# eckertzhang/Text2NeRF

Hardware: AMD Instinct MI355X
Metric: ray-samples/s (render) + iters/s (train), 300^3 VM-split, 800x800 (higher is better)
Workload: dtype f32 (basis/MLP products as f16x2-split MFMA, fp32 accumulate); 1 GPU; C2 300^3 800x800 view/GPU, N=518, S1-soft seed 0, white_bg, weights=0, tile marcher; evaluated_samples_per_frame=77423712, appearance_samples_per_frame=4284741, rays_per_gpu=640000, samples_per_ray=518, warmup_frames=233, inregion_timing=none, parallelism=ray-tile x1

## Files before the change

include/t2n.h:

```cpp
#ifndef T2N_H_
#define T2N_H_

#include <stddef.h>
#include <stdint.h>

#ifdef __cplusplus
extern "C" {
#endif

typedef struct t2n_field t2n_field;
typedef void* t2n_stream;

enum {
    T2N_OK = 0,
    T2N_ERR_INVALID = -1,
    T2N_ERR_UNSUPPORTED = -2,
    T2N_ERR_HIP = -3,
    T2N_ERR_WORKSPACE = -4,
    T2N_ERR_STATE = -5
};

enum { T2N_SHADE_MLP_FEA_NOVIEW = 0, T2N_SHADE_SH = 1, T2N_SHADE_RGB = 2,
       T2N_SHADE_MLP_FEA = 3, T2N_SHADE_MLP_PE = 4, T2N_SHADE_MLP = 5 };
enum { T2N_ACT_SOFTPLUS = 0, T2N_ACT_RELU = 1 };

enum {
    T2N_FLAG_TRAIN = 1u,
    T2N_FLAG_ADD_BG = 2u,
    T2N_FLAG_KEEP_CTX = 4u,
    T2N_FLAG_NDC = 16u,
    T2N_FLAG_DEVICE_ROWS = 32u,
    T2N_FLAG_PIPELINE = 64u,
    T2N_FLAG_GATHER_BATCH = 128u,
    T2N_FLAG_REG_L1 = 256u,
    T2N_FLAG_REG_ORTHO = 512u,
    T2N_FLAG_COHERENT = 8u
};

typedef struct t2n_field_desc {
    float aabb_min[3], aabb_max[3];
    float inv_aabb_size[3];
    int32_t grid[3];
    int32_t density_n_comp;
    int32_t app_n_comp;
    int32_t app_dim;
    int32_t shading;
    int32_t fea_pe;
    int32_t feature_c;
    int32_t act;
    float density_shift;
    float distance_scale;
    float weight_thres;
    float step_size;
    float near, far;
    float z_gate;
    int32_t view_pe, pos_pe;
} t2n_field_desc;

typedef struct t2n_field_params {
    const float* density_plane[3];
    const float* density_line[3];
    const float* app_plane[3];
    const float* app_line[3];
    const float* basis_weight;
    const float* mlp_w0; const float* mlp_b0;
    const float* mlp_w1; const float* mlp_b1;
    const float* mlp_w2; const float* mlp_b2;
} t2n_field_params;

typedef struct t2n_field_grads {
    float* density_plane[3];
    float* density_line[3];
    float* app_plane[3];
    float* app_line[3];
    float* basis_weight;
    float* mlp_w0; float* mlp_b0;
    float* mlp_w1; float* mlp_b1;
    float* mlp_w2; float* mlp_b2;
} t2n_field_grads;

enum { T2N_STAT_EVALUATED = 0,
       T2N_STAT_APPEARANCE = 1,
       T2N_STAT_RAYS = 2,
       T2N_STAT_OVERFLOW = 3,
       T2N_STAT_F16_REDO = 4,
       T2N_STAT_LIST_RETRY = 5,
       T2N_STAT_COUNT = 8 };

const char* t2n_last_error(void);
int t2n_version(void);

int t2n_field_create(const t2n_field_desc* desc, t2n_field** out);
int t2n_field_destroy(t2n_field* f);
int t2n_field_upload(t2n_field* f, const t2n_field_params* p, t2n_stream stream);
int t2n_field_set_desc(t2n_field* f, const t2n_field_desc* desc);
int t2n_field_set_factor_storage(t2n_field* f, int bf16);

int t2n_field_set_mlp_precision(t2n_field* f, int exact_fp32);
int t2n_field_set_alpha_mask(t2n_field* f, const float* volume, int D, int H, int W, const float* aabb_min_host,
                             const float* inv_size_host, t2n_stream stream);
int t2n_alpha_at(const t2n_field* f, const float* xyz_world, int64_t n, float* alpha, t2n_stream stream);
int t2n_field_set_early_termination(t2n_field* f, float eps);
int t2n_field_set_feature_staging(t2n_field* f, int on);
int t2n_field_feature_staging_counts(const t2n_field* f, uint64_t out[2]);
int t2n_field_set_density_cache(t2n_field* f, int on);
int t2n_field_set_density_cache_cap(t2n_field* f, uint64_t bytes);
int t2n_field_release_density_cache(t2n_field* f);
int t2n_field_density_cache_counts(const t2n_field* f, uint64_t out[4]);
int t2n_field_density_sum_table(const t2n_field* f, const int* shift, float* out, t2n_stream stream);
#define T2N_APP_VOLUME_MIN_FRAMES 33
int t2n_field_set_appearance_volume(t2n_field* f, int on, int min_frames);
int t2n_field_set_appearance_volume_cap(t2n_field* f, uint64_t bytes);
int t2n_field_release_appearance_volume(t2n_field* f);
int t2n_field_appearance_volume_counts(const t2n_field* f, uint64_t out[4]);
int t2n_field_set_feature_fusion(t2n_field* f, int on);
int t2n_field_feature_fusion_counts(const t2n_field* f, uint64_t out[2]);
int t2n_render_list_shape(int64_t n_rays, int n_samples, int entries_per_ray, uint64_t out[6]);
int t2n_field_feature_rows(t2n_field* f, const float* app_pos, const uint32_t* counters, uint32_t list_cap, int volume, float* feat,
                           uint32_t feat_rows, t2n_stream stream);
int t2n_field_set_feature_stage_shape(t2n_field* f, int workgroups, int defer_cap);
int t2n_field_set_frame_width(t2n_field* f, int width);

int t2n_ray_directions(int H, int W, float fx, float fy, float cx, float cy, int normalize, float* dirs ,
                       t2n_stream stream);
int t2n_get_rays(const float* dirs , int64_t n, const float* c2w_host ,
                 float* rays_o , float* rays_d , float* rays6 ,
                 t2n_stream stream);
int t2n_generate_rays(int H, int W, float fx, float fy, float cx, float cy, const float* c2w_host, float* rays6,
                      t2n_stream stream);

int t2n_sample_ray(const t2n_field* f, const float* rays_o, const float* rays_d, int64_t n, int n_samples, const float* jitter, int ndc,
                   float* pts , float* z_vals , uint8_t* valid , t2n_stream stream);

int t2n_filter_rays_bbox(const t2n_field* f, const float* rays, int64_t n_rays, int ray_stride, uint8_t* mask,
                         t2n_stream stream);

int t2n_density_at(const t2n_field* f, const float* xyz_norm, int64_t n, float* feat, float* sigma, t2n_stream stream);
size_t t2n_shade_workspace_bytes(int64_t n);
int t2n_shade_at(const t2n_field* f, const float* xyz_norm, const float* viewdirs, int64_t n, float* app_feat, float* rgb,
                 void* workspace, size_t workspace_bytes, t2n_stream stream);
int t2n_raw2alpha(const float* sigma, const float* dist, int64_t n_rays, int n_samples, float* alpha, float* weights,
                  float* bg, t2n_stream stream);

size_t t2n_render_workspace_bytes(int64_t rays_per_launch, int n_samples);
size_t t2n_render_head_scratch_bytes(const t2n_field* f, int64_t n_rays);
int t2n_field_set_head_scratch_rows(t2n_field* f, int rows_per_ray);
size_t t2n_render_workspace_bytes_hint(const t2n_field* f, int64_t n_rays, int n_samples);
size_t t2n_render_workspace_bytes_budget(int64_t n_rays, int n_samples, int entries_per_ray);
uint64_t t2n_field_list_retries(const t2n_field* f);
int t2n_render_forward(t2n_field* f, const float* rays, int64_t n_rays, int ray_stride, int n_samples, uint32_t flags,
                       const float* jitter, float* rgb, float* depth, float* weights, float* z_vals, uint64_t* stats,
                       void* workspace, size_t workspace_bytes, t2n_stream stream);

typedef struct t2n_generic_desc {
    float aabb_min[3], aabb_max[3], inv_aabb_size[3];
    int32_t grid[3];
    int32_t density_n_comp[3], app_n_comp[3];
    int32_t app_dim, shading, fea_pe, view_pe, feature_c, act;
    float density_shift, distance_scale, weight_thres, step_size, near, far, z_gate;
    const float* alpha_volume;
    int32_t alpha_dims[3];
    float alpha_aabb_min[3], alpha_aabb_max[3];
} t2n_generic_desc;
size_t t2n_generic_workspace_bytes(int64_t n_rays, int n_samples);
size_t t2n_generic_workspace_bytes_desc(const t2n_generic_desc* desc, int64_t n_rays, int n_samples);
int t2n_generic_forward(const t2n_generic_desc* desc, const t2n_field_params* params, const float* rays, int64_t n_rays, int ray_stride,
                        int n_samples, uint32_t flags, const float* jitter, float* rgb, float* depth, float* weights, float* z_vals,
                        uint64_t* stats, void* workspace, size_t workspace_bytes, t2n_stream stream);
int t2n_generic_backward(const t2n_generic_desc* desc, const t2n_field_params* params, const float* rays, int64_t n_rays, int ray_stride,
                         int n_samples, uint32_t flags, const float* jitter, const float* weights, const float* z_vals,
                         const float* d_rgb, const float* d_depth, const float* d_weights, const t2n_field_grads* grads,
                         void* workspace, size_t workspace_bytes, t2n_stream stream);
typedef struct t2n_generic_bwd_plan {
    int kernel_form;
    uint32_t pass_rows;
    uint32_t max_passes;
    size_t workspace_bytes;
} t2n_generic_bwd_plan;
int t2n_generic_backward_plan(const t2n_generic_desc* desc, int64_t n_rays, int n_samples, uint32_t pass_rows, t2n_generic_bwd_plan* out);
int t2n_generic_backward_staged(const t2n_generic_desc* desc, const t2n_field_params* params, const float* rays, int64_t n_rays,
                                int ray_stride, int n_samples, uint32_t flags, const float* jitter, const float* weights,
                                const float* z_vals, const float* d_rgb, const float* d_depth, const float* d_weights,
                                const t2n_field_grads* grads, void* workspace, size_t workspace_bytes, void* bwd_workspace,
                                size_t bwd_bytes, uint32_t pass_rows, t2n_stream stream);
int t2n_generic_dense_alpha(const t2n_generic_desc* desc, const t2n_field_params* params, const float* lin_x, const float* lin_y,
                            const float* lin_z, int gx, int gy, int gz, float length, float* alpha, t2n_stream stream);
int t2n_generic_filter_rays(const t2n_generic_desc* desc, const float* rays, int64_t n_rays, int ray_stride, int n_samples, int bbox_only,
                            uint8_t* mask, t2n_stream stream);

int t2n_ndc_rays(int H, int W, float focal, float near, int blender, const float* rays_o, const float* rays_d, int64_t n,
                 float* o_out, float* d_out, t2n_stream stream);

int t2n_eval_sh_bases(int deg, const float* dirs, int64_t n, float* out, t2n_stream stream);

int t2n_ray_marcher(const float* rays, int64_t n, int ray_stride, int n_samples, int lindisp, const float* bbox_host,
                    const float* steps, const float* perturb, float* xyz, float* z_vals, float* near_far, t2n_stream stream);

int t2n_frame_postprocess(const float* rgb , const float* depth , int64_t n, float depth_sub, float depth_add,
                          int shift_clamp, float mi, float ma, uint8_t* rgb8, uint8_t* depth8, const float* gt_rgb, double* sq_err_sum,
                          t2n_stream stream);

size_t t2n_ssim_views_workspace_bytes(int V, int H, int W, int filter_size);
int t2n_ssim_views(const void* img0, const void* img1, int dtype , int V, int H, int W,
                   const double* filter_host , int filter_size, double c1, double c2, int clamp01_img0,
                   double* ssim , double* ssim_map , double* sq_err ,
                   void* workspace, size_t workspace_bytes, t2n_stream stream);

size_t t2n_image_filter_workspace_bytes(int H, int W);
int t2n_sparse_bilateral_filtering(const float* depth , const float* image , int H, int W,
                                   const int* filter_sizes_host, int num_iter, float depth_threshold, float* photo_out,
                                   float* depth_out, void* workspace, size_t workspace_bytes, t2n_stream stream);
size_t t2n_warp_workspace_bytes(int H, int W);
int t2n_warp_view(const float* rgb , const float* depth , const uint8_t* mask1 , int H,
                  int W, const double* Ki9_host, const double* T12_host, const double* K9_host, uint8_t* filled, uint8_t* image_u8,
                  double* depth_out, void* workspace, size_t workspace_bytes, t2n_stream stream);
int t2n_warp_finish(const uint8_t* filled, const uint8_t* image_u8, int H, int W, float* image_out ,
                    int64_t* mask_out , t2n_stream stream);

int t2n_dibr_filter_mask2(float* image, int32_t* known, double* depth, int H, int W, float threshold, t2n_stream stream);
int t2n_dibr_filter_mask(float* image, int32_t* known, int H, int W, t2n_stream stream);

size_t t2n_warp_views_workspace_bytes(int H, int W, int V);
int t2n_warp_views(const float* rgb, const float* depth, const uint8_t* mask1, const uint8_t* mask_aux, int H, int W, int V,
                   const double* Ki9_host, const double* T12_host, const double* K9_host, float* image_out, int64_t* mask_out,
                   double* depth_out, float* depth32_out, int64_t* aux_out, void* workspace, size_t workspace_bytes,
                   t2n_stream stream);

enum { T2N_MASK_U8 = 0, T2N_MASK_I32 = 1, T2N_MASK_I64 = 2, T2N_MASK_F32 = 3, T2N_MASK_F64 = 4 };
size_t t2n_format_views_workspace_bytes(int H, int W, int N);
int t2n_format_views(const float* images, const float* depths, const void* masks, int mask_dtype, int N, int H, int W,
                     const float* c2w_host, float fx, float fy, float cx, float cy, float* rays_split, float* all_rays,
                     float* all_rgbs, float* all_depths, int64_t capacity_rows, int64_t* record, void* workspace,
                     size_t workspace_bytes, t2n_stream stream);

size_t t2n_image_filter_views_workspace_bytes(int H, int W, int V);
int t2n_sparse_bilateral_filtering_views(const float* depth, const float* image, int V, int H, int W, const int* filter_sizes_host,
                                         int num_iter, float depth_threshold, float* photo_out, float* depth_out, void* workspace,
                                         size_t workspace_bytes, t2n_stream stream);
size_t t2n_warp_sources_workspace_bytes(int H, int W, int V);
int t2n_warp_sources(const float* rgb, const float* depth, const uint8_t* mask1, int H, int W, int V, const double* Ki9_host,
                     const double* T12_host, const double* K9_host, float* image_out, int64_t* mask_out, double* depth_out,
                     void* workspace, size_t workspace_bytes, t2n_stream stream);
int t2n_inpaint_pack(const float* warp_image, const int32_t* known, const float* rgb_render, const float* depth_render, int H, int W,
                     uint8_t* warp_u8, int64_t* map_filt, uint8_t* mask_image, uint8_t* mask_inv, int64_t* mask_ex, uint8_t* rgb_u8,
                     uint8_t* rgb_masked_u8, double* depth_masked, t2n_stream stream);

size_t t2n_render_workspace_bytes_ctx(int64_t n_rays, int n_samples);
int t2n_render_ctx_rows(const void* fwd_workspace, int64_t n_rays, int n_samples, t2n_stream stream, int64_t* rows);
int t2n_field_device_rows_record(const t2n_field* f, uint32_t out[10]);
size_t t2n_backward_workspace_bytes(const t2n_field* f, int64_t rows, int64_t n_rays, int n_samples);
int t2n_render_backward(t2n_field* f, const float* rays, int64_t n_rays, int ray_stride, int n_samples, uint32_t flags,
                        const float* jitter, const float* d_rgb, const float* d_depth, const float* d_weights,
                        const t2n_field_grads* g, void* fwd_workspace, size_t fwd_workspace_bytes, void* bwd_workspace,
                        size_t bwd_workspace_bytes, t2n_stream stream);

size_t t2n_field_grad_buffer_bytes(const t2n_field* f);
int t2n_field_set_grad_buffer(t2n_field* f, void* buf, size_t bytes);
size_t t2n_field_grad_buffer_density_bytes(const t2n_field* f);
int t2n_field_wait_density_grads(const t2n_field* f, t2n_stream waiter);

size_t t2n_train_loss_workspace_bytes(int64_t n_rays);
int t2n_train_loss(const float* rgb, const float* depth, const float* weights, const float* z_vals, const float* rgb_t,
                   const float* depth_t, int64_t n_rays, int n_samples, float w_depth, float w_trans, float delta, float* d_rgb,
                   float* d_depth, float* d_weights, float* losses, void* workspace, size_t workspace_bytes, t2n_stream stream);

size_t t2n_train_loss_ex_workspace_bytes(int64_t n_rays);
int t2n_train_loss_ex(const float* rgb, const float* depth, const float* weights, const float* z_vals, const float* rgb_t,
                      const float* depth_t, int64_t n_rays, int n_samples, float w_depth, float w_trans, float delta, int depth_kind,
                      float target_std, float* d_rgb, float* d_depth, float* d_weights, float* losses, double* aux, void* workspace,
                      size_t workspace_bytes, t2n_stream stream);
// ... 140 lines not shown
```

text2nerf_amd/_lib.py:

```python
from __future__ import annotations

import ctypes as C
import os
import threading

_HERE = os.path.dirname(os.path.abspath(__file__))
LIB_PATH = os.environ.get("T2N_LIB") or os.path.join(_HERE, "libt2n_hip.so")

T2N_STAT_COUNT = 8
T2N_K_COUNT = 14
KERNEL_NAMES = ("march", "shade", "composite", "upload", "bwd_march", "bwd_mlp", "bwd_scatter", "density", "app_features",
                "bwd_wgrad", "bwd_density", "tv_seed", "adam", "head_step")
STAT_EVALUATED, STAT_APPEARANCE, STAT_RAYS, STAT_OVERFLOW, STAT_F16_REDO, STAT_LIST_RETRY = 0, 1, 2, 3, 4, 5

FLAG_TRAIN, FLAG_ADD_BG, FLAG_KEEP_CTX, FLAG_COHERENT, FLAG_NDC = 1, 2, 4, 8, 16
FLAG_DEVICE_ROWS = 32
FLAG_PIPELINE = 64
FLAG_GATHER_BATCH = 128
FLAG_REG_L1, FLAG_REG_ORTHO = 256, 512
REG_SLOTS = 64
SHADE_IDS = {"MLP_Fea_noview": 0, "SH": 1, "RGB": 2, "MLP_Fea": 3, "MLP_PE": 4, "MLP": 5}
ACT_IDS = {"softplus": 0, "relu": 1}
DEPTH_KINDS = {"mse": 0, "gnll": 1, "si_log": 2, "ssi": 3}
MASK_U8, MASK_I32, MASK_I64, MASK_F32, MASK_F64 = 0, 1, 2, 3, 4


class T2NError(RuntimeError):
    pass


class FieldDesc(C.Structure):
    _fields_ = [("aabb_min", C.c_float * 3), ("aabb_max", C.c_float * 3), ("inv_aabb_size", C.c_float * 3),
                ("grid", C.c_int32 * 3), ("density_n_comp", C.c_int32), ("app_n_comp", C.c_int32),
                ("app_dim", C.c_int32), ("shading", C.c_int32), ("fea_pe", C.c_int32), ("feature_c", C.c_int32),
                ("act", C.c_int32), ("density_shift", C.c_float), ("distance_scale", C.c_float),
                ("weight_thres", C.c_float), ("step_size", C.c_float), ("near", C.c_float), ("far", C.c_float),
                ("z_gate", C.c_float), ("view_pe", C.c_int32), ("pos_pe", C.c_int32)]


class FieldParams(C.Structure):
    _fields_ = [("density_plane", C.c_void_p * 3), ("density_line", C.c_void_p * 3), ("app_plane", C.c_void_p * 3),
                ("app_line", C.c_void_p * 3), ("basis_weight", C.c_void_p),
                ("mlp_w0", C.c_void_p), ("mlp_b0", C.c_void_p), ("mlp_w1", C.c_void_p), ("mlp_b1", C.c_void_p),
                ("mlp_w2", C.c_void_p), ("mlp_b2", C.c_void_p)]


FieldGrads = FieldParams


class GenericDesc(C.Structure):
    _fields_ = [("aabb_min", C.c_float * 3), ("aabb_max", C.c_float * 3), ("inv_aabb_size", C.c_float * 3), ("grid", C.c_int32 * 3),
                ("density_n_comp", C.c_int32 * 3), ("app_n_comp", C.c_int32 * 3), ("app_dim", C.c_int32), ("shading", C.c_int32),
                ("fea_pe", C.c_int32), ("view_pe", C.c_int32), ("feature_c", C.c_int32), ("act", C.c_int32),
                ("density_shift", C.c_float), ("distance_scale", C.c_float), ("weight_thres", C.c_float), ("step_size", C.c_float),
                ("near", C.c_float), ("far", C.c_float), ("z_gate", C.c_float),
                ("alpha_volume", C.c_void_p), ("alpha_dims", C.c_int32 * 3), ("alpha_aabb_min", C.c_float * 3),
                ("alpha_aabb_max", C.c_float * 3)]


class GenericBwdPlan(C.Structure):
    _fields_ = [("kernel_form", C.c_int), ("pass_rows", C.c_uint32), ("max_passes", C.c_uint32), ("workspace_bytes", C.c_size_t)]


TRAIN_HYPER_FLOATS = 32
TRAIN_HEAD_GRAD_FLOATS = 27 * 144 + 128 * 351 + 128 + 128 * 128 + 128 + 3 * 128 + 3 + 1
TRAIN_HEAD_SIZES = (27 * 144, 128 * 351, 128, 128 * 128, 128, 3 * 128, 3)


class TrainStepArgs(C.Structure):
    _fields_ = [("rays", C.c_void_p), ("n_rays", C.c_int64), ("ray_stride", C.c_int32), ("n_samples", C.c_int32),
                ("flags", C.c_uint32), ("phases", C.c_uint32),
                ("jitter", C.c_void_p), ("rgb_target", C.c_void_p), ("depth_target", C.c_void_p),
                ("w_depth", C.c_float), ("w_trans", C.c_float), ("delta", C.c_float),
                ("beta1", C.c_float), ("beta2", C.c_float), ("eps", C.c_float),
                ("hyper", C.c_void_p), ("params", FieldParams),
                ("exp_avg", C.c_void_p * 19), ("exp_avg_sq", C.c_void_p * 19),
                ("head_grads", C.c_void_p), ("rows_capacity", C.c_int64),
                ("workspace", C.c_void_p), ("workspace_bytes", C.c_size_t), ("losses", C.c_void_p), ("host_batch", C.c_void_p), ("host_batch_bytes", C.c_size_t), ("batch_buffer", C.c_void_p),
                ("shard_world", C.c_int32), ("shard_rank", C.c_int32)]


class TrainSource(C.Structure):
    _fields_ = [("rays", C.c_void_p), ("ray_stride", C.c_int32), ("rgb", C.c_void_p), ("depth", C.c_void_p), ("n_rows", C.c_int64),
                ("ids", C.c_void_p)]


_lib = None
_lock = threading.Lock()

SIGNATURES = {
    "t2n_last_error": (C.c_char_p, []),
    "t2n_version": (C.c_int, []),
    "t2n_field_create": (C.c_int, [C.POINTER(FieldDesc), C.POINTER(C.c_void_p)]),
    "t2n_field_destroy": (C.c_int, [C.c_void_p]),
    "t2n_field_upload": (C.c_int, [C.c_void_p, C.POINTER(FieldParams), C.c_void_p]),
    "t2n_field_set_desc": (C.c_int, [C.c_void_p, C.POINTER(FieldDesc)]),
    "t2n_field_set_mlp_precision": (C.c_int, [C.c_void_p, C.c_int]),
    "t2n_field_set_early_termination": (C.c_int, [C.c_void_p, C.c_float]),
    "t2n_field_set_feature_staging": (C.c_int, [C.c_void_p, C.c_int]),
    "t2n_field_feature_staging_counts": (C.c_int, [C.c_void_p, C.POINTER(C.c_uint64)]),
    "t2n_field_set_feature_stage_shape": (C.c_int, [C.c_void_p, C.c_int, C.c_int]),
    "t2n_field_set_density_cache": (C.c_int, [C.c_void_p, C.c_int]),
    "t2n_field_set_density_cache_cap": (C.c_int, [C.c_void_p, C.c_uint64]),
    "t2n_field_release_density_cache": (C.c_int, [C.c_void_p]),
    "t2n_field_density_cache_counts": (C.c_int, [C.c_void_p, C.POINTER(C.c_uint64)]),
    "t2n_field_set_appearance_volume": (C.c_int, [C.c_void_p, C.c_int, C.c_int]),
    "t2n_field_set_appearance_volume_cap": (C.c_int, [C.c_void_p, C.c_uint64]),
    "t2n_field_release_appearance_volume": (C.c_int, [C.c_void_p]),
    "t2n_field_appearance_volume_counts": (C.c_int, [C.c_void_p, C.POINTER(C.c_uint64)]),
    "t2n_field_set_feature_fusion": (C.c_int, [C.c_void_p, C.c_int]),
    "t2n_field_feature_fusion_counts": (C.c_int, [C.c_void_p, C.POINTER(C.c_uint64)]),
    "t2n_render_list_shape": (C.c_int, [C.c_int64, C.c_int, C.c_int, C.POINTER(C.c_uint64)]),
    "t2n_field_feature_rows": (C.c_int, [C.c_void_p, C.c_void_p, C.c_void_p, C.c_uint32, C.c_int, C.c_void_p, C.c_uint32, C.c_void_p]),
    "t2n_field_density_sum_table": (C.c_int, [C.c_void_p, C.POINTER(C.c_int), C.c_void_p, C.c_void_p]),
    "t2n_sample_ray": (C.c_int, [C.c_void_p, C.c_void_p, C.c_void_p, C.c_int64, C.c_int, C.c_void_p, C.c_int, C.c_void_p, C.c_void_p,
                                 C.c_void_p, C.c_void_p]),
    "t2n_field_set_frame_width": (C.c_int, [C.c_void_p, C.c_int]),
    "t2n_field_set_alpha_mask": (C.c_int, [C.c_void_p, C.c_void_p, C.c_int, C.c_int, C.c_int, C.POINTER(C.c_float),
                                           C.POINTER(C.c_float), C.c_void_p]),
    "t2n_alpha_at": (C.c_int, [C.c_void_p, C.c_void_p, C.c_int64, C.c_void_p, C.c_void_p]),
    "t2n_ray_directions": (C.c_int, [C.c_int, C.c_int, C.c_float, C.c_float, C.c_float, C.c_float, C.c_int,
                                     C.c_void_p, C.c_void_p]),
    "t2n_get_rays": (C.c_int, [C.c_void_p, C.c_int64, C.POINTER(C.c_float), C.c_void_p, C.c_void_p, C.c_void_p,
                               C.c_void_p]),
    "t2n_generate_rays": (C.c_int, [C.c_int, C.c_int, C.c_float, C.c_float, C.c_float, C.c_float,
                                    C.POINTER(C.c_float), C.c_void_p, C.c_void_p]),
    "t2n_filter_rays_bbox": (C.c_int, [C.c_void_p, C.c_void_p, C.c_int64, C.c_int, C.c_void_p, C.c_void_p]),
    "t2n_density_at": (C.c_int, [C.c_void_p, C.c_void_p, C.c_int64, C.c_void_p, C.c_void_p, C.c_void_p]),
    "t2n_shade_workspace_bytes": (C.c_size_t, [C.c_int64]),
    "t2n_shade_at": (C.c_int, [C.c_void_p, C.c_void_p, C.c_void_p, C.c_int64, C.c_void_p, C.c_void_p, C.c_void_p,
                               C.c_size_t, C.c_void_p]),
    "t2n_raw2alpha": (C.c_int, [C.c_void_p, C.c_void_p, C.c_int64, C.c_int, C.c_void_p, C.c_void_p, C.c_void_p,
                                C.c_void_p]),
    "t2n_render_workspace_bytes": (C.c_size_t, [C.c_int64, C.c_int]),
    "t2n_render_head_scratch_bytes": (C.c_size_t, [C.c_void_p, C.c_int64]),
    "t2n_field_set_head_scratch_rows": (C.c_int, [C.c_void_p, C.c_int]),
    "t2n_render_workspace_bytes_hint": (C.c_size_t, [C.c_void_p, C.c_int64, C.c_int]),
    "t2n_field_list_retries": (C.c_uint64, [C.c_void_p]),
    "t2n_render_workspace_bytes_budget": (C.c_size_t, [C.c_int64, C.c_int, C.c_int]),
    "t2n_render_forward": (C.c_int, [C.c_void_p, C.c_void_p, C.c_int64, C.c_int, C.c_int, C.c_uint32, C.c_void_p,
                                     C.c_void_p, C.c_void_p, C.c_void_p, C.c_void_p, C.c_void_p, C.c_void_p,
                                     C.c_size_t, C.c_void_p]),
    "t2n_render_workspace_bytes_ctx": (C.c_size_t, [C.c_int64, C.c_int]),
    "t2n_depth_align_global": (C.c_int, [C.c_void_p, C.c_void_p, C.c_int, C.c_int, C.c_void_p, C.c_int, C.c_double, C.c_void_p, C.c_void_p,
                                         C.c_void_p]),
    "t2n_depth_align_fallback": (C.c_int, [C.c_void_p, C.c_void_p, C.c_int, C.c_int, C.c_double, C.c_void_p, C.c_void_p, C.c_void_p]),
    "t2n_filled_pixels_workspace_bytes": (C.c_size_t, [C.c_int, C.c_int]),
    "t2n_filled_pixels_count": (C.c_int, [C.c_void_p, C.c_int, C.c_int, C.c_void_p, C.c_void_p, C.c_void_p]),
    "t2n_filled_pixels_select": (C.c_int, [C.c_void_p, C.c_int, C.c_int, C.c_void_p, C.c_void_p, C.c_int, C.c_void_p, C.c_void_p]),
    "t2n_depth_merge_inputs": (C.c_int, [C.c_void_p, C.c_void_p, C.c_void_p, C.c_int, C.c_int, C.c_double, C.c_void_p, C.c_void_p,
                                         C.c_void_p, C.c_void_p]),
    "t2n_view_finish": (C.c_int, [C.c_void_p, C.c_void_p, C.c_void_p, C.c_int, C.c_int, C.c_double, C.c_void_p, C.c_void_p, C.c_void_p,
                                  C.c_void_p]),
    "t2n_mask_expand": (C.c_int, [C.c_void_p, C.c_int, C.c_int, C.c_void_p, C.c_void_p, C.c_void_p]),
    "t2n_mc_workspace_bytes": (C.c_size_t, [C.c_int, C.c_int, C.c_int]),
    "t2n_mc_count": (C.c_int, [C.c_void_p, C.c_int, C.c_int, C.c_int, C.c_float, C.c_void_p, C.c_void_p, C.c_void_p]),
    "t2n_mc_emit": (C.c_int, [C.c_void_p, C.c_int, C.c_int, C.c_int, C.c_float, C.c_void_p, C.POINTER(C.c_float), C.POINTER(C.c_float),
                              C.c_int, C.c_void_p, C.c_void_p, C.c_void_p, C.c_void_p]),
    "t2n_mesh_components_workspace_bytes": (C.c_size_t, [C.c_int64, C.c_int64]),
    "t2n_mesh_components": (C.c_int, [C.c_void_p, C.c_int64, C.c_int64, C.c_void_p, C.c_void_p, C.c_void_p, C.c_size_t, C.c_void_p]),
    "t2n_mesh_component_sizes": (C.c_int, [C.c_void_p, C.c_int64, C.c_void_p, C.c_int64, C.c_int64, C.c_void_p, C.c_void_p, C.c_void_p]),
    "t2n_mesh_filter_count": (C.c_int, [C.c_void_p, C.c_int64, C.c_void_p, C.c_int64, C.c_void_p, C.c_int64, C.c_void_p, C.c_size_t,
                                        C.c_void_p, C.c_void_p]),
    "t2n_mesh_filter_emit": (C.c_int, [C.c_void_p, C.c_int64, C.c_void_p, C.c_int64, C.c_void_p, C.c_int64, C.c_void_p, C.c_void_p,
                                       C.c_void_p, C.c_void_p, C.c_size_t, C.c_void_p, C.c_void_p, C.c_void_p, C.c_void_p, C.c_void_p]),
    "t2n_field_grad_buffer_bytes": (C.c_size_t, [C.c_void_p]),
    "t2n_field_set_grad_buffer": (C.c_int, [C.c_void_p, C.c_void_p, C.c_size_t]),
    "t2n_field_grad_buffer_density_bytes": (C.c_size_t, [C.c_void_p]),
    "t2n_field_wait_density_grads": (C.c_int, [C.c_void_p, C.c_void_p]),
    "t2n_train_loss_workspace_bytes": (C.c_size_t, [C.c_int64]),
    "t2n_train_loss": (C.c_int, [C.c_void_p, C.c_void_p, C.c_void_p, C.c_void_p, C.c_void_p, C.c_void_p, C.c_int64, C.c_int, C.c_float,
                                 C.c_float, C.c_float, C.c_void_p, C.c_void_p, C.c_void_p, C.c_void_p, C.c_void_p, C.c_size_t, C.c_void_p]),
    "t2n_train_loss_ex_workspace_bytes": (C.c_size_t, [C.c_int64]),
    "t2n_train_loss_ex": (C.c_int, [C.c_void_p, C.c_void_p, C.c_void_p, C.c_void_p, C.c_void_p, C.c_void_p, C.c_int64, C.c_int, C.c_float,
                                    C.c_float, C.c_float, C.c_int, C.c_float, C.c_void_p, C.c_void_p, C.c_void_p, C.c_void_p, C.c_void_p,
                                    C.c_void_p, C.c_size_t, C.c_void_p]),
    "t2n_depth_loss_workspace_bytes": (C.c_size_t, [C.c_int64]),
    "t2n_depth_loss": (C.c_int, [C.c_int, C.c_void_p, C.c_void_p, C.c_void_p, C.c_void_p, C.c_int64, C.c_int, C.c_float, C.c_void_p,
                                 C.c_void_p, C.c_void_p, C.c_void_p, C.c_void_p, C.c_size_t, C.c_void_p]),
    "t2n_distortion_loss_workspace_bytes": (C.c_size_t, [C.c_int64]),
    "t2n_distortion_loss": (C.c_int, [C.c_void_p, C.c_void_p, C.c_int64, C.c_int, C.c_float, C.c_void_p, C.c_void_p, C.c_void_p, C.c_size_t,
                                      C.c_void_p]),
    "t2n_train_loss_dist_workspace_bytes": (C.c_size_t, [C.c_int64]),
    "t2n_train_loss_dist": (C.c_int, [C.c_void_p, C.c_void_p, C.c_void_p, C.c_void_p, C.c_void_p, C.c_void_p, C.c_int64, C.c_int, C.c_float,
                                      C.c_float, C.c_float, C.c_int, C.c_float, C.c_float, C.c_float, C.c_void_p, C.c_void_p, C.c_void_p,
                                      C.c_void_p, C.c_void_p, C.c_void_p, C.c_void_p, C.c_size_t, C.c_void_p]),
    "t2n_field_set_factor_storage": (C.c_int, [C.c_void_p, C.c_int]),
    "t2n_frame_postprocess": (C.c_int, [C.c_void_p, C.c_void_p, C.c_int64, C.c_float, C.c_float, C.c_int, C.c_float, C.c_float,
                              C.c_void_p, C.c_void_p, C.c_void_p, C.c_void_p, C.c_void_p]),
    "t2n_ssim_views_workspace_bytes": (C.c_size_t, [C.c_int, C.c_int, C.c_int, C.c_int]),
    "t2n_ssim_views": (C.c_int, [C.c_void_p, C.c_void_p, C.c_int, C.c_int, C.c_int, C.c_int, C.POINTER(C.c_double), C.c_int, C.c_double,
                                 C.c_double, C.c_int, C.c_void_p, C.c_void_p, C.c_void_p, C.c_void_p, C.c_size_t, C.c_void_p]),
    "t2n_image_filter_workspace_bytes": (C.c_size_t, [C.c_int, C.c_int]),
    "t2n_sparse_bilateral_filtering": (C.c_int, [C.c_void_p, C.c_void_p, C.c_int, C.c_int, C.POINTER(C.c_int), C.c_int, C.c_float,
                                                 C.c_void_p, C.c_void_p, C.c_void_p, C.c_size_t, C.c_void_p]),
    "t2n_warp_workspace_bytes": (C.c_size_t, [C.c_int, C.c_int]),
    "t2n_warp_view": (C.c_int, [C.c_void_p, C.c_void_p, C.c_void_p, C.c_int, C.c_int, C.POINTER(C.c_double), C.POINTER(C.c_double),
                                C.POINTER(C.c_double), C.c_void_p, C.c_void_p, C.c_void_p, C.c_void_p, C.c_size_t, C.c_void_p]),
    "t2n_warp_finish": (C.c_int, [C.c_void_p, C.c_void_p, C.c_int, C.c_int, C.c_void_p, C.c_void_p, C.c_void_p]),
    "t2n_warp_views_workspace_bytes": (C.c_size_t, [C.c_int, C.c_int, C.c_int]),
    "t2n_warp_views": (C.c_int, [C.c_void_p, C.c_void_p, C.c_void_p, C.c_void_p, C.c_int, C.c_int, C.c_int, C.POINTER(C.c_double),
                                 C.POINTER(C.c_double), C.POINTER(C.c_double), C.c_void_p, C.c_void_p, C.c_void_p, C.c_void_p,
                                 C.c_void_p, C.c_void_p, C.c_size_t, C.c_void_p]),
    "t2n_format_views_workspace_bytes": (C.c_size_t, [C.c_int, C.c_int, C.c_int]),
    "t2n_format_views": (C.c_int, [C.c_void_p, C.c_void_p, C.c_void_p, C.c_int, C.c_int, C.c_int, C.c_int, C.POINTER(C.c_float),
                                   C.c_float, C.c_float, C.c_float, C.c_float, C.c_void_p, C.c_void_p, C.c_void_p, C.c_void_p,
                                   C.c_int64, C.c_void_p, C.c_void_p, C.c_size_t, C.c_void_p]),
    "t2n_image_filter_views_workspace_bytes": (C.c_size_t, [C.c_int, C.c_int, C.c_int]),
    "t2n_sparse_bilateral_filtering_views": (C.c_int, [C.c_void_p, C.c_void_p, C.c_int, C.c_int, C.c_int, C.POINTER(C.c_int), C.c_int,
                                                       C.c_float, C.c_void_p, C.c_void_p, C.c_void_p, C.c_size_t, C.c_void_p]),
    "t2n_warp_sources_workspace_bytes": (C.c_size_t, [C.c_int, C.c_int, C.c_int]),
    "t2n_warp_sources": (C.c_int, [C.c_void_p, C.c_void_p, C.c_void_p, C.c_int, C.c_int, C.c_int, C.POINTER(C.c_double),
                                   C.POINTER(C.c_double), C.POINTER(C.c_double), C.c_void_p, C.c_void_p, C.c_void_p, C.c_void_p,
                                   C.c_size_t, C.c_void_p]),
    "t2n_inpaint_pack": (C.c_int, [C.c_void_p, C.c_void_p, C.c_void_p, C.c_void_p, C.c_int, C.c_int, C.c_void_p, C.c_void_p, C.c_void_p,
                                   C.c_void_p, C.c_void_p, C.c_void_p, C.c_void_p, C.c_void_p, C.c_void_p]),
    "t2n_adam_step_multi": (C.c_int, [C.c_int, C.c_void_p, C.c_void_p, C.c_void_p, C.c_void_p, C.c_void_p, C.c_void_p, C.c_float,
                            C.c_float, C.c_float, C.c_void_p, C.c_void_p]),
    "t2n_ray_marcher": (C.c_int, [C.c_void_p, C.c_int64, C.c_int, C.c_int, C.c_int, C.POINTER(C.c_float), C.c_void_p, C.c_void_p,
                        C.c_void_p, C.c_void_p, C.c_void_p, C.c_void_p]),
    "t2n_dibr_filter_mask2": (C.c_int, [C.c_void_p, C.c_void_p, C.c_void_p, C.c_int, C.c_int, C.c_float, C.c_void_p]),
    "t2n_dibr_filter_mask": (C.c_int, [C.c_void_p, C.c_void_p, C.c_int, C.c_int, C.c_void_p]),
    "t2n_eval_sh_bases": (C.c_int, [C.c_int, C.c_void_p, C.c_int64, C.c_void_p, C.c_void_p]),
    "t2n_ndc_rays": (C.c_int, [C.c_int, C.c_int, C.c_float, C.c_float, C.c_int, C.c_void_p, C.c_void_p, C.c_int64, C.c_void_p,
                     C.c_void_p, C.c_void_p]),
    "t2n_render_ctx_rows": (C.c_int, [C.c_void_p, C.c_int64, C.c_int, C.c_void_p, C.POINTER(C.c_int64)]),
    "t2n_field_device_rows_record": (C.c_int, [C.c_void_p, C.POINTER(C.c_uint32)]),
    "t2n_backward_workspace_bytes": (C.c_size_t, [C.c_void_p, C.c_int64, C.c_int64, C.c_int]),
    "t2n_render_backward": (C.c_int, [C.c_void_p, C.c_void_p, C.c_int64, C.c_int, C.c_int, C.c_uint32, C.c_void_p,
                                      C.c_void_p, C.c_void_p, C.c_void_p, C.POINTER(FieldGrads), C.c_void_p, C.c_size_t,
                                      C.c_void_p, C.c_size_t, C.c_void_p]),
    "t2n_tv_grad_add": (C.c_int, [C.c_void_p, C.c_void_p, C.c_int, C.c_int, C.c_int, C.c_float, C.c_void_p]),
    "t2n_tv_value": (C.c_int, [C.c_void_p, C.c_int, C.c_int, C.c_int, C.c_void_p, C.c_void_p]),
    "t2n_tv_grad_set": (C.c_int, [C.c_void_p, C.c_void_p, C.c_int, C.c_int, C.c_int, C.c_float, C.c_void_p, C.c_void_p]),
    "t2n_field_tv_adam_step": (C.c_int, [C.c_void_p, C.c_void_p, C.c_void_p, C.c_void_p, C.c_void_p, C.c_void_p, C.c_float, C.c_float,
                                         C.c_float, C.c_float, C.c_float, C.c_void_p]),
    "t2n_field_tv_seed": (C.c_int, [C.c_void_p, C.c_float, C.c_float, C.c_void_p]),
    "t2n_l1_value": (C.c_int, [C.c_void_p, C.c_int64, C.c_void_p, C.c_void_p]),
    "t2n_l1_grad_add": (C.c_int, [C.c_void_p, C.c_void_p, C.c_int64, C.c_float, C.c_void_p]),
    "t2n_l1_grad_set": (C.c_int, [C.c_void_p, C.c_void_p, C.c_int64, C.c_float, C.c_void_p, C.c_void_p]),
    "t2n_ortho_workspace_bytes": (C.c_size_t, [C.c_int]),
    "t2n_ortho_value": (C.c_int, [C.c_void_p, C.c_int, C.c_int64, C.c_void_p, C.c_void_p, C.c_size_t, C.c_void_p]),
    "t2n_ortho_grad_add": (C.c_int, [C.c_void_p, C.c_void_p, C.c_int, C.c_int64, C.c_float, C.c_void_p, C.c_size_t, C.c_void_p]),
    "t2n_ortho_grad_set": (C.c_int, [C.c_void_p, C.c_void_p, C.c_int, C.c_int64, C.c_float, C.c_void_p, C.c_void_p, C.c_size_t,
                                     C.c_void_p]),
    "t2n_field_reg_seed": (C.c_int, [C.c_void_p, C.c_float, C.c_float, C.c_float, C.c_float, C.c_float, C.c_float, C.c_void_p]),
    "t2n_field_reg_adam_step": (C.c_int, [C.c_void_p, C.c_void_p, C.c_void_p, C.c_void_p, C.c_void_p, C.c_void_p, C.c_float, C.c_float,
                                          C.c_float, C.c_float, C.c_float, C.c_float, C.c_float, C.c_float, C.c_float, C.c_void_p]),
    "t2n_field_upload_head": (C.c_int, [C.c_void_p, C.c_void_p, C.c_void_p]),
    "t2n_adam_step": (C.c_int, [C.c_void_p, C.c_void_p, C.c_void_p, C.c_void_p, C.c_int64, C.c_float, C.c_float, C.c_float,
                                C.c_float, C.c_int64, C.c_void_p]),
    "t2n_compute_alpha": (C.c_int, [C.c_void_p, C.c_void_p, C.c_int64, C.c_float, C.c_void_p, C.c_void_p]),
    "t2n_dense_alpha": (C.c_int, [C.c_void_p, C.c_void_p, C.c_void_p, C.c_void_p, C.c_int, C.c_int, C.c_int, C.c_float,
                                  C.c_void_p, C.c_void_p]),
    "t2n_alpha_volume": (C.c_int, [C.c_void_p, C.c_int, C.c_int, C.c_int, C.c_float, C.c_void_p, C.c_void_p, C.c_void_p]),
    "t2n_upsample_bilinear": (C.c_int, [C.c_void_p, C.c_int, C.c_int, C.c_int, C.c_void_p, C.c_int, C.c_int, C.c_void_p]),
    "t2n_filter_rays_alpha": (C.c_int, [C.c_void_p, C.c_void_p, C.c_int64, C.c_int, C.c_int, C.c_void_p, C.c_void_p]),
    "t2n_generic_workspace_bytes": (C.c_size_t, [C.c_int64, C.c_int]),
    "t2n_generic_workspace_bytes_desc": (C.c_size_t, [C.POINTER(GenericDesc), C.c_int64, C.c_int]),
    "t2n_generic_forward": (C.c_int, [C.POINTER(GenericDesc), C.POINTER(FieldParams), C.c_void_p, C.c_int64, C.c_int, C.c_int, C.c_uint32,
                                      C.c_void_p, C.c_void_p, C.c_void_p, C.c_void_p, C.c_void_p, C.c_void_p, C.c_void_p, C.c_size_t,
                                      C.c_void_p]),
    "t2n_generic_backward": (C.c_int, [C.POINTER(GenericDesc), C.POINTER(FieldParams), C.c_void_p, C.c_int64, C.c_int, C.c_int, C.c_uint32,
                                       C.c_void_p, C.c_void_p, C.c_void_p, C.c_void_p, C.c_void_p, C.c_void_p, C.POINTER(FieldGrads),
# ... 60 lines not shown
```

text2nerf_amd/csrc/t2n_api.hip:

```cpp
#include <stdarg.h>

#include "t2n_device.h"

namespace t2n {

static thread_local char g_err[512] = "";

void set_error(const char* fmt, ...) {
    va_list ap;
    va_start(ap, fmt);
    vsnprintf(g_err, sizeof(g_err), fmt, ap);
    va_end(ap);
}

int hip_fail(hipError_t e, const char* what) {
    set_error("HIP error %d (%s) in %s", (int)e, hipGetErrorString(e), what);
    return T2N_ERR_HIP;
}

void timing_begin(t2n_field* f, int k, hipStream_t s) {
    if (!((f->timing >> k) & 1)) return;
    TimingSlot& t = f->slots[k];
    if (t.used >= kTimingEvents) return;
    if (!t.start[t.used]) {
// ... 751 lines not shown
                    ShadeCtx ctx{nullptr, feat32 - row0 * 32, nullptr, nullptr};
                    if ((rc = launch_shade_list(f, L.app_pos, L.app_ray, L.rays, ray_stride, L.counters, L.list_cap, L.app_rgb, &ctx, s, true,
                                                (unsigned)(row0 + cap), nullptr, 0, nullptr, (unsigned)(row0 / 32), (unsigned)((row0 + cap) / 32)))) return rc;
                    if ((rc = launch_head_forward(f, nullptr, cap, feat32, L.app_pos, L.app_ray, L.rays, ray_stride, L.counters, L.list_cap, x0, h0,
                                                  h1, L.app_rgb, s, plan, row0))) return rc;
                }
            }
        } else {
            if (kr.rows >= 32) {
                ShadeCtx ctx{(float*)(ws + kr.x144), (float*)(ws + kr.feat32), (float*)(ws + kr.h0), (float*)(ws + kr.h1)};
                if ((rc = launch_shade_list(f, L.app_pos, L.app_ray, L.rays, ray_stride, L.counters, L.list_cap, L.app_rgb, &ctx, s, false, kr.rows))) return rc;
            } else if ((rc = launch_shade_list(f, L.app_pos, L.app_ray, L.rays, ray_stride, L.counters, L.list_cap, L.app_rgb, nullptr, s, false,
                                               0xffffffffu, keep ? nullptr : L.feat, L.feat_rows, stats, 0, 0xffffffffu, L.slot_rows))) return rc;
        }
        if ((rc = tiles ? launch_composite(f, L, s, f->frame_w, (int)(cnt / f->frame_w)) : launch_composite(f, L, s))) return rc;
        if (tiles && finish_supported(f) && (rc = launch_finish_rays(f, L, (const float*)(ws + c.sigma), (const float4*)(ws + c.scratch), s))) return rc;
    }
    return T2N_OK;
}

extern "C" size_t t2n_render_workspace_bytes_hint(const t2n_field* f, int64_t n_rays, int n_samples) {
    if (!f || n_rays <= 0 || n_samples <= 0) return 0;
    counts_poll(const_cast<t2n_field*>(f), false);
    const size_t worst = carve(n_rays, n_samples).total;
    if (n_rays < kBudgetMinRays) return worst;
    unsigned b = f->list_hint ? f->list_hint + f->list_hint / 2u + 12u : 32u;
    if (b < kBudgetMin) b = kBudgetMin;
    if (b >= (unsigned)n_samples) return worst;
    const size_t want = carve_workspace(n_rays, n_samples, true, true, b).total;
    return want < worst ? want : worst;
}
extern "C" uint64_t t2n_field_list_retries(const t2n_field* f) {
    if (!f) return 0;
    counts_poll(const_cast<t2n_field*>(f), true);
    return f->list_retries;
}
extern "C" size_t t2n_render_workspace_bytes_budget(int64_t n_rays, int n_samples, int entries_per_ray) {
    if (n_rays <= 0 || n_samples <= 0 || entries_per_ray < 0) return 0;
    return carve_workspace(n_rays, n_samples, true, true, (unsigned)entries_per_ray).total;
}

extern "C" int t2n_field_set_alpha_mask(t2n_field* f, const float* volume, int D, int H, int W, const float* aabb_min_host,
                                        const float* inv_size_host, t2n_stream stream) {
    if (!f) { set_error("t2n_field_set_alpha_mask: NULL field"); return T2N_ERR_INVALID; }
    if (f->buf_alpha) { T2N_HIP(hipStreamSynchronize((hipStream_t)stream)); (void)hipFree(f->buf_alpha); f->buf_alpha = nullptr; }
    f->dev.alpha = nullptr;
    if (!volume) return T2N_OK;
    if (D < 1 || H < 1 || W < 1 || !aabb_min_host || !inv_size_host) { set_error("t2n_field_set_alpha_mask: bad argument"); return T2N_ERR_INVALID; }
    const size_t bytes = (size_t)D * H * W * sizeof(float);
    T2N_HIP(hipMalloc((void**)&f->buf_alpha, bytes));
    T2N_HIP(hipMemcpyAsync(f->buf_alpha, volume, bytes, hipMemcpyDeviceToDevice, (hipStream_t)stream));
    f->dev.alpha = f->buf_alpha; f->dev.aD = D; f->dev.aH = H; f->dev.aW = W;
    for (int k = 0; k < 3; ++k) { f->dev.a_min[k] = aabb_min_host[k]; f->dev.a_inv[k] = inv_size_host[k]; }
    return T2N_OK;
}

extern "C" int t2n_field_set_head_scratch_rows(t2n_field* f, int rows_per_ray) {
    if (!f || rows_per_ray < 1 || rows_per_ray > 4096) { set_error("t2n_field_set_head_scratch_rows: rows_per_ray must lie in [1, 4096]"); return T2N_ERR_INVALID; }
    f->head_rows_per_ray = rows_per_ray;
    return T2N_OK;
}

extern "C" int t2n_field_set_frame_width(t2n_field* f, int width) {
    if (!f || width < 0) { set_error("t2n_field_set_frame_width: bad argument"); return T2N_ERR_INVALID; }
    f->frame_w = width;
    return T2N_OK;
}

extern "C" int t2n_field_set_factor_storage(t2n_field* f, int bf16) {
    if (!f) { set_error("t2n_field_set_factor_storage: NULL field"); return T2N_ERR_INVALID; }
    if ((bf16 != 0) != (f->factor_bf16 != 0)) f->uploaded = false;
    f->factor_bf16 = bf16 ? 1 : 0;
    if (!f->factor_bf16)
        for (int k = 0; k < 3; ++k) {
            f->dev.den.plane_h[k] = f->dev.den.line_h[k] = f->dev.app.plane_h[k] = f->dev.app.line_h[k] = nullptr;
        }
    return T2N_OK;
}

extern "C" int t2n_field_set_early_termination(t2n_field* f, float eps) {
    if (!f || !(eps >= 0.f) || eps > f->desc.weight_thres) {
        set_error("t2n_field_set_early_termination: eps must lie in [0, weight_thres]");
        return T2N_ERR_INVALID;
    }
    f->term_eps = eps;
    return T2N_OK;
}

extern "C" int t2n_field_set_mlp_precision(t2n_field* f, int exact_fp32) {
    if (!f) { set_error("t2n_field_set_mlp_precision: NULL field"); return T2N_ERR_INVALID; }
    f->mlp_split = exact_fp32 ? 0 : 1;
    return T2N_OK;
}

extern "C" int t2n_field_set_feature_staging(t2n_field* f, int on) {
    if (!f) { set_error("t2n_field_set_feature_staging: NULL field"); return T2N_ERR_INVALID; }
    f->feature_staging = on ? 1 : 0;
    return T2N_OK;
}

extern "C" int t2n_field_set_density_cache(t2n_field* f, int on) {
    if (!f) { set_error("t2n_field_set_density_cache: NULL field"); return T2N_ERR_INVALID; }
    f->dcache_on = on ? 1 : 0;
    return T2N_OK;
}
extern "C" int t2n_field_set_density_cache_cap(t2n_field* f, uint64_t bytes) {
    if (!f) { set_error("t2n_field_set_density_cache_cap: NULL field"); return T2N_ERR_INVALID; }
    f->dcache_cap = (size_t)bytes;
    f->dcache_alloc_failed = false;
    return T2N_OK;
}
extern "C" int t2n_field_release_density_cache(t2n_field* f) {
    if (!f) { set_error("t2n_field_release_density_cache: NULL field"); return T2N_ERR_INVALID; }
    density_cache_release(f);
    return T2N_OK;
}
extern "C" int t2n_field_density_cache_counts(const t2n_field* f, uint64_t out[4]) {
    if (!f || !out) { set_error("t2n_field_density_cache_counts: NULL argument"); return T2N_ERR_INVALID; }
    out[0] = f->dcache_counts[0]; out[1] = f->dcache_counts[1]; out[2] = f->dcache_counts[2]; out[3] = (uint64_t)f->dcache_bytes;
    return T2N_OK;
}
extern "C" int t2n_field_set_appearance_volume(t2n_field* f, int on, int min_frames) {
    if (!f || min_frames < 0) { set_error("t2n_field_set_appearance_volume: NULL field or min_frames < 0"); return T2N_ERR_INVALID; }
    f->avol_on = on ? 1 : 0;
    f->avol_min_frames = min_frames ? min_frames : T2N_APP_VOLUME_MIN_FRAMES;
    return T2N_OK;
}
extern "C" int t2n_field_set_appearance_volume_cap(t2n_field* f, uint64_t bytes) {
    if (!f) { set_error("t2n_field_set_appearance_volume_cap: NULL field"); return T2N_ERR_INVALID; }
    f->avol_cap = (size_t)bytes;
    f->avol_alloc_failed = false;
    return T2N_OK;
}
extern "C" int t2n_field_release_appearance_volume(t2n_field* f) {
    if (!f) { set_error("t2n_field_release_appearance_volume: NULL field"); return T2N_ERR_INVALID; }
    appearance_volume_release(f);
    return T2N_OK;
}
extern "C" int t2n_field_appearance_volume_counts(const t2n_field* f, uint64_t out[4]) {
    if (!f || !out) { set_error("t2n_field_appearance_volume_counts: NULL argument"); return T2N_ERR_INVALID; }
    out[0] = (uint64_t)f->avol_bytes; out[1] = f->avol_counts[2]; out[2] = f->avol_counts[0]; out[3] = f->avol_counts[1];
    return T2N_OK;
}
extern "C" int t2n_field_set_feature_fusion(t2n_field* f, int on) {
    if (!f) { set_error("t2n_field_set_feature_fusion: NULL field"); return T2N_ERR_INVALID; }
    f->fusion_on = on ? 1 : 0;
    return T2N_OK;
}
extern "C" int t2n_field_feature_fusion_counts(const t2n_field* f, uint64_t out[2]) {
    if (!f || !out) { set_error("t2n_field_feature_fusion_counts: NULL argument"); return T2N_ERR_INVALID; }
    out[0] = f->fusion_counts[0]; out[1] = f->fusion_counts[1];
    return T2N_OK;
}
extern "C" int t2n_render_list_shape(int64_t n_rays, int n_samples, int entries_per_ray, uint64_t out[6]) {
    if (n_rays <= 0 || n_samples <= 0 || entries_per_ray < 0 || !out) { set_error("t2n_render_list_shape: bad argument"); return T2N_ERR_INVALID; }
    const Carve c = carve_workspace(n_rays, n_samples, true, true, (unsigned)entries_per_ray);
    out[0] = c.list_cap; out[1] = c.feat_rows; out[2] = fuse_rows(c.list_cap, c.feat_rows) ? 1 : 0;
    out[3] = c.app_pos; out[4] = c.feat; out[5] = c.counters;
    return T2N_OK;
}
extern "C" int t2n_field_feature_rows(t2n_field* f, const float* app_pos, const uint32_t* counters, uint32_t list_cap, int volume, float* feat,
                                      uint32_t feat_rows, t2n_stream stream) {
    if (!f || !app_pos || !counters || !feat || feat_rows % 32u) { set_error("t2n_field_feature_rows: bad argument"); return T2N_ERR_INVALID; }
    if (!f->uploaded) { set_error("t2n_field_feature_rows: the field has no uploaded parameters"); return T2N_ERR_STATE; }
    if (f->desc.shading != T2N_SHADE_MLP_FEA_NOVIEW || !f->mlp_split) { set_error("t2n_field_feature_rows: needs the fused MLP_Fea_noview head on split products"); return T2N_ERR_UNSUPPORTED; }
    hipStream_t s = (hipStream_t)stream;
    AvolScope avol_scope{f};
    f->dev.avol = nullptr;
    if (volume) {
        const int on = f->avol_on, mf = f->avol_min_frames;
        f->avol_on = 1; f->avol_min_frames = 1;
        const int rc = appearance_volume_prepare(f, s);
        f->avol_on = on; f->avol_min_frames = mf;
        if (rc) return rc;
        if (!f->dev.avol) { set_error("t2n_field_feature_rows: this field gets no feature volume (cap, addressing, allocation)"); return T2N_ERR_UNSUPPORTED; }
    }
    return launch_feature_rows(f, (const float4*)app_pos, counters, list_cap, feat, feat_rows, s);
}
extern "C" int t2n_field_density_sum_table(const t2n_field* f, const int* shift, float* out, t2n_stream stream) {
    if (!f || !shift || !out) { set_error("t2n_field_density_sum_table: NULL argument"); return T2N_ERR_INVALID; }
    if (!f->uploaded) { set_error("t2n_field_density_sum_table: the field has no uploaded factors"); return T2N_ERR_STATE; }
    return launch_density_sum_table(f, out, shift, (hipStream_t)stream);
}

extern "C" int t2n_field_set_feature_stage_shape(t2n_field* f, int workgroups, int defer_cap) {
    if (!f) { set_error("t2n_field_set_feature_stage_shape: NULL field"); return T2N_ERR_INVALID; }
    if (workgroups < 0 || defer_cap < 0 || defer_cap > 64) { set_error("t2n_field_set_feature_stage_shape: workgroups >= 0, defer_cap in [0, 64]"); return T2N_ERR_INVALID; }
    f->feature_workgroups = workgroups;
    f->feature_defer_cap = defer_cap ? defer_cap : 16;
    return T2N_OK;
}

extern "C" int t2n_field_feature_staging_counts(const t2n_field* f, uint64_t out[2]) {
    if (!f || !out) { set_error("t2n_field_feature_staging_counts: NULL argument"); return T2N_ERR_INVALID; }
    out[0] = out[1] = 0;
    if (!f->staging_counts) return T2N_OK;
    T2N_HIP(hipDeviceSynchronize());
    unsigned long long h[2];
    T2N_HIP(hipMemcpy(h, f->staging_counts, sizeof(h), hipMemcpyDeviceToHost));
    out[0] = h[0]; out[1] = h[1];
    return T2N_OK;
}

extern "C" int t2n_timing_enable(t2n_field* f, int on) {
    if (!f) return T2N_ERR_INVALID;
    f->timing = on == 0 ? 0 : (on == 1 ? (1 << T2N_K_COUNT) - 1 : (on >> 1) & ((1 << T2N_K_COUNT) - 1));
    return T2N_OK;
}

extern "C" int t2n_timing_read(t2n_field* f, double* ms, int64_t* launches, int reset) {
    if (!f || !ms || !launches) { set_error("t2n_timing_read: NULL argument"); return T2N_ERR_INVALID; }
    timing_flush(f);
    for (int k = 0; k < T2N_K_COUNT; ++k) {
        ms[k] = f->slots[k].ms; launches[k] = f->slots[k].launches;
        if (reset) { f->slots[k].ms = 0.0; f->slots[k].launches = 0; }
    }
    return T2N_OK;
}
```

text2nerf_amd/csrc/t2n_app_rows.h:

```cpp
#pragma once
#include "t2n_internal.h"
#include "t2n_device.h"

namespace t2n {

struct AvVolume { const float* avol; unsigned row, slice, ny1; };

template <int LPE>
__device__ __forceinline__ void av_feature_row(const FactorSet& app, const AvVolume& v, const float4 mine, const bool live, const int q,
                                               float* __restrict__ row, const bool store) {
    constexpr int NQ = 8 / LPE;
    const char* __restrict__ V = reinterpret_cast<const char*>(v.avol);
    const Axes3 A = sample_axes_inbox(app, mine.x, mine.y, mine.z);
    const unsigned ix = (unsigned)min(max(A.a[0].i0, 0), app.W[0] - 1), iy = (unsigned)min(max(A.a[1].i0, 0), app.H[0] - 1);
    const unsigned iz = (unsigned)min(max(A.a[2].i0, 0), app.H[1] - 1);
    const unsigned cell = umad24(umad24(iz, v.ny1, iy), v.row, ix * kAvCornerBytes);
    const unsigned o00 = (live ? cell : 0u) + (unsigned)q * 16u;
    const unsigned o01 = o00 + v.row, o10 = o00 + v.slice, o11 = o10 + v.row;
    const unsigned off[4] = {o00, o01, o10, o11};
    float4 c[4][2][NQ];
#pragma unroll
    for (int zy = 0; zy < 4; ++zy)
#pragma unroll
        for (int x = 0; x < 2; ++x)
#pragma unroll
            for (int i = 0; i < NQ; ++i)
                c[zy][x][i] = *reinterpret_cast<const float4*>(V + (size_t)off[zy] + ((int)kAvCornerBytes * x + 16 * LPE * i));
    __builtin_amdgcn_sched_barrier(0);
    const float wx0 = live ? A.a[0].w0 : 0.f, wx1 = live ? A.a[0].w1 : 0.f;
    const float wyx[2][2] = {{A.a[1].w0 * wx0, A.a[1].w0 * wx1}, {A.a[1].w1 * wx0, A.a[1].w1 * wx1}};
    const float wz[2] = {A.a[2].w0, A.a[2].w1};
    float4 r[NQ];
#pragma unroll
    for (int zy = 0; zy < 4; ++zy)
#pragma unroll
        for (int x = 0; x < 2; ++x) {
            const float w = wyx[zy & 1][x] * wz[zy >> 1];
#pragma unroll
            for (int i = 0; i < NQ; ++i) r[i] = (zy == 0 && x == 0) ? f4_mul(c[0][0][i], w) : f4_fma(c[zy][x][i], w, r[i]);
        }
    if (q == 6 % LPE) r[6 / LPE].w = live ? mine.w : 0.f;
    if (q == 7 % LPE) r[7 / LPE] = make_float4(0.f, 0.f, 0.f, 0.f);
    if (store) {
#pragma unroll
        for (int i = 0; i < NQ; ++i) *reinterpret_cast<float4*>(row + 4 * LPE * i) = r[i];
    }
}

__device__ __forceinline__ void av_slot_rows(const FactorSet& app, const AvVolume& v, const float4* pos, float* feat, unsigned count, int lane) {
    typedef unsigned u32x4_t __attribute__((ext_vector_type(4)));
    const int e = lane >> 3, q = lane & 7;
    const auto rsrc = __builtin_amdgcn_make_buffer_rsrc(const_cast<float4*>(pos), 0, (int)(count * 16u), 0x00020000);
#pragma unroll 1
    for (unsigned c0 = 0; c0 < count; c0 += 64u) {
        const unsigned left = count - c0;
        const unsigned mine_i = (unsigned)lane < left ? c0 + (unsigned)lane : count - 1u;
        const u32x4_t p = __builtin_amdgcn_raw_buffer_load_b128(rsrc, (int)(mine_i * 16u), 0, 16);
        const unsigned npass = left < 64u ? (left + 7u) >> 3 : 8u;
#pragma unroll 1
        for (unsigned s = 0; s < npass; ++s) {
            const int src = (int)(8u * s) + e;
            const float4 mine = make_float4(__uint_as_float(__shfl(p.x, src)), __uint_as_float(__shfl(p.y, src)),
                                            __uint_as_float(__shfl(p.z, src)), __uint_as_float(__shfl(p.w, src)));
            const bool live = (unsigned)src < left;
            av_feature_row<8>(app, v, mine, live, q, feat + (size_t)(c0 + (unsigned)src) * 32u + 4u * (unsigned)q, live);
        }
    }
}

}
```

text2nerf_amd/csrc/t2n_internal.h:

```cpp
#pragma once
#include <hip/hip_runtime.h>
#include <stdint.h>
#include <stdio.h>
#include <string.h>

#include "../../include/t2n.h"

namespace t2n {

constexpr int kWave = 64;
constexpr int kMaxSamples = 8192;
constexpr int kAppDimMax = 32;

__host__ __device__ constexpr int mat0(int k) { return k == 2 ? 1 : 0; }
__host__ __device__ constexpr int mat1(int k) { return k == 0 ? 1 : 2; }
__host__ __device__ constexpr int vecm(int k) { return 2 - k; }

struct FactorSet {
    const float* plane[3];
    const float* line[3];
    int W[3], H[3], L[3];
    int C;
    const void* plane_h[3];
    const void* line_h[3];
};

struct FieldDev {
    FactorSet den, app;
    float aabb0[3], aabb1[3], inv[3];
    float shift, dscale, thres, step, near, far, zgate;
    int act, shading, app_dim;
    const float* basisA;
    const float* w0A;
    const float* w1A;
    const float* w2A;
    const float* alpha; int aW, aH, aD; float a_min[3], a_inv[3];
    const uint4* basisH; const uint4* w0H; const uint4* w1H; const uint4* w2H; const float* biasH;
    const float* ztab;
    float term_eps;
    const float* dsum; unsigned ds_row, ds_slice;
    const float* avol; unsigned av_row, av_slice;
};

struct TrainScalars {
    float lr_over_bc1[19];
    float inv_bc2_sqrt;
    unsigned skip;
    unsigned pad[3];
};
struct TrainState {
    unsigned step;
    unsigned seq;
    unsigned skipped;
    unsigned pad[5];
    TrainScalars sc[2];
};

constexpr int kTimingEvents = 1024;
struct TimingSlot {
    hipEvent_t start[kTimingEvents], stop[kTimingEvents];
    int used = 0;
    int64_t untimed = 0;
    double ms = 0.0;
    int64_t launches = 0;
};

}

struct t2n_field {
    t2n_field_desc desc;
    t2n::FieldDev dev;
    float* buf_den_plane[3] = {nullptr, nullptr, nullptr};
    float* buf_den_line[3] = {nullptr, nullptr, nullptr};
    float* buf_app_plane[3] = {nullptr, nullptr, nullptr};
    float* buf_app_line[3] = {nullptr, nullptr, nullptr};
    void* hbuf_den_plane[3] = {nullptr, nullptr, nullptr};
    void* hbuf_den_line[3] = {nullptr, nullptr, nullptr};
    void* hbuf_app_plane[3] = {nullptr, nullptr, nullptr};
    void* hbuf_app_line[3] = {nullptr, nullptr, nullptr};
    int factor_bf16 = 0;
    float* buf_mlp = nullptr;
    void* buf_mlp_h = nullptr;
    const unsigned* split_unsafe = nullptr;
    void* buf_ss = nullptr;
    bool ss_dirty = true;
    void* ss_event = nullptr; void* ss_stream = nullptr;
    unsigned* ss_ok_host = nullptr; void* ss_ok_event = nullptr; int ss_variant = -2;
    float* buf_alpha = nullptr;
    int mlp_split = 1;
    int feature_staging = 1;
    unsigned long long* staging_counts = nullptr;
    int feature_defer_cap = 16;
    int feature_workgroups = 0;
    float* gbuf_den_plane[3] = {nullptr, nullptr, nullptr};
    float* gbuf_den_line[3] = {nullptr, nullptr, nullptr};
    float* gbuf_app_plane[3] = {nullptr, nullptr, nullptr};
    float* gbuf_app_line[3] = {nullptr, nullptr, nullptr};
    bool gbuf_external = false;
    float* gbuf_all = nullptr; size_t gbuf_bytes = 0;
    t2n_field_params params_ref;
    bool uploaded = false;
    int timing = 0;
    int frame_w = 0;
    int head_rows_per_ray = 32;
    float term_eps = 0.f;
    t2n::TimingSlot slots[T2N_K_COUNT];
    static constexpr int kCountSlots = 4;
    struct CountSlot { unsigned* host = nullptr; void* ev = nullptr; bool pending = false; int64_t n_rays = 0; int n_samples = 0; unsigned budget = 0; };
    CountSlot count_slots[kCountSlots]; int count_next = 0;
    void* side_stream = nullptr; void* ev_fork = nullptr; void* ev_join = nullptr;
    void* ev_den = nullptr;
    unsigned* plan_host = nullptr; unsigned plan_seq = 0;
    void* ev_pack = nullptr;
    void* gemm_stream = nullptr; void* ev_fork2 = nullptr; void* ev_join2 = nullptr;
    void* train_dev = nullptr; unsigned* train_host = nullptr; void* train_ev[12] = {};
    unsigned train_calls = 0; bool train_chain = false;
    bool train_packed = false;
    t2n_train_source train_src = {}; bool train_src_set = false;
    bool train_src_fresh = false;
    unsigned list_hint = 0;
    void* reg_ws = nullptr; size_t reg_ws_bytes = 0;
    unsigned long long list_retries = 0;
    float* dcache = nullptr; size_t dcache_bytes = 0;
    unsigned long long den_version = 1, dcache_version = 0, dcache_seen = 0;
    int dcache_on = 1; size_t dcache_cap = 0;
    bool dcache_alloc_failed = false;
    void* dcache_ev = nullptr; void* dcache_stream = nullptr;
    unsigned long long dcache_counts[3] = {0, 0, 0};
    float* avol = nullptr; size_t avol_bytes = 0;
    unsigned long long app_version = 1, avol_version = 0, avol_seen = 0, avol_run = 0;
    int avol_on = 1, avol_min_frames = T2N_APP_VOLUME_MIN_FRAMES; size_t avol_cap = 0;
    bool avol_alloc_failed = false;
    void* avol_ev = nullptr; void* avol_stream = nullptr;
    unsigned long long avol_counts[3] = {0, 0, 0};
    int fusion_on = 1;
    unsigned long long fusion_counts[2] = {0, 0};
};

namespace t2n {

void set_error(const char* fmt, ...);
int hip_fail(hipError_t e, const char* what);

#define T2N_HIP(call)                                        \
    do {                                                     \
        hipError_t e__ = (call);                             \
        if (e__ != hipSuccess) return t2n::hip_fail(e__, #call); \
    } while (0)

void counts_poll(t2n_field* f, bool wait);
void timing_begin(t2n_field* f, int k, hipStream_t s);
void timing_end(t2n_field* f, int k, hipStream_t s);

int launch_relayout(t2n_field* f, const t2n_field_params* p, hipStream_t s);
int launch_pack_mlp(t2n_field* f, const t2n_field_params* p, hipStream_t s, unsigned* absmax_out = nullptr);

struct RenderLaunch {
    const float* rays; int64_t n_rays; int ray_stride; int n_samples; uint32_t flags;
    const float* jitter; float* rgb; float* depth; float* weights; float* z_vals; uint64_t* stats;
    float* acc; int4* ray_app; unsigned* counters; float4* app_pos; int* app_ray; float4* app_rgb; unsigned list_cap;
    float* feat = nullptr; unsigned feat_rows = 0;
    bool slot_rows = false;
    float* sigma_ctx; float4* rgb_raw;
};
int launch_march(t2n_field* f, const RenderLaunch& L, hipStream_t s);
int launch_ray_stats(const RenderLaunch& L, hipStream_t s);
int launch_filter_bbox(const FieldDev& F, const float* rays, long long n_rays, int ray_stride, uint8_t* mask, hipStream_t s);
int launch_filter_alpha(const FieldDev& F, const float* rays, long long n_rays, int ray_stride, int n_samples, uint8_t* mask, hipStream_t s);
size_t density_cache_bytes(const t2n_field* f);
int density_cache_prepare(t2n_field* f, hipStream_t s);
void density_cache_release(t2n_field* f);
int launch_density_sum_table(const t2n_field* f, float* out, const int shift[3], hipStream_t s);
#ifndef T2N_AVOL_STRIDE
#define T2N_AVOL_STRIDE 32
#endif
constexpr int kAvStride = T2N_AVOL_STRIDE;
constexpr int kAvFeatures = 27;
constexpr unsigned kAvCornerBytes = kAvStride * sizeof(float);
static_assert(kAvStride % 4 == 0 && kAvStride >= 28 && kAvStride <= 32, "corner stride: whole quads that hold the 27 features");
struct AvolScope { t2n_field* f; ~AvolScope() { f->dev.avol = nullptr; } };
size_t appearance_volume_bytes(const t2n_field* f);
int appearance_volume_prepare(t2n_field* f, hipStream_t s);
void appearance_volume_release(t2n_field* f);
int launch_app_volume_build(const t2n_field* f, float* out, hipStream_t s);
int launch_app_features_vol(t2n_field* f, const float4* app_pos, const unsigned* counters_dev, unsigned list_cap, unsigned tile_hi, float* feat,
                            hipStream_t s);
int launch_feature_rows(t2n_field* f, const float4* app_pos, const unsigned* counters_dev, unsigned list_cap, float* feat, unsigned feat_rows,
                        hipStream_t s);
int launch_march_tiles(t2n_field* f, const RenderLaunch& L, int img_w, int img_h, float* spill, float4* scratch, hipStream_t s);
constexpr int kLists = 8;
inline bool fuse_rows(unsigned list_cap, unsigned feat_rows) { return feat_rows && (unsigned long long)list_cap * kLists <= feat_rows; }
constexpr int kCounterStride = 64;
inline unsigned list_capacity(long long n_rays, int n_samples) {
    const unsigned nblocks = (unsigned)((n_rays + 3) / 4);
    return ((nblocks >> 3) + ((nblocks & 7u) ? 1u : 0u)) * 4u * (unsigned)n_samples + (unsigned)n_samples;
}
inline unsigned list_capacity_budget(long long n_rays, int n_samples, unsigned budget) {
    const unsigned worst = list_capacity(n_rays, n_samples);
    if (budget == 0 || budget >= (unsigned)n_samples) return worst;
    const unsigned long long per = ((unsigned long long)n_rays * budget + kLists - 1) / kLists + (unsigned)n_samples;
    return per < worst ? (unsigned)per : worst;
}
struct ShadeCtx { float* x144; float* feat32; float* h0; float* h1; };
int launch_shade_list(t2n_field* f, const float4* app_pos, const int* app_ray, const float* rays, int ray_stride,
                      const unsigned* counters_dev, unsigned list_cap, float4* app_rgb, const ShadeCtx* ctx, hipStream_t s,
                      bool features_only = false, unsigned ctx_rows = 0xffffffffu, float* feat = nullptr, unsigned feat_rows = 0,
                      uint64_t* stats = nullptr, unsigned tile_lo = 0, unsigned tile_hi = 0xffffffffu, bool slot_rows = false);
constexpr int kRangeFlagWord = 32;
constexpr int kKeptMagicWord = 33, kKeptRowsWord = 34;
constexpr int kOverflowWord = 35;
constexpr int kHeadPlanWord = 40;
constexpr int kFailEntriesWord = 36;
constexpr unsigned kKeptMagic = 0x4b455054u;
int launch_mlp_ss(t2n_field* f, const float* feat, const unsigned* counters_dev, unsigned list_cap, unsigned tile_hi, float4* app_rgb,
                  unsigned* range_flag, hipStream_t s, bool slot_rows = false);

struct HeadDims { int shading, C, fea_pe, view_pe, pos_pe, o_feat, o_view, o_pe_a, n_pe_a, o_pe_v, n_pe_v, K0, K0pad; };
HeadDims head_dims(const t2n_field_desc& d);
inline bool head_is_generic(int shading) { return shading == T2N_SHADE_MLP_FEA || shading == T2N_SHADE_MLP_PE || shading == T2N_SHADE_MLP; }
struct HeadPlanDev { unsigned t[kLists + 1]; unsigned rows; };
int launch_head_plan(const unsigned* counters, unsigned list_cap, HeadPlanDev* plan, hipStream_t s);
int launch_dense_rows(const float* IN, int ldin, const float* Wt, int K, int N, const float* bias, int relu, long long rows, float* OUT, int ldo,
                      hipStream_t s, const HeadPlanDev* plan, long long row0);
int launch_head_forward(t2n_field* f, const unsigned tiles_before[kLists + 1], long long rows, const float* feat32, const float4* app_pos,
                        const int* app_ray, const float* rays, int ray_stride, const unsigned* counters, unsigned list_cap, float* x0,
                        float* h0, float* h1, float4* app_rgb, hipStream_t s, const HeadPlanDev* plan = nullptr, long long row0 = 0);
int launch_head_in_bwd(t2n_field* f, const float* gx, const float* feat32, long long rows, float* gf, hipStream_t s);
struct SetupOps {
    unsigned* zero_ptr[6]; unsigned long long zero_words[6]; int nz = 0;
    unsigned* set_ptr[4]; unsigned set_val[4]; int ns = 0;
    bool overflow = false;
    void zero(void* p, size_t bytes) {
        if (!p || !bytes) return;
        if (nz >= 6) { overflow = true; return; }
        zero_ptr[nz] = (unsigned*)p; zero_words[nz] = (bytes + 3) / 4; ++nz;
    }
    void set(void* p, unsigned v) {
        if (ns >= 4) { overflow = true; return; }
        set_ptr[ns] = (unsigned*)p; set_val[ns] = v; ++ns;
    }
};
int launch_setup(const SetupOps& o, hipStream_t s);
int launch_simple_head_bwd(t2n_field* f, const unsigned tiles_before[kLists + 1], long long rows, const float4* go, const float4* app_rgb,
                           const int* app_ray, const float* rays, int ray_stride, const unsigned* counters, unsigned list_cap, float* gf,
                           hipStream_t s);

size_t gemm_h_pack_bytes(int K0);
int gemm_h_pack(t2n_field* f, void* buf, int K0, hipStream_t s);
int launch_gemm_nn_h(void* packbuf, int which, int K0, const float* IN, int ldin, long long rows, const float* ACT, int ldact, float* OUT,
                     int ldo, hipStream_t s);
int launch_gemm_tn_b(const float* A, int lda, const float* B, int ldb, long long rows, int N, float* part, int ldp, int chunk_rows,
                     int ng, int chunks, bool pe, float* db, hipStream_t s, const unsigned* rows_dev = nullptr);
struct TnPlan { int chunk_rows, chunks, ng, ldp; };
TnPlan tn_plan(int64_t rows, int N);
size_t tn_part_bytes(int64_t rows, int k0);
bool gemm_fp32_mode(const t2n_field* f);
void launch_bwd_l2(const float4* go, const float* h1, long long rows, const float* w2, float* g1, float* dw2, float* db2, float* scratch,
                   hipStream_t s, const unsigned* rows_dev = nullptr);
void launch_gemm_tn(int MB, bool fp32, const float* A, int lda, const float* B, int ldb, long long rows, int M, int N, float* C, int ldc,
                    float* part, hipStream_t s, const float* pe_feat = nullptr, float* db = nullptr, const unsigned* rows_dev = nullptr,
                    bool reduce = true);
struct WgradRegions { size_t l2, tn[3], total; };
WgradRegions wgrad_regions(int64_t rows, int k0);
void launch_wgrad_reduce(const char* base, long long rows, float* dw2, float* db2, float* dw1, float* dw0, float* dwb, hipStream_t s,
                         const float* loss_part = nullptr, long long n_rays = 0, float w_depth = 0.f, float w_trans = 0.f, float* losses = nullptr);
void launch_gemm_nn(const float* IN, int ldin, const float* W, int ldw, long long rows, int K, int N, const float* ACT, int ldact, float* OUT,
                    int ldo, hipStream_t s);
void launch_colsum(const float* G, int ld, long long rows, int N, float* db, hipStream_t s);
void launch_pe_fwd(const float* feat, long long rows, float* x, hipStream_t s);
void launch_pe_bwd(const float* gx, const float* feat, long long rows, float* gf, hipStream_t s);
size_t mlp_bwd_ss_pack_bytes();
int launch_mlp_bwd_ss(t2n_field* f, void* packbuf, const float4* go, float* h1, const float* h0, const float* feat, float* g0, float* gf,
                      float* gx, long long rows, hipStream_t s, bool packed = false, const unsigned* rows_dev = nullptr,
                      float* g1_out = nullptr);
int mlp_bwd_ss_pack(t2n_field* f, void* packbuf, hipStream_t s, bool zeroed, bool one_launch = false, bool absmax_done = false);
void* mlp_bwd_ss_absmax_words(void* packbuf);
int launch_tv_seed_dev(t2n_field* f, const float* tvw_dev, hipStream_t s, int world = 1, int rank = 0, bool l1_dev = false);
int launch_ortho_lines(t2n_field* f, float w_den, float w_app, const float* w_dev, hipStream_t s);
size_t reg_ws_bytes(const t2n_field* f);
int launch_factor_adam_dev(t2n_field* f, const t2n_field_params* params, float* const* m, float* const* v, float beta1, float beta2, float eps,
                           const TrainScalars* st, int first, int count, hipStream_t s, int world = 1, int rank = 0, bool relayout_only = false);
void shard_partition(const t2n_field* f, int world, int rank, unsigned lo[12], unsigned hi[12], unsigned body[12]);
int launch_head_adam_dev(const t2n_field_params* params, const float* grads_flat, float* const* m, float* const* v, float beta1, float beta2,
                         float eps, const TrainScalars* st, hipStream_t s, bool zero_grads = false, unsigned* zero_words4 = nullptr);
int launch_train_loss(const float* rgb, const float* depth, const float* weights, const float* z_vals, const float* rgb_t, const float* depth_t,
                      int64_t n_rays, int n_samples, float w_depth, float w_trans, float delta, float* d_rgb, float* d_depth, float* d_weights,
                      float* losses, float* part, bool reduce, hipStream_t s);
struct Carve { size_t acc, ray_app, counters, app_pos, app_ray, app_rgb, sigma, rgb_raw, scratch, feat, total; unsigned list_cap, feat_rows; };
Carve carve_workspace(int64_t rays, int n_samples, bool ctx, bool feat = true, unsigned budget = 0);
int launch_composite(t2n_field* f, const RenderLaunch& L, hipStream_t s, int img_w = 0, int img_h = 0);
inline bool finish_supported(const t2n_field* f) { return !head_is_generic(f->desc.shading); }
int launch_finish_rays(t2n_field* f, const RenderLaunch& L, const float* spill, const float4* scratch, hipStream_t s);
int post_counts(const unsigned* counters_dev, unsigned* host_dst, hipStream_t s);
int ctx_counts_post(const void* ws, const unsigned* counters_dev, hipStream_t s);
struct KeptRows { size_t x144, feat32, h0, h1; unsigned rows; };
inline KeptRows kept_rows(size_t ctx_total, size_t workspace_bytes) {
    KeptRows k{0, 0, 0, 0, 0};
    const size_t base = (ctx_total + 255) / 256 * 256;
    if (workspace_bytes <= base) return k;
    size_t rows = (workspace_bytes - base) / ((144 + 32 + 128 + 128) * 4);
    rows = rows / 32 * 32;
    if (rows > 0x7fffffe0u) rows = 0x7fffffe0u;
    k.rows = (unsigned)rows;
    k.x144 = base; k.feat32 = k.x144 + rows * 144 * 4; k.h0 = k.feat32 + rows * 32 * 4; k.h1 = k.h0 + rows * 128 * 4;
    return k;
}

}
```

text2nerf_amd/csrc/t2n_march_tiles.hip:

```cpp
#include "t2n_device.h"
#include "t2n_app_rows.h"

namespace t2n {

constexpr int kMaxLog2W = 2;
constexpr int kDStrideMax = (1 << (2 * kMaxLog2W)) + 4;
constexpr int kPairFloats = 3 * 16 * kDStrideMax;
constexpr int kSumFloats = 96;
constexpr int kStageFloats = kPairFloats + kSumFloats;
static_assert(63 + 21 < kSumFloats && kStageFloats % 4 == 0, "summed table: the farthest read stays in the wave's region; 16-B aligned regions");
typedef float f32x4_t __attribute__((ext_vector_type(4)));

struct TileArgs {
    FieldDev F;
    const float* rays; long long n_rays; int ray_stride; int n_samples; int img_w, img_h;
    float* acc; float* depth; int4* ray_app;
    float* wbuf;
    float4* scratch; int cap; unsigned* ovf_count; int* ovf_list;
    float4* app_pos; int* app_ray; unsigned* counters; unsigned list_cap; unsigned long long* stats;
    float* dense_w;
    float* feat;
#ifdef MT_PROF
    unsigned long long* prof;
#endif
};

__device__ __forceinline__ void lds_fence_w() {
    __builtin_amdgcn_fence(__ATOMIC_RELEASE, "wavefront");
    __builtin_amdgcn_wave_barrier();
    __builtin_amdgcn_fence(__ATOMIC_ACQUIRE, "wavefront");
}

template <int CTRL>
__device__ __forceinline__ int dpp_shr(int v, int identity) {
    return __builtin_amdgcn_update_dpp(identity, v, CTRL, 0xf, 0xf, false);
}
__device__ __forceinline__ int wave_min_i(int v) {
    const int big = 0x7fffffff;
    v = min(v, dpp_shr<0x111>(v, big));
    v = min(v, dpp_shr<0x112>(v, big));
    v = min(v, dpp_shr<0x114>(v, big));
    v = min(v, dpp_shr<0x118>(v, big));
    const int a = __builtin_amdgcn_readlane(v, 15), b = __builtin_amdgcn_readlane(v, 31);
    const int c = __builtin_amdgcn_readlane(v, 47), d = __builtin_amdgcn_readlane(v, 63);
    return min(min(a, b), min(c, d));
}
__device__ __forceinline__ int wave_max_i(int v) {
    const int small = -0x7fffffff;
    v = max(v, dpp_shr<0x111>(v, small));
    v = max(v, dpp_shr<0x112>(v, small));
    v = max(v, dpp_shr<0x114>(v, small));
    v = max(v, dpp_shr<0x118>(v, small));
    const int a = __builtin_amdgcn_readlane(v, 15), b = __builtin_amdgcn_readlane(v, 31);
    const int c = __builtin_amdgcn_readlane(v, 47), d = __builtin_amdgcn_readlane(v, 63);
    return max(max(a, b), max(c, d));
}

__device__ __forceinline__ unsigned wave_or_u(unsigned v) {
    v |= (unsigned)dpp_shr<0x111>((int)v, 0);
    v |= (unsigned)dpp_shr<0x112>((int)v, 0);
    v |= (unsigned)dpp_shr<0x114>((int)v, 0);
    v |= (unsigned)dpp_shr<0x118>((int)v, 0);
    const unsigned a = (unsigned)__builtin_amdgcn_readlane((int)v, 15), b = (unsigned)__builtin_amdgcn_readlane((int)v, 31);
    const unsigned c = (unsigned)__builtin_amdgcn_readlane((int)v, 47), d = (unsigned)__builtin_amdgcn_readlane((int)v, 63);
    return (a | b) | (c | d);
}

template <int LOG2W>
__device__ __forceinline__ void table_build(const FactorSet& S, const int (&amn)[3], float* __restrict__ stD, int l15, int lq) {
    constexpr int WS = 1 << LOG2W, SL = WS * WS, NB = SL / 16, ST = SL + 4;
    const int gs[3] = {S.W[0], S.H[0], S.H[1]};
    float4 av[3][NB], bv[3];
#pragma unroll
    for (int k = 0; k < 3; ++k) {
        const int m0 = mat0(k), m1 = mat1(k), vv = vecm(k);
        const float4* __restrict__ P = reinterpret_cast<const float4*>(S.plane[k]);
        const float4* __restrict__ Ln = reinterpret_cast<const float4*>(S.line[k]);
        const unsigned jr = (unsigned)min(amn[vv] + (l15 & (WS - 1)), gs[vv] - 1);
        bv[k] = Ln[jr * 4u + (unsigned)lq];
#pragma unroll
        for (int mb = 0; mb < NB; ++mb) {
            const int t = mb * 16 + l15;
            const unsigned yy = (unsigned)min(amn[m1] + (t >> LOG2W), gs[m1] - 1), xx = (unsigned)min(amn[m0] + (t & (WS - 1)), gs[m0] - 1);
            av[k][mb] = P[(__umul24(yy, (unsigned)gs[m0]) + xx) * 4u + (unsigned)lq];
        }
    }
#pragma unroll
    for (int k = 0; k < 3; ++k) {
        float* __restrict__ Dk = stD + kSumFloats + k * 16 * ST + l15 * ST + lq * 4;
#pragma unroll
        for (int mb = 0; mb < NB; ++mb) {
            f32x4_t d = {0.f, 0.f, 0.f, 0.f};
            d = __builtin_amdgcn_mfma_f32_16x16x4f32(av[k][mb].x, bv[k].x, d, 0, 0, 0);
            d = __builtin_amdgcn_mfma_f32_16x16x4f32(av[k][mb].y, bv[k].y, d, 0, 0, 0);
            d = __builtin_amdgcn_mfma_f32_16x16x4f32(av[k][mb].z, bv[k].z, d, 0, 0, 0);
            d = __builtin_amdgcn_mfma_f32_16x16x4f32(av[k][mb].w, bv[k].w, d, 0, 0, 0);
            *reinterpret_cast<float4*>(Dk + mb * 16) = make_float4(d[0], d[1], d[2], d[3]);
        }
    }
}
template <int LOG2W>
__device__ __forceinline__ void table_sum(float* __restrict__ stD, int lane) {
    static_assert(LOG2W == 2, "the summed table is one entry per lane: 4 taps per axis");
    constexpr int ST = (1 << (2 * LOG2W)) + 4;
    const unsigned x = (unsigned)lane & 3u, y = ((unsigned)lane >> 2) & 3u, z = (unsigned)lane >> 4;
    const float* __restrict__ D = stD + kSumFloats;
    const float d0 = D[__umul24(z, (unsigned)ST) + ((unsigned)lane & 15u)];
    const float d1 = D[16 * ST + __umul24(y, (unsigned)ST) + (z << 2 | x)];
    const float d2 = D[32 * ST + __umul24(x, (unsigned)ST) + (z << 2 | y)];
    stD[lane] = (d0 + d1) + d2;
}
__device__ __forceinline__ float table_read3(const Axes3& A, int org, const float* __restrict__ stS) {
    const Axis& ax = A.a[0];
    const Axis& ay = A.a[1];
    const Axis& az = A.a[2];
    const float* __restrict__ D = stS + (((az.i0 << 4) + ((ay.i0 << 2) + ax.i0)) - org);
    const float wnw = ay.w0 * ax.w0, wne = ay.w0 * ax.w1, wsw = ay.w1 * ax.w0, wse = ay.w1 * ax.w1;
    float v0 = D[0] * wnw, v1 = D[16] * wnw;
    v0 = fmaf(D[1], wne, v0); v1 = fmaf(D[17], wne, v1);
    v0 = fmaf(D[4], wsw, v0); v1 = fmaf(D[20], wsw, v1);
    v0 = fmaf(D[5], wse, v0); v1 = fmaf(D[21], wse, v1);
    return fmaf(v1, az.w1, v0 * az.w0);
}

struct __attribute__((aligned(4))) F2U { float a, b; };
struct CellTaps { F2U d00, d01, d10, d11; };
__device__ __forceinline__ unsigned cached_offset(const FieldDev& F, const Axes3& A) {
    return umad24(umad24((unsigned)A.a[2].i0, (unsigned)F.den.H[0] + 1u, (unsigned)A.a[1].i0), F.ds_row, (unsigned)A.a[0].i0 << 2);
}
__device__ __forceinline__ CellTaps cached_load(const FieldDev& F, unsigned off) {
    const char* __restrict__ B = reinterpret_cast<const char*>(F.dsum);
    CellTaps t;
    t.d00 = *reinterpret_cast<const F2U*>(B + off);
    t.d01 = *reinterpret_cast<const F2U*>(B + (off + F.ds_row));
    t.d10 = *reinterpret_cast<const F2U*>(B + (off + F.ds_slice));
    t.d11 = *reinterpret_cast<const F2U*>(B + (off + F.ds_slice + F.ds_row));
    return t;
}
__device__ __forceinline__ float cached_read3(const Axes3& A, const CellTaps& t) {
    const Axis& ax = A.a[0];
    const Axis& ay = A.a[1];
    const Axis& az = A.a[2];
    const float wnw = ay.w0 * ax.w0, wne = ay.w0 * ax.w1, wsw = ay.w1 * ax.w0, wse = ay.w1 * ax.w1;
    float v0 = t.d00.a * wnw, v1 = t.d10.a * wnw;
    v0 = fmaf(t.d00.b, wne, v0); v1 = fmaf(t.d10.b, wne, v1);
    v0 = fmaf(t.d01.a, wsw, v0); v1 = fmaf(t.d11.a, wsw, v1);
    v0 = fmaf(t.d01.b, wse, v0); v1 = fmaf(t.d11.b, wse, v1);
    return fmaf(v1, az.w1, v0 * az.w0);
}

template <int K>
__device__ __forceinline__ float pair_dot_global(const FactorSet& S, const Axes3& A, float part) {
    const Axis& ax = A.a[mat0(K)];
    const Axis& ay = A.a[mat1(K)];
    const Axis& al = A.a[vecm(K)];
    const float4* __restrict__ P = reinterpret_cast<const float4*>(S.plane[K]);
    const float4* __restrict__ L = reinterpret_cast<const float4*>(S.line[K]);
    const unsigned W = (unsigned)S.W[K];
    const unsigned nw = ((unsigned)ay.i0 * W + ax.i0) * 4, ne = ((unsigned)ay.i0 * W + ax.i1) * 4;
    const unsigned sw = ((unsigned)ay.i1 * W + ax.i0) * 4, se = ((unsigned)ay.i1 * W + ax.i1) * 4;
#pragma unroll 1
    for (int q = 0; q < 4; ++q) {
        float4 v = f4_mul(P[nw + q], ay.w0 * ax.w0);
        v = f4_fma(P[ne + q], ay.w0 * ax.w1, v);
        v = f4_fma(P[sw + q], ay.w1 * ax.w0, v);
        v = f4_fma(P[se + q], ay.w1 * ax.w1, v);
        float4 l = f4_mul(L[al.i0 * 4 + q], al.w0);
        l = f4_fma(L[al.i1 * 4 + q], al.w1, l);
        part = fmaf(v.x, l.x, part); part = fmaf(v.y, l.y, part); part = fmaf(v.z, l.z, part); part = fmaf(v.w, l.w, part);
    }
    return part;
}

__device__ __forceinline__ void void_entries(float4* __restrict__ app_pos, int* __restrict__ app_ray, unsigned list, unsigned list_cap,
                                             unsigned lo, unsigned hi, int lane) {
    if (hi > list_cap) hi = list_cap;
    for (unsigned e = lo + (unsigned)lane; e < hi; e += 64u) {
        app_pos[(size_t)list * list_cap + e] = make_float4(0.f, 0.f, 0.f, 0.f);
        app_ray[(size_t)list * list_cap + e] = 0;
    }
}

__device__ __forceinline__ void slot_rows(const FieldDev& F, const float4* __restrict__ app_pos, float* __restrict__ feat, size_t slot,
                                          unsigned count, int lane) {
    if (!count) return;
    asm volatile("s_waitcnt vmcnt(0)" ::: "memory");
    const AvVolume vol{F.avol, F.av_row, F.av_slice, (unsigned)F.app.H[0] + 1u};
    av_slot_rows(F.app, vol, app_pos + slot, feat + slot * 32u, count, lane);
}

constexpr int kDenseLd = 20;
constexpr int kDenseFloats = 64 * kDenseLd;
struct __attribute__((aligned(4))) F4U { float x, y, z, w; };

#ifndef T2N_MT_WAVES
#define T2N_MT_WAVES 5
#endif
#ifndef T2N_MTD_WAVES
#define T2N_MTD_WAVES 4
#endif
#ifndef T2N_MTC_WAVES
#define T2N_MTC_WAVES 5
#endif
#ifndef T2N_MTCD_WAVES
#define T2N_MTCD_WAVES 4
#endif
#ifdef MT_PROF
#define MT_T(var) do { const unsigned long long tn = __builtin_readcyclecounter(); var += tn - p_t; p_t = tn; } while (0)
#else
#define MT_T(var) do {} while (0)
#endif
constexpr int mt_waves(bool dense, bool cached) { return cached ? (dense ? T2N_MTCD_WAVES : T2N_MTC_WAVES) : (dense ? T2N_MTD_WAVES : T2N_MT_WAVES); }
template <bool DENSE, bool ALPHA = false, bool RELU = false, bool CACHED = false, bool ROWS = false>
__global__ __launch_bounds__(256) __attribute__((amdgpu_waves_per_eu(mt_waves(DENSE, CACHED), mt_waves(DENSE, CACHED)))) void k_march_tiles(const TileArgs a) {
    extern __shared__ __attribute__((aligned(16))) float smem[];
    const int lane = threadIdx.x & 63, wid = threadIdx.x >> 6;
    const int l15 = lane & 15, lq = lane >> 4;
    float* __restrict__ stD = smem + (size_t)wid * kStageFloats;
    if constexpr (!CACHED) {
        for (int i = lane; i < kStageFloats; i += 64) stD[i] = 0.f;
        lds_fence_w();
    }
    float* __restrict__ wt = smem + (CACHED ? 0 : 4 * kStageFloats) + (size_t)wid * kDenseFloats;
    const FieldDev& F = a.F;
    const int tiles_x = (a.img_w + 7) >> 3;
    const long long tile = (long long)blockIdx.x * 4 + wid;
    const int ty = (int)(tile / tiles_x), tx = (int)(tile - (long long)ty * tiles_x);
    const int px = tx * 8 + (lane & 7), py = ty * 8 + (lane >> 3);
    if (ty * 8 >= a.img_h) return;
    const bool have = px < a.img_w && py < a.img_h;
    const long long r = have ? (long long)py * a.img_w + px : 0;
    const int N = a.n_samples;
    Ray ray;
    if (have) ray = load_ray(F, a.rays + r * a.ray_stride, a.ray_stride);
    else { ray.ox = ray.oy = ray.oz = 1e30f; ray.dx = ray.dy = ray.dz = 0.f; ray.tmin = 0.f; ray.last = 0.f; }
    int lo = N, hi = -1;
    if (have) ray_interval<false>(F, ray, N, lo, hi);
    const int wlo = wave_min_i(lo), whi = wave_max_i(hi);

    float T = 1.f, acc = 0.f, dep = 0.f;
    int first = -1, last = -1;
    unsigned napp = 0;
    int nev = 0;
    int ovf_from = 0;

    long long frow[4];
    if constexpr (DENSE) {
#pragma unroll
        for (int j = 0; j < 4; ++j) {
            const int rho = (lane >> 2) + 16 * j;
            const int fx = tx * 8 + (rho & 7), fy = ty * 8 + (rho >> 3);
            frow[j] = (fx < a.img_w && fy < a.img_h) ? ((long long)fy * a.img_w + fx) * N : -1;
        }
    }
    constexpr int kSteps = 2;
    const int i_begin = DENSE ? (wlo & ~15) : wlo, i_end = DENSE ? min(N - 1, whi | 15) : whi;
    const float eps = DENSE ? 0.f : F.term_eps;
    bool dead = false;
#ifdef MT_PROF
    unsigned long long p_coord = 0, p_axes = 0, p_build = 0, p_read = 0, p_act = 0, p_pairs = 0;
    const unsigned long long p_start = __builtin_readcyclecounter();
    unsigned long long p_t = p_start;
#endif
    for (int i = i_begin; i <= i_end; i += kSteps) {
        if (eps > 0.f && (((i - i_begin) & 15) == 0)) {
            dead = T < eps;
            if (!__any(have && i <= hi && !dead)) break;
        }
        float xn[kSteps], yn[kSteps], zn[kSteps], z[kSteps], w_out[kSteps];
        bool ok[kSteps];
        Axes3 A[kSteps];
        bool any_ok = false;
#pragma unroll
        for (int q = 0; q < kSteps; ++q) {
            const int idx = i + q;
            xn[q] = yn[q] = zn[q] = z[q] = w_out[q] = 0.f;
            ok[q] = false;
            if (have && idx >= lo && idx <= hi && idx <= i_end && !dead) {
                z[q] = sample_z<false, true>(F, ray, idx, 0.f);
                ok[q] = sample_point<false>(F, ray, z[q], xn[q], yn[q], zn[q]);
                if constexpr (ALPHA) { if (ok[q]) ok[q] = alpha_pass(F, ray, z[q]); }
            }
            any_ok |= ok[q];
        }
        const unsigned long long okm = __ballot(any_ok);
        MT_T(p_coord);
        if (!DENSE && !okm && !__any(have && napp >= (unsigned)a.cap)) continue;
        float part[kSteps];
#pragma unroll
        for (int q = 0; q < kSteps; ++q) part[q] = 0.f;
        if (okm) {
#pragma unroll
            for (int q = 0; q < kSteps; ++q) A[q] = sample_axes_inbox(F.den, xn[q], yn[q], zn[q]);
            int sel0 = 0, sel1 = 0, sel2 = 0;
#pragma unroll
            for (int q = kSteps - 1; q >= 0; --q)
                if (ok[q]) { sel0 = A[q].a[0].i0; sel1 = A[q].a[1].i0; sel2 = A[q].a[2].i0; }
            const int lead = (int)__builtin_ctzll(okm);
            const int ref0 = __builtin_amdgcn_readlane(sel0, lead), ref1 = __builtin_amdgcn_readlane(sel1, lead),
                      ref2 = __builtin_amdgcn_readlane(sel2, lead);
            unsigned bits = 0u;
#pragma unroll
            for (int q = 0; q < kSteps; ++q)
                if (ok[q]) {
                    const unsigned d0 = (unsigned)(A[q].a[0].i0 - ref0 + 5), d1 = (unsigned)(A[q].a[1].i0 - ref1 + 5),
                                   d2 = (unsigned)(A[q].a[2].i0 - ref2 + 5);
                    bits |= (d0 < 10u ? 1u << d0 : 0x40000000u) | (d1 < 10u ? 1u << (10u + d1) : 0x40000000u) |
                            (d2 < 10u ? 1u << (20u + d2) : 0x40000000u);
                }
            bits = wave_or_u(bits);
            const unsigned f0 = bits & 1023u, f1 = (bits >> 10) & 1023u, f2 = (bits >> 20) & 1023u;
            const int amn[3] = {ref0 - 5 + __builtin_ctz(f0), ref1 - 5 + __builtin_ctz(f1), ref2 - 5 + __builtin_ctz(f2)};
            const int span = max(max(32 - __builtin_clz(f0) - __builtin_ctz(f0), 32 - __builtin_clz(f1) - __builtin_ctz(f1)),
                                 32 - __builtin_clz(f2) - __builtin_ctz(f2)) + 1;
            const bool ranged = !(bits & 0x40000000u);
            MT_T(p_axes);
            if (CACHED && ranged && span <= 4) {
                unsigned off[kSteps];
                CellTaps ct[kSteps];
#pragma unroll
                for (int q = 0; q < kSteps; ++q) off[q] = ok[q] ? cached_offset(F, A[q]) : 0u;
#pragma unroll
                for (int q = 0; q < kSteps; ++q) ct[q] = cached_load(F, off[q]);
                MT_T(p_build);
#pragma unroll
                for (int q = 0; q < kSteps; ++q)
                    if (ok[q]) part[q] = cached_read3(A[q], ct[q]);
                MT_T(p_read);
            } else if (ranged && span <= 4) {
                table_build<2>(F.den, amn, stD, l15, lq);
                lds_fence_w();
                {
                    int ln = lane;
                    asm volatile("" : "+v"(ln));
                    table_sum<2>(stD, ln);
                }
                lds_fence_w();
                MT_T(p_build);
                int org = (amn[2] << 4) + (amn[1] << 2) + amn[0];
                asm volatile("" : "+s"(org));
#pragma unroll
                for (int q = 0; q < kSteps; ++q)
                    if (ok[q]) part[q] = table_read3(A[q], org, stD);
                lds_fence_w();
                MT_T(p_read);
            } else {
#pragma unroll
                for (int q = 0; q < kSteps; ++q)
                    if (ok[q]) {
                        float pq = pair_dot_global<0>(F.den, A[q], 0.f);
                        pq = pair_dot_global<1>(F.den, A[q], pq);
                        part[q] = pair_dot_global<2>(F.den, A[q], pq);
                    }
            }
        }
#pragma unroll
        for (int q = 0; q < kSteps; ++q) {
            const int idx = i + q;
            const bool spill = have && idx <= i_end && napp >= (unsigned)a.cap && !DENSE;
            if (ok[q]) {
                const float sg = feature2density<RELU ? T2N_ACT_RELU : T2N_ACT_SOFTPLUS>(F, part[q]);
                const float dist = idx < N - 1 ? sample_z<false, true>(F, ray, idx + 1, 0.f) - z[q] : 0.f;
                const float alpha = 1.f - exp_finite((-sg) * (dist * F.dscale));
                const float w = alpha * T;
                T = T * ((1.f - alpha) + 1e-10f);
                acc += w;
                dep = fmaf(w, z[q], dep);
                if (w > F.thres) {
                    if (napp < (unsigned)a.cap) a.scratch[(size_t)r * a.cap + napp] = make_float4(xn[q], yn[q], zn[q], w);
                    ++napp;
                    if (napp == (unsigned)a.cap) ovf_from = idx + 1;
                }
                if (first < 0) first = idx;
                last = idx;
                ++nev;
                w_out[q] = w;
            }
            if (spill) a.wbuf[r * N + idx] = w_out[q];
            if constexpr (DENSE) {
                if (idx < N) {
                    const int c16 = idx & 15;
                    wt[lane * kDenseLd + c16] = w_out[q];
                }
                if ((idx < N && (idx & 15) == 15) || idx == N - 1) {
                    lds_fence_w();
                    const int col = (idx & ~15) + 4 * (lane & 3);
#pragma unroll
                    for (int j = 0; j < 4; ++j) {
                        if (frow[j] < 0 || col >= N) continue;
                        const int rho = (lane >> 2) + 16 * j;
                        const float4 vw = *reinterpret_cast<const float4*>(wt + rho * kDenseLd + 4 * (lane & 3));
                        if (col + 3 < N) {
                            *reinterpret_cast<F4U*>(a.dense_w + frow[j] + col) = F4U{vw.x, vw.y, vw.z, vw.w};
                        } else {
                            const float ew[4] = {vw.x, vw.y, vw.z, vw.w};
#pragma unroll
                            for (int e = 0; e < 4; ++e)
                                if (col + e < N) a.dense_w[frow[j] + col + e] = ew[e];
                        }
                    }
                    lds_fence_w();
                }
            }
        }
#ifdef MT_PROF
        MT_T(p_act); ++p_pairs;
#endif
    }
#ifdef MT_PROF
    if (lane == 0 && a.prof) {
        unsigned long long* o = a.prof + (size_t)(blockIdx.x * 4 + wid) * 8;
        o[0] = p_coord; o[1] = p_axes; o[2] = p_build; o[3] = p_read; o[4] = p_act; o[5] = p_pairs; o[6] = __builtin_readcyclecounter() - p_start;
    }
#endif
    const int Lw = last >= first && first >= 0 ? last - first + 1 : 0;
    if (have) {
        a.acc[r] = acc;
        a.depth[r] = dep + (1.f - acc) * ray.last;
    }
    const bool over = have && napp > (unsigned)a.cap;
    const unsigned n = (have && !over) ? napp : 0u;
    unsigned incl = n;
#pragma unroll
    for (int o = 1; o < 64; o <<= 1) {
        const unsigned t = __shfl_up(incl, o);
        if (lane >= o) incl += t;
    }
    const unsigned total = __shfl(incl, 63);
    const unsigned list = blockIdx.x & 7u;
    unsigned base = 0;
    if (lane == 0 && total) base = atomicAdd(&a.counters[list * kCounterStride], total);
    base = __shfl(base, 0);
    const bool fits = base + total <= a.list_cap;
    if (!fits && total) void_entries(a.app_pos, a.app_ray, list, a.list_cap, base, base + total, lane);
    const unsigned slot0 = list * a.list_cap + base + (incl - n);
    if (have) {
        if (over || !fits) {
            const unsigned k = atomicAdd(a.ovf_count, 1u);
            a.ovf_list[k] = (int)r;
            a.ray_app[r] = make_int4(ovf_from, (int)napp, nev, Lw > 0 ? (first | (Lw << 11)) : 0);
        } else {
            a.ray_app[r] = make_int4((int)slot0, fits ? (int)n : 0, nev, Lw > 0 ? (first | (Lw << 11)) : 0);
            if (fits) {
                const float4* __restrict__ src = a.scratch + (size_t)r * a.cap;
                for (unsigned k = 0; k < n; k += 4) {
                    const float4 e0 = src[k], e1 = src[k + 1 < n ? k + 1 : n - 1], e2 = src[k + 2 < n ? k + 2 : n - 1],
                                 e3 = src[k + 3 < n ? k + 3 : n - 1];
                    a.app_pos[slot0 + k] = e0; a.app_ray[slot0 + k] = (int)r;
                    if (k + 1 < n) { a.app_pos[slot0 + k + 1] = e1; a.app_ray[slot0 + k + 1] = (int)r; }
                    if (k + 2 < n) { a.app_pos[slot0 + k + 2] = e2; a.app_ray[slot0 + k + 2] = (int)r; }
                    if (k + 3 < n) { a.app_pos[slot0 + k + 3] = e3; a.app_ray[slot0 + k + 3] = (int)r; }
                }
            }
        }
    }
    if constexpr (ROWS) {
        static_assert(CACHED && !DENSE, "rows in the tail: cached, weight-free frames only");
#ifndef T2N_MT_NO_TAIL_ROWS
        const unsigned ubase = (unsigned)__builtin_amdgcn_readfirstlane((int)base), utotal = (unsigned)__builtin_amdgcn_readfirstlane((int)total);
        unsigned cnt = utotal;
        if (ubase + utotal > a.list_cap) cnt = ubase < a.list_cap ? a.list_cap - ubase : 0u;
        slot_rows(F, a.app_pos, a.feat, (size_t)list * a.list_cap + ubase, cnt, lane);
#endif
    }
}

struct CompactArgs {
    FieldDev F;
    const float* rays; long long n_rays; int ray_stride; int n_samples;
    const float* wbuf;
    int4* ray_app; float4* app_pos; int* app_ray; unsigned* counters; unsigned list_cap;
    unsigned long long* stats;
    const float4* scratch; int cap;
    int finisher;
    float* feat;
};
__device__ __forceinline__ void reserve_slots(const CompactArgs& a, long long r, unsigned list, int lane, const int4 ra, unsigned& slot0,
                                              unsigned& napp, int* ovf_slot) {
    slot0 = 0;
    napp = (unsigned)__builtin_amdgcn_readfirstlane((int)napp);
    bool fits = napp == 0;
    for (unsigned att = 0; att < (unsigned)kLists && !fits; ++att) {
        const unsigned l = (list + att) & (unsigned)(kLists - 1);
        unsigned s0 = 0xffffffffu;
        if (lane == 0 && a.counters[l * kCounterStride] + napp <= a.list_cap) s0 = atomicAdd(&a.counters[l * kCounterStride], napp);
        s0 = (unsigned)__builtin_amdgcn_readfirstlane((int)s0);
        if (s0 == 0xffffffffu) continue;
        if (s0 + napp <= a.list_cap) { slot0 = l * a.list_cap + s0; fits = true; }
        else if (s0 < a.list_cap) {
            void_entries(a.app_pos, a.app_ray, l, a.list_cap, s0, a.list_cap, lane);
            if (a.feat) slot_rows(a.F, a.app_pos, a.feat, (size_t)l * a.list_cap + s0, a.list_cap - s0, lane);
        }
    }
    if (lane == 0) {
        if (fits || !a.finisher) a.ray_app[r] = make_int4((int)slot0, fits ? (int)napp : 0, ra.z, ra.w);
        else {
            a.ray_app[r] = make_int4(-ra.x - 1, (int)napp, ra.z, ra.w);
            *ovf_slot = (int)((unsigned)r | 0x80000000u);
            atomicAdd(&a.counters[kFailEntriesWord], napp);
        }
        if (!fits && !a.finisher && a.stats) a.stats[T2N_STAT_OVERFLOW] = 1ull;
        if (!fits) a.counters[kOverflowWord] = 1u;
    }
    if (!fits) napp = 0;
}
__device__ __forceinline__ void compact_span(const CompactArgs& a, long long r, const Ray& ray, int from, int end, unsigned slot0, unsigned run,
                                             int lane) {
    const FieldDev& F = a.F;
    const int N = a.n_samples;
    for (int base = from; base < end; base += 64) {
        const int i = base + lane;
        const float w = i < end ? a.wbuf[r * N + i] : 0.f;
        const bool m = (i < end) & (w > F.thres);
        const unsigned long long bal = __ballot(m);
        if (m) {
            const unsigned pre = (unsigned)__popcll(bal & ((1ull << lane) - 1ull));
            const float z = sample_z<false>(F, ray, i, 0.f);
            float xn, yn, zn;
            sample_point<false>(F, ray, z, xn, yn, zn);
            const unsigned s = slot0 + run + pre;
            a.app_pos[s] = make_float4(xn, yn, zn, w);
            a.app_ray[s] = (int)r;
        }
        run += (unsigned)__popcll(bal);
    }
}
__device__ __forceinline__ void compact_ray_staged(const CompactArgs& a, long long r, unsigned list, int lane, int* ovf_slot) {
    const int4 ra = a.ray_app[r];
    const int first = ra.w & 2047, Lw = ra.w >> 11, from = ra.x;
    unsigned napp = (unsigned)ra.y, slot0;
    reserve_slots(a, r, list, lane, ra, slot0, napp, ovf_slot);
    const unsigned staged = napp < (unsigned)a.cap ? napp : (unsigned)a.cap;
    for (unsigned k = (unsigned)lane; k < staged; k += 64u) {
        a.app_pos[slot0 + k] = a.scratch[(size_t)r * a.cap + k];
        a.app_ray[slot0 + k] = (int)r;
    }
    if (napp > staged) {
        const Ray ray = load_ray(a.F, a.rays + r * a.ray_stride, a.ray_stride);
        compact_span(a, r, ray, from, first + Lw, slot0, staged, lane);
    }
    if (a.feat) slot_rows(a.F, a.app_pos, a.feat, (size_t)slot0, napp, lane);
}
__global__ __launch_bounds__(256) void k_compact_list(const CompactArgs a, const unsigned* ovf_count, int* ovf_list) {
    const int lane = threadIdx.x & 63;
    const unsigned n = *ovf_count;
    for (unsigned k = blockIdx.x * 4u + (threadIdx.x >> 6); k < n; k += gridDim.x * 4u)
        compact_ray_staged(a, ovf_list[k], blockIdx.x & 7u, lane, ovf_list + k);
}

__global__ __launch_bounds__(256) void k_dense_fill(const FieldDev F, const float* __restrict__ rays, long long n_rays, int ray_stride, int N,
                                                    float* __restrict__ w, float* __restrict__ z) {
    const int lane = threadIdx.x & 63;
    const long long r = (long long)blockIdx.x * 4 + (threadIdx.x >> 6);
    if (r >= n_rays) return;
    Ray ray;
    if (z) ray = load_ray(F, rays + r * ray_stride, ray_stride);
    for (int i = lane; i < N; i += 64) {
        if (z) z[r * N + i] = sample_z<false>(F, ray, i, 0.f);
        if (w) w[r * N + i] = 0.f;
    }
}

struct SumTableArgs { FactorSet den; float* out; int n[3]; int nb[3]; int shift[3]; long long boxes; };
__global__ __launch_bounds__(256) void k_density_sum_table(const SumTableArgs a) {
    __shared__ __attribute__((aligned(16))) float smem[4 * kStageFloats];
    const int lane = threadIdx.x & 63, wid = threadIdx.x >> 6;
    const long long box = (long long)blockIdx.x * 4 + wid;
    if (box >= a.boxes) return;
    float* __restrict__ stD = smem + (size_t)wid * kStageFloats;
    const int bx = (int)(box % a.nb[0]), by = (int)((box / a.nb[0]) % a.nb[1]), bz = (int)(box / ((long long)a.nb[0] * a.nb[1]));
    const int o[3] = {4 * bx - a.shift[0], 4 * by - a.shift[1], 4 * bz - a.shift[2]};
    const int amn[3] = {max(o[0], 0), max(o[1], 0), max(o[2], 0)};
    table_build<2>(a.den, amn, stD, lane & 15, lane >> 4);
    lds_fence_w();
    table_sum<2>(stD, lane);
    lds_fence_w();
    const int x = amn[0] + (lane & 3), y = amn[1] + ((lane >> 2) & 3), z = amn[2] + (lane >> 4);
    if (x < o[0] + 4 && y < o[1] + 4 && z < o[2] + 4 && x <= a.n[0] && y <= a.n[1] && z <= a.n[2])
        a.out[((size_t)z * (a.n[1] + 1) + y) * (a.n[0] + 1) + x] = stD[lane];
}

size_t density_cache_bytes(const t2n_field* f) {
    const int* g = f->desc.grid;
    return (size_t)(g[0] + 1) * (g[1] + 1) * (g[2] + 1) * sizeof(float);
}

int launch_density_sum_table(const t2n_field* f, float* out, const int shift[3], hipStream_t s) {
    SumTableArgs a;
    a.den = f->dev.den; a.out = out;
    a.boxes = 1;
    for (int k = 0; k < 3; ++k) {
        if (shift[k] < 0 || shift[k] > 3) { set_error("density sum table: shift[%d]=%d outside [0, 3]", k, shift[k]); return T2N_ERR_INVALID; }
        a.n[k] = f->desc.grid[k]; a.shift[k] = shift[k];
        a.nb[k] = (a.n[k] + shift[k]) / 4 + 1;
        a.boxes *= a.nb[k];
    }
    hipLaunchKernelGGL(k_density_sum_table, dim3((unsigned)((a.boxes + 3) / 4)), dim3(256), 0, s, a);
    T2N_HIP(hipGetLastError());
    return T2N_OK;
}

void density_cache_release(t2n_field* f) {
    if (f->dcache) { (void)hipDeviceSynchronize(); (void)hipFree(f->dcache); }
    f->dcache = nullptr; f->dcache_bytes = 0; f->dcache_version = 0; f->dcache_seen = 0; f->dcache_alloc_failed = false;
    f->dev.dsum = nullptr;
}

int density_cache_prepare(t2n_field* f, hipStream_t s) {
    f->dev.dsum = nullptr;
    const bool second = f->dcache_seen == f->den_version;
    f->dcache_seen = f->den_version;
    if (!f->dcache_on) return T2N_OK;
    const int* g = f->desc.grid;
    const size_t bytes = density_cache_bytes(f);
    size_t cap = f->dcache_cap;
    if (!cap) {
        static size_t dev_total = 0;
        if (!dev_total) { size_t fr = 0, tot = 0; if (hipMemGetInfo(&fr, &tot) == hipSuccess) dev_total = tot; else (void)hipGetLastError(); }
        cap = dev_total / 64;
    }
    const bool addressable = (size_t)(g[1] + 1) * (g[2] + 1) < (1u << 24) && bytes < (1ull << 32);
    if ((size_t)g[0] * g[1] * g[2] * sizeof(float) > cap || !addressable) return T2N_OK;
    if (f->dcache && f->dcache_version == f->den_version) {
        if (f->dcache_stream != (void*)s) T2N_HIP(hipStreamWaitEvent(s, (hipEvent_t)f->dcache_ev, 0));
    } else {
        if (!second) return T2N_OK;
        if (!f->dcache) {
            if (f->dcache_alloc_failed) return T2N_OK;
            if (hipMalloc((void**)&f->dcache, bytes + 16) != hipSuccess) {
                (void)hipGetLastError();
                f->dcache = nullptr; f->dcache_alloc_failed = true;
                return T2N_OK;
            }
            f->dcache_bytes = bytes + 16;
        }
        if (!f->dcache_ev) T2N_HIP(hipEventCreateWithFlags((hipEvent_t*)&f->dcache_ev, hipEventDisableTiming));
        const int shift[3] = {0, 0, 0};
        const int rc = launch_density_sum_table(f, f->dcache, shift, s);
        if (rc) return rc;
        T2N_HIP(hipEventRecord((hipEvent_t)f->dcache_ev, s));
        f->dcache_stream = (void*)s;
        f->dcache_version = f->den_version;
        ++f->dcache_counts[2];
    }
    f->dev.dsum = f->dcache;
    f->dev.ds_row = (unsigned)(g[0] + 1) * 4u;
    f->dev.ds_slice = f->dev.ds_row * (unsigned)(g[1] + 1);
    return T2N_OK;
}

int launch_march_tiles(t2n_field* f, const RenderLaunch& L, int img_w, int img_h, float* spill, float4* scratch, hipStream_t s) {
    const int cap = L.n_samples / 4 > 0 ? L.n_samples / 4 : 1;
    unsigned* ovf_count = (unsigned*)((char*)scratch + (size_t)L.n_rays * cap * 16);
    int* ovf_list = (int*)((char*)ovf_count + 256);
    const bool dense = L.weights != nullptr;
    TileArgs a;
    a.F = f->dev;
    a.rays = L.rays; a.n_rays = L.n_rays; a.ray_stride = L.ray_stride; a.n_samples = L.n_samples; a.img_w = img_w; a.img_h = img_h;
    a.acc = L.acc; a.depth = L.depth; a.ray_app = L.ray_app;
    a.wbuf = L.weights ? L.weights : spill;
    a.scratch = scratch; a.cap = cap; a.ovf_count = ovf_count; a.ovf_list = ovf_list;
    a.app_pos = L.app_pos; a.app_ray = L.app_ray; a.counters = L.counters; a.list_cap = L.list_cap; a.stats = (unsigned long long*)L.stats;
    a.dense_w = L.weights;
    const bool rows = L.slot_rows && f->dev.dsum != nullptr && f->dev.avol != nullptr && !dense && !f->dev.alpha;
    if (L.slot_rows && !rows) { set_error("launch_march_tiles: a fused frame needs the cached table, the feature volume, no mask and no weights rows"); return T2N_ERR_STATE; }
    a.feat = rows ? L.feat : nullptr;
    ++f->fusion_counts[rows ? 0 : 1];
    a.F.term_eps = (!L.weights && !L.z_vals && !L.sigma_ctx) ? f->term_eps : 0.f;
#ifdef MT_PROF
    static unsigned long long* prof = nullptr;
    static int prof_calls = 0;
    const long long prof_waves = ((long long)((img_w + 7) / 8) * ((img_h + 7) / 8) + 3) / 4 * 4;
    if (!prof) T2N_HIP(hipMalloc((void**)&prof, (size_t)65536 * 8 * 8));
    T2N_HIP(hipMemsetAsync(prof, 0, (size_t)65536 * 8 * 8, s));
    a.prof = prof_waves <= 65536 ? prof : nullptr;
#endif
    const long long tiles = (long long)((img_w + 7) / 8) * ((img_h + 7) / 8);
    const dim3 grid((unsigned)((tiles + 3) / 4));
    timing_begin(f, T2N_K_MARCH, s);
    if (L.weights || L.z_vals)
        hipLaunchKernelGGL(k_dense_fill, dim3((unsigned)((L.n_rays + 3) / 4)), dim3(256), 0, s, f->dev, L.rays, (long long)L.n_rays, L.ray_stride,
                           L.n_samples, L.weights, L.z_vals);
    const bool cached = f->dev.dsum != nullptr;
    const size_t lds = (size_t)4 * ((cached ? 0 : kStageFloats) + (dense ? kDenseFloats : 0)) * sizeof(float);
    const bool mask = f->dev.alpha != nullptr, relu = f->dev.act == T2N_ACT_RELU;
    ++f->dcache_counts[cached ? 0 : 1];
#define T2N_MT_LAUNCH(D, A, R) do { if (rows) hipLaunchKernelGGL((k_march_tiles<D, A, R, true, !D && !A>), grid, dim3(256), lds, s, a); \
                                    else if (cached) hipLaunchKernelGGL((k_march_tiles<D, A, R, true>), grid, dim3(256), lds, s, a); \
                                    else hipLaunchKernelGGL((k_march_tiles<D, A, R, false>), grid, dim3(256), lds, s, a); } while (0)
    if (dense) { if (mask) { if (relu) T2N_MT_LAUNCH(true, true, true); else T2N_MT_LAUNCH(true, true, false); }
                 else { if (relu) T2N_MT_LAUNCH(true, false, true); else T2N_MT_LAUNCH(true, false, false); } }
    else { if (mask) { if (relu) T2N_MT_LAUNCH(false, true, true); else T2N_MT_LAUNCH(false, true, false); }
           else { if (relu) T2N_MT_LAUNCH(false, false, true); else T2N_MT_LAUNCH(false, false, false); } }
#undef T2N_MT_LAUNCH
    T2N_HIP(hipGetLastError());
#ifdef MT_PROF
    if (a.prof && ++prof_calls == 20) {
        static unsigned long long h[65536 * 8];
        T2N_HIP(hipStreamSynchronize(s));
        T2N_HIP(hipMemcpy(h, prof, sizeof(h), hipMemcpyDeviceToHost));
        double sum[8] = {0, 0, 0, 0, 0, 0, 0, 0};
        long long n = 0;
        for (long long i = 0; i < prof_waves; ++i) if (h[i * 8 + 5]) { ++n; for (int k = 0; k < 8; ++k) sum[k] += (double)h[i * 8 + k]; }
        if (n) fprintf(stderr, "[mt prof] %lld waves, per wave: step pairs %.1f, cycles in the step loop %.0f = coordinates + validity %.0f, axis taps + union bit set %.0f, "
                               "table build (loads -> MFMA -> LDS) %.0f, table reads %.0f, activation + compositing + staging %.0f; per step pair %.0f\n",
                       n, sum[5] / n, (sum[0] + sum[1] + sum[2] + sum[3] + sum[4]) / n, sum[0] / n, sum[1] / n, sum[2] / n, sum[3] / n, sum[4] / n,
                       (sum[0] + sum[1] + sum[2] + sum[3] + sum[4]) / (sum[5] > 0 ? sum[5] : 1));
    }
#endif
    CompactArgs c;
    c.F = f->dev;
    c.rays = L.rays; c.n_rays = L.n_rays; c.ray_stride = L.ray_stride; c.n_samples = L.n_samples;
    c.wbuf = a.wbuf;
    c.ray_app = L.ray_app; c.app_pos = L.app_pos; c.app_ray = L.app_ray; c.counters = L.counters; c.list_cap = L.list_cap;
    c.stats = (unsigned long long*)L.stats;
    c.scratch = scratch; c.cap = cap;
    c.finisher = finish_supported(f) ? 1 : 0;
    c.feat = a.feat;
    hipLaunchKernelGGL(k_compact_list, dim3(64), dim3(256), 0, s, c, (const unsigned*)ovf_count, ovf_list);
    timing_end(f, T2N_K_MARCH, s);
    T2N_HIP(hipGetLastError());
    return launch_ray_stats(L, s);
}

}
```

text2nerf_amd/tensorf.py:

```python
from __future__ import annotations

import ctypes as C
import math
import os
import weakref
import time
from typing import Optional

import numpy as np
import torch
import torch.nn as nn

from . import _lib
from ._lib import FLAG_ADD_BG, FLAG_COHERENT, FLAG_DEVICE_ROWS, FLAG_KEEP_CTX, FLAG_NDC, FLAG_TRAIN, T2NError

MAT_MODE = [[0, 1], [0, 2], [1, 2]]
VEC_MODE = [2, 1, 0]

_SEED_MIN_RAYS = 8192
_WORKSPACE = {}


def _distortion_weight(w) -> float:
    w = float(w)
# ... 184 lines not shown
def workspace_budget(device=None) -> int:
    env = os.environ.get("T2N_WORKSPACE_GIB")
    if env is not None:
        return int(float(env) * (1 << 30))
    total = torch.cuda.get_device_properties(device).total_memory if device is not None and torch.cuda.is_available() else 64 << 30
    return int(min(32 << 30, total // 8))


def raw2alpha(sigma: torch.Tensor, dist: torch.Tensor):
    lib = _lib.load()
    sigma = sigma.contiguous().float()
    dist = dist.contiguous().float()
    R, N = sigma.shape
    alpha = torch.empty_like(sigma)
    w = torch.empty_like(sigma)
    bg = torch.empty(R, 1, device=sigma.device, dtype=torch.float32)
    _lib.check(lib.t2n_raw2alpha(_lib.ptr(sigma), _lib.ptr(dist), R, N, _lib.ptr(alpha), _lib.ptr(w), _lib.ptr(bg),
                                 _lib.current_stream_ptr(sigma.device)), "t2n_raw2alpha")
    return alpha, w, bg


def positional_encoding(positions, freqs):
    if positions.device.type != "cuda":
        raise T2NError("positional_encoding: the mirror computes on the MI355X only")
    octaves = torch.pow(2.0, torch.arange(freqs, device=positions.device, dtype=torch.float32))
    arg = (positions.unsqueeze(-1) * octaves).flatten(-2)
    return torch.cat([arg.sin(), arg.cos()], dim=-1)


def SHRender(xyz_sampled, viewdirs, features):
    from .sh import eval_sh_bases
    basis = eval_sh_bases(2, viewdirs)
    coeff = features.reshape(-1, 3, basis.shape[-1])
    return torch.relu((coeff * basis[:, None]).sum(-1) + 0.5)


def RGBRender(xyz_sampled, viewdirs, features):
    return features


class AlphaGridMask(nn.Module):

    def __init__(self, device, aabb, alpha_volume):
        super().__init__()
        self.device = device
        self.aabb = torch.as_tensor(aabb, dtype=torch.float32).to(device)
        self.aabbSize = self.aabb[1] - self.aabb[0]
        self.invgridSize = 1.0 / self.aabbSize * 2
        self.alpha_volume = alpha_volume.view(1, 1, *alpha_volume.shape[-3:]).float().to(device)
        self.gridSize = torch.LongTensor([alpha_volume.shape[-1], alpha_volume.shape[-2], alpha_volume.shape[-3]]).to(device)
        object.__setattr__(self, "_field", None)

    def normalize_coord(self, xyz_sampled):
        return (xyz_sampled - self.aabb[0]) * self.invgridSize - 1

    def sample_alpha(self, xyz_sampled):
        if self._field is None:
            raise T2NError("AlphaGridMask.sample_alpha needs the mask to be attached to a TensorVMSplit (tensorf.alphaMask = mask)")
        return self._field._alpha_at(xyz_sampled)


class MLPRender_Fea_noview(nn.Module):

    def __init__(self, inChanel, feape=6, featureC=128):
        super().__init__()
        self.in_mlpC = 2 * feape * inChanel + inChanel
        self.feape = feape
        l0, l1, l2 = nn.Linear(self.in_mlpC, featureC), nn.Linear(featureC, featureC), nn.Linear(featureC, 3)
        self.mlp = nn.Sequential(l0, nn.ReLU(inplace=True), l1, nn.ReLU(inplace=True), l2)
        nn.init.constant_(self.mlp[-1].bias, 0)

    def forward(self, pts, viewdirs, features):
        raise T2NError("MLPRender_Fea_noview runs fused inside TensorVMSplit's HIP shade kernel; call "
                       "TensorVMSplit.shade(xyz_norm) / forward(rays) instead")


class _ViewHead(nn.Module):

    def _build(self, in_mlpC, featureC):
        self.in_mlpC = in_mlpC
        l0, l1, l2 = nn.Linear(in_mlpC, featureC), nn.Linear(featureC, featureC), nn.Linear(featureC, 3)
        self.mlp = nn.Sequential(l0, nn.ReLU(inplace=True), l1, nn.ReLU(inplace=True), l2)
        nn.init.constant_(self.mlp[-1].bias, 0)

    def forward(self, pts, viewdirs, features):
        raise T2NError(f"{type(self).__name__} runs inside TensorVMSplit's HIP render call; use TensorVMSplit.forward(rays)")


class MLPRender_Fea(_ViewHead):

    def __init__(self, inChanel, viewpe=6, feape=6, featureC=128):
        super().__init__()
        self.viewpe, self.feape = viewpe, feape
        self._build(2 * viewpe * 3 + 2 * feape * inChanel + 3 + inChanel, featureC)


class MLPRender_PE(_ViewHead):

    def __init__(self, inChanel, viewpe=6, pospe=6, featureC=128):
        super().__init__()
        self.viewpe, self.pospe = viewpe, pospe
        self._build((3 + 2 * viewpe * 3) + (3 + 2 * pospe * 3) + inChanel, featureC)


class MLPRender(_ViewHead):

    def __init__(self, inChanel, viewpe=6, featureC=128):
        super().__init__()
        self.viewpe = viewpe
        self._build((3 + 2 * viewpe * 3) + inChanel, featureC)


class TensorBase(nn.Module):

    def __init__(self, aabb, gridSize, device, density_n_comp=8, appearance_n_comp=24, app_dim=27,
                 shadingMode="MLP_PE", alphaMask=None, near_far=[2.0, 6.0], density_shift=-10, alphaMask_thres=0.001,
                 distance_scale=25, rayMarch_weight_thres=0.0001, pos_pe=6, view_pe=6, fea_pe=6, featureC=128,
                 step_ratio=2.0, fea2denseAct="softplus"):
        super().__init__()
        if isinstance(density_n_comp, int):
            density_n_comp = [density_n_comp] * 3
        if isinstance(appearance_n_comp, int):
            appearance_n_comp = [appearance_n_comp] * 3
        self.density_n_comp = list(density_n_comp)
        self.app_n_comp = list(appearance_n_comp)
        self.app_dim = app_dim
        self.aabb = torch.as_tensor(aabb, dtype=torch.float32).to(device)
        self.alphaMask = alphaMask
        self.device = device
        self.density_shift = density_shift
        self.alphaMask_thres = alphaMask_thres
        self.distance_scale = distance_scale
        self.rayMarch_weight_thres = rayMarch_weight_thres
        self.fea2denseAct = fea2denseAct
        self.near_far = near_far
        self.step_ratio = step_ratio
        self.matMode, self.vecMode, self.comp_w = MAT_MODE, VEC_MODE, [1, 1, 1]
        self.shadingMode, self.pos_pe, self.view_pe, self.fea_pe, self.featureC = shadingMode, pos_pe, view_pe, fea_pe, featureC
        self.keep_activation_rows = True
        self.defer_factor_grads = False
        self.materialize_weights = True
        self.z_gate = 2.0
        self.frame_width = 0
        self.mlp_exact_fp32 = False
        self.feature_stage_shape = (0, 0)
        self.feature_staging = True
        self.factor_storage = "fp32"
        self.density_cache = True
        self.density_cache_cap_bytes = 0
        self.appearance_volume = True
        self.appearance_volume_min_frames = 0
        self.appearance_volume_cap_bytes = 0
        self.feature_fusion = True
        self.early_termination = 0.0
        self._handle = None
        self._uploaded_key = None
        self._gbuf = None
        self._gbuf_dirty = False
        self._gbuf_stale = False
        self.last_stats = None
        self._dcache_base = [0, 0, 0]
        _FIELDS.add(self)

        if shadingMode not in _lib.SHADE_IDS:
            raise T2NError(f"shadingMode {shadingMode!r} is not implemented by the HIP renderer "
                           f"(supported: {sorted(_lib.SHADE_IDS)})")
        self.update_stepSize(gridSize)
        self.init_svd_volume(gridSize[0], device)
        self.init_render_func(shadingMode, pos_pe, view_pe, fea_pe, featureC, device)
        self._is_general()

    def init_render_func(self, shadingMode, pos_pe, view_pe, fea_pe, featureC, device):
        if shadingMode == "MLP_Fea_noview":
            self.renderModule = MLPRender_Fea_noview(self.app_dim, fea_pe, featureC).to(device)
        elif shadingMode == "MLP_PE":
            raise T2NError("shadingMode 'MLP_PE': the reference's MLPRender_PE sizes its first layer for 3 inputs it never "
                           "concatenates (models/tensorBase.py:115 vs :126-131) and fails with a shape error for every "
                           "pos_pe / view_pe; there is no behaviour to reproduce")
        elif shadingMode == "MLP_Fea":
            self.renderModule = MLPRender_Fea(self.app_dim, view_pe, fea_pe, featureC).to(device)
        elif shadingMode == "MLP":
            self.renderModule = MLPRender(self.app_dim, view_pe, featureC).to(device)
        elif shadingMode == "SH":
            self.renderModule = SHRender
        elif shadingMode == "RGB":
            assert self.app_dim == 3
            self.renderModule = RGBRender
        else:
            raise T2NError(f"Unrecognized shading module {shadingMode!r}")

    def _sample(self, rays_o, rays_d, N, jitter, ndc):
        lib = _lib.load()
        h = self.sync_params()
        dev = self.basis_mat.weight.device if hasattr(self, "basis_mat") else self._all_params()[0].device
        o = rays_o.detach().reshape(-1, 3).contiguous().float().to(dev)
        d = rays_d.detach().reshape(-1, 3).contiguous().float().to(dev)
        n = o.shape[0]
        pts = torch.empty(n, N, 3, device=dev, dtype=torch.float32)
        z = None if ndc else torch.empty(n, N, device=dev, dtype=torch.float32)
        valid = torch.empty(n, N, device=dev, dtype=torch.uint8)
        with torch.cuda.device(dev):
            _lib.check(lib.t2n_sample_ray(h, _lib.ptr(o), _lib.ptr(d), n, int(N), _lib.ptr(jitter), 1 if ndc else 0, _lib.ptr(pts),
                                          _lib.ptr(z), _lib.ptr(valid), _lib.current_stream_ptr(dev)), "t2n_sample_ray")
        return pts, z, valid.bool()

    def sample_ray(self, rays_o, rays_d, is_train=True, N_samples=-1):
        N = int(N_samples) if N_samples > 0 else self.nSamples
        jitter = None
        if is_train:
            jitter = to_device_async(torch.rand(rays_d.reshape(-1, 3).shape[0], 1), self._all_params()[0].device).reshape(-1).contiguous()
        pts, z, valid = self._sample(rays_o, rays_d, N, jitter, False)
        lead = tuple(rays_o.shape[:-1])
        return pts.reshape(lead + (N, 3)), z.reshape(lead + (N,)), valid.reshape(lead + (N,))

    def sample_ray_ndc(self, rays_o, rays_d, is_train=True, N_samples=-1):
        N = int(N_samples) if N_samples > 0 else self.nSamples
        near, far = self.near_far
        dev = self._all_params()[0].device
        interpx = torch.linspace(near, far, N).unsqueeze(0).to(rays_o)
        if is_train:
            interpx += torch.rand_like(interpx).to(rays_o) * ((far - near) / N)
        table = interpx.to(dev).reshape(-1).contiguous().float()
        pts, _, valid = self._sample(rays_o, rays_d, N, table, True)
        lead = tuple(rays_o.shape[:-1])
        return pts.reshape(lead + (N, 3)), interpx, valid.reshape(lead + (N,))

    def update_stepSize(self, gridSize):
        aabb = self.aabb.detach().float().cpu()
        size = aabb[1] - aabb[0]
        grid = torch.LongTensor([int(x) for x in gridSize])
        units = size / (grid - 1)
        step = torch.mean(units) * self.step_ratio
        diag = torch.sqrt(torch.sum(torch.square(size)))
        self.aabbSize = size.to(self.device)
        self.invaabbSize = (2.0 / size).to(self.device)
        self.gridSize = grid.to(self.device)
        self.units = units.to(self.device)
        self.stepSize = step.to(self.device)
        self.aabbDiag = diag.to(self.device)
        self.nSamples = int((diag / step).item()) + 1
        if self._handle is not None:
            lib = _lib.load()
            d = self._desc()
            _lib.check(lib.t2n_field_set_desc(self._handle, C.byref(d)), "t2n_field_set_desc")

    def get_kwargs(self):
        return {"aabb": self.aabb, "gridSize": self.gridSize.tolist(), "density_n_comp": self.density_n_comp,
                "appearance_n_comp": self.app_n_comp, "app_dim": self.app_dim, "density_shift": self.density_shift,
                "alphaMask_thres": self.alphaMask_thres, "distance_scale": self.distance_scale,
                "rayMarch_weight_thres": self.rayMarch_weight_thres, "fea2denseAct": self.fea2denseAct,
                "near_far": self.near_far, "step_ratio": self.step_ratio, "shadingMode": self.shadingMode,
                "pos_pe": self.pos_pe, "view_pe": self.view_pe, "fea_pe": self.fea_pe, "featureC": self.featureC}

    def state_dict(self, *a, **k):
        sd = super().state_dict(*a, **k)
        return type(sd)((key, v) for key, v in sd.items() if not key.startswith("alphaMask."))

    def save(self, path):
        ckpt = {"kwargs": self.get_kwargs(), "state_dict": self.state_dict()}
        if self.alphaMask is not None:
            vol = self.alphaMask.alpha_volume.bool().cpu().numpy()
            ckpt.update({"alphaMask.shape": vol.shape})
            ckpt.update({"alphaMask.mask": np.packbits(vol.reshape(-1))})
            ckpt.update({"alphaMask.aabb": self.alphaMask.aabb.cpu()})
        torch.save(ckpt, path)

    def load(self, ckpt):
        if "alphaMask.aabb" in ckpt.keys():
            length = int(np.prod(ckpt["alphaMask.shape"]))
            vol = torch.from_numpy(np.unpackbits(ckpt["alphaMask.mask"])[:length].reshape(ckpt["alphaMask.shape"]))
            self.alphaMask = AlphaGridMask(self.device, ckpt["alphaMask.aabb"].to(self.device), vol.float().to(self.device))
        self.load_state_dict(ckpt["state_dict"], strict=False)

    def _desc(self) -> _lib.FieldDesc:
        d = _lib.FieldDesc()
        a = self.aabb.detach().float().cpu()
        inv = self.invaabbSize.detach().float().cpu()
        for k in range(3):
            d.aabb_min[k], d.aabb_max[k], d.inv_aabb_size[k] = float(a[0, k]), float(a[1, k]), float(inv[k])
            d.grid[k] = int(self.gridSize[k])
        kd, ka, kdim, kpe, kfc = self._kernel_shape()
        d.density_n_comp, d.app_n_comp, d.app_dim = kd, ka, kdim
        d.shading = _lib.SHADE_IDS[self.shadingMode]
        d.fea_pe, d.feature_c = kpe, kfc
        d.act = _lib.ACT_IDS[self.fea2denseAct]
        d.density_shift, d.distance_scale = float(self.density_shift), float(self.distance_scale)
        d.weight_thres = float(self.rayMarch_weight_thres)
        d.step_size = float(self.stepSize)
        d.near, d.far = float(self.near_far[0]), float(self.near_far[1])
        d.z_gate = float(self.z_gate)
        d.view_pe, d.pos_pe = int(self.view_pe), int(self.pos_pe)
        return d

    KERNEL_DEN, KERNEL_APP, KERNEL_DIM, KERNEL_PE, KERNEL_FC = 16, 48, 27, 6, 128

    GENERAL_DIM, GENERAL_FC, GENERAL_PE = 64, 256, 16

    def _is_general(self):
        flag = self.__dict__.get("_general_flag")
        if flag is None:
            wide_head = False
            if isinstance(self.renderModule, nn.Module):
                wide_head = self.featureC > self.KERNEL_FC
                if self.shadingMode == "MLP_Fea_noview":
                    wide_head = wide_head or self.app_dim > self.KERNEL_DIM or self.fea_pe > self.KERNEL_PE
                else:
# ... 97 lines not shown
        return self._embedded_params() if self._needs_embed() else self._real_params()

    def _autograd_params(self):
        return self._all_params()

    def _kernel_views(self, tensors):
        return list(tensors)

    def _param_struct(self, tensors, cls=_lib.FieldParams):
        s = cls()
        t = [None if x is None else x.data_ptr() for x in tensors]
        for k in range(3):
            s.density_plane[k] = t[k]
            s.density_line[k] = t[3 + k]
            s.app_plane[k] = t[6 + k]
            s.app_line[k] = t[9 + k]
        s.basis_weight = t[12]
        if len(t) > 13:
            s.mlp_w0, s.mlp_b0, s.mlp_w1, s.mlp_b1, s.mlp_w2, s.mlp_b2 = t[13:19]
        return s

    def supports_deferred_factor_grads(self):
        return type(self)._kernel_views is TensorVMSplit._kernel_views and type(self)._autograd_params is TensorVMSplit._autograd_params \
            and self.factor_storage == "fp32" and not self._needs_embed() and not self._is_general()

    def factor_grad_buffer(self, _raw=False):
        if getattr(self, "_gbuf", None) is not None:
            if getattr(self, "_gbuf_stale", False) and not _raw:
                self._drop_preseed()
                self._gbuf.zero_()
                self._gbuf_stale = False
                self._gbuf_dirty = False
            return self._gbuf
        h = self.sync_params()
        if getattr(self, "_gbuf", None) is None:
            lib = _lib.load()
            dev = self.basis_mat.weight.device
            n = int(lib.t2n_field_grad_buffer_bytes(h))
            self._gbuf = torch.zeros(n // 4, device=dev, dtype=torch.float32)
            _lib.check(lib.t2n_field_set_grad_buffer(h, _lib.ptr(self._gbuf), n), "t2n_field_set_grad_buffer")
            self._gbuf_dirty = False
            self._gbuf_stale = False
        return self._gbuf

    def zero_factor_grads(self, lazy=False):
        have = getattr(self, "_gbuf", None) is not None
        if lazy and have and self._gbuf_dirty:
            self._gbuf_stale = True
        else:
            self._drop_preseed()
            if have and self._gbuf_dirty:
                self._gbuf.zero_()
            self._gbuf_stale = False
            self._gbuf_dirty = False
        self._gbuf_reduced = False
        self._deferred_grad_key = None

    def _drop_preseed(self):
        pre = self.__dict__.get("_gbuf_preseed")
        if pre is not None:
            torch.cuda.current_stream(self.basis_mat.weight.device).wait_event(pre[3])
            self.__dict__["_gbuf_preseed"] = None

    def _tv_weights(self, tv):
        tv_d = tv_a = 0.0
        for planes, weight in tv:
            if planes is self.density_plane:
                tv_d = float(weight) * 1e-2
            elif planes is self.app_plane:
                tv_a = float(weight) * 1e-2
            else:
                raise T2NError("train_step: tv entries must be tensorf.density_plane / tensorf.app_plane")
        return tv_d, tv_a

    def _reg_weights(self, l1, ortho):
        l1_p = l1_l = o_d = o_a = 0.0
        for group, weight in l1:
            if group is self.density_plane:
                l1_p = float(weight)
            elif group is self.density_line:
                l1_l = float(weight)
            else:
                raise T2NError("l1 entries must be tensorf.density_plane / tensorf.density_line")
        for group, weight in ortho:
            if group is self.density_line:
                o_d = float(weight)
            elif group is self.app_line:
                o_a = float(weight)
            else:
                raise T2NError("ortho entries must be tensorf.density_line / tensorf.app_line")
        return l1_p, l1_l, o_d, o_a

    def _factor_key(self):
        return tuple((p.data_ptr(), p._version) for p in self._all_params()[:12])

    def seed_factor_grads_with_tv(self, tv, ahead=False, l1=(), ortho=()):
        lib = _lib.load()
        tv_d, tv_a = self._tv_weights(tv)
        reg = self._reg_weights(l1, ortho)
        dev = self.basis_mat.weight.device
        pre = self.__dict__.get("_gbuf_preseed")
        if not ahead and pre is not None and getattr(self, "_gbuf_stale", False) and pre[:2] == (tv_d, tv_a) and pre[2] == self._factor_key() \
                and pre[4] == reg:
            self.__dict__["_gbuf_preseed"] = None
            self._gbuf_stale = False
            self._gbuf_dirty = True
            self._gbuf_reduced = False
            return pre[3]
        h = self.sync_params()
        self.factor_grad_buffer(_raw=True)
        cur = torch.cuda.current_stream(dev)
        side = self.__dict__.get("_seed_stream")
        if side is None:
            side = self.__dict__["_seed_stream"] = torch.cuda.Stream(device=dev)
        side.wait_stream(cur)
        with torch.cuda.device(dev):
            if any(reg):
                _lib.check(lib.t2n_field_reg_seed(h, tv_d, tv_a, *reg, side.cuda_stream), "t2n_field_reg_seed")
            else:
                _lib.check(lib.t2n_field_tv_seed(h, tv_d, tv_a, side.cuda_stream), "t2n_field_tv_seed")
        ev = side.record_event()
        self._gbuf_dirty = True
        self._gbuf_reduced = False
        if ahead:
            self._gbuf_stale = True
            self.__dict__["_gbuf_preseed"] = (tv_d, tv_a, self._factor_key(), ev, reg)
        else:
            self._gbuf_stale = False
            self.__dict__["_gbuf_preseed"] = None
        return ev

    def sync_params(self, force=False, frame_width=None):
        lib = _lib.load()
        ps = self._all_params()
        dev = ps[0].device
        if dev.type != "cuda":
            raise T2NError(f"TensorVMSplit parameters live on {dev}; the renderer runs on an MI355X (cuda/HIP) only")
        for p in ps:
            if p.dtype != torch.float32 or not p.is_contiguous():
                raise T2NError("parameters must be contiguous float32")
        if self._handle is None:
            h = C.c_void_p()
            d = self._desc()
            _lib.check(lib.t2n_field_create(C.byref(d), C.byref(h)), "t2n_field_create")
            self._handle = h
            self._precision_set = None
            self._term_set = None
            self._storage_set = None
            self._frame_w_set = None
            self._staging_set = None
            self._dcache_set = (True, 0)
            self._avol_set = (True, 0, 0)
            self._fusion_set = True
            self._stage_shape_set = (0, 0)
            self._head_rows_set = 32
            self._alpha_key = "unset"
        queued = False
        mask = self.alphaMask
        mkey = None if mask is None else (mask.alpha_volume.data_ptr(), mask.alpha_volume._version, tuple(mask.alpha_volume.shape))
        if getattr(self, "_alpha_key", "unset") != mkey:
            queued = True
            self._wait_readers(dev)
            with torch.cuda.device(dev):
                if mask is None:
                    _lib.check(lib.t2n_field_set_alpha_mask(self._handle, None, 0, 0, 0, None, None, _lib.current_stream_ptr(dev)),
                               "t2n_field_set_alpha_mask")
                else:
                    vol = mask.alpha_volume.reshape(mask.alpha_volume.shape[-3:]).contiguous().float().to(dev)
                    amin = (C.c_float * 3)(*mask.aabb[0].float().cpu().tolist())
                    ainv = (C.c_float * 3)(*mask.invgridSize.float().cpu().tolist())
                    D, H, W = vol.shape
                    _lib.check(lib.t2n_field_set_alpha_mask(self._handle, _lib.ptr(vol), D, H, W, amin, ainv,
                                                            _lib.current_stream_ptr(dev)), "t2n_field_set_alpha_mask")
                    object.__setattr__(mask, "_field", self)
            self._alpha_key = mkey
        hr = int(getattr(self, "head_scratch_rows_per_ray", 32))
        if getattr(self, "_head_rows_set", 32) != hr:
            _lib.check(lib.t2n_field_set_head_scratch_rows(self._handle, hr), "t2n_field_set_head_scratch_rows")
            self._head_rows_set = hr
        fw = int(self.frame_width if frame_width is None else frame_width)
        if getattr(self, "_frame_w_set", None) != fw:
            _lib.check(lib.t2n_field_set_frame_width(self._handle, fw), "t2n_field_set_frame_width")
            self._frame_w_set = fw
        if self._precision_set != bool(self.mlp_exact_fp32):
            _lib.check(lib.t2n_field_set_mlp_precision(self._handle, 1 if self.mlp_exact_fp32 else 0),
                       "t2n_field_set_mlp_precision")
            self._precision_set = bool(self.mlp_exact_fp32)
        if getattr(self, "_staging_set", None) != bool(self.feature_staging):
            _lib.check(lib.t2n_field_set_feature_staging(self._handle, 1 if self.feature_staging else 0),
                       "t2n_field_set_feature_staging")
            self._staging_set = bool(self.feature_staging)
        dc = (bool(getattr(self, "density_cache", True)), int(getattr(self, "density_cache_cap_bytes", 0)))
        if getattr(self, "_dcache_set", (True, 0)) != dc:
            _lib.check(lib.t2n_field_set_density_cache(self._handle, 1 if dc[0] else 0), "t2n_field_set_density_cache")
            _lib.check(lib.t2n_field_set_density_cache_cap(self._handle, dc[1]), "t2n_field_set_density_cache_cap")
            self._dcache_set = dc
        av = (bool(getattr(self, "appearance_volume", True)), int(getattr(self, "appearance_volume_min_frames", 0)),
              int(getattr(self, "appearance_volume_cap_bytes", 0)))
        if getattr(self, "_avol_set", (True, 0, 0)) != av:
            _lib.check(lib.t2n_field_set_appearance_volume(self._handle, 1 if av[0] else 0, av[1]), "t2n_field_set_appearance_volume")
            _lib.check(lib.t2n_field_set_appearance_volume_cap(self._handle, av[2]), "t2n_field_set_appearance_volume_cap")
            self._avol_set = av
        fu = bool(getattr(self, "feature_fusion", True))
        if getattr(self, "_fusion_set", True) != fu:
            _lib.check(lib.t2n_field_set_feature_fusion(self._handle, 1 if fu else 0), "t2n_field_set_feature_fusion")
            self._fusion_set = fu
        shape = tuple(int(v) for v in self.feature_stage_shape)
        if getattr(self, "_stage_shape_set", (0, 0)) != shape:
            _lib.check(lib.t2n_field_set_feature_stage_shape(self._handle, shape[0], shape[1]), "t2n_field_set_feature_stage_shape")
            self._stage_shape_set = shape
        et = max(0.0, min(float(self.early_termination or 0.0), float(self.rayMarch_weight_thres)))
        if getattr(self, "_term_set", None) != et:
            _lib.check(lib.t2n_field_set_early_termination(self._handle, et), "t2n_field_set_early_termination")
            self._term_set = et
        if self.factor_storage not in ("fp32", "bf16"):
            raise T2NError(f"factor_storage {self.factor_storage!r}: expected 'fp32' or 'bf16'")
        if getattr(self, "_storage_set", None) != self.factor_storage:
            _lib.check(lib.t2n_field_set_factor_storage(self._handle, 1 if self.factor_storage == "bf16" else 0),
                       "t2n_field_set_factor_storage")
            self._storage_set = self.factor_storage
            force = True
        key = tuple((p.data_ptr(), p._version) for p in ps)
        if force or key != self._uploaded_key:
            self._wait_readers(dev)
            with torch.cuda.device(dev):
                st = self._param_struct([p.detach() for p in ps])
                if not force and self._uploaded_key is not None and key[:12] == getattr(self, "_device_factor_key", None):
                    _lib.check(lib.t2n_field_upload_head(self._handle, C.byref(st), _lib.current_stream_ptr(dev)),
                               "t2n_field_upload_head")
                else:
                    _lib.check(lib.t2n_field_upload(self._handle, C.byref(st), _lib.current_stream_ptr(dev)),
                               "t2n_field_upload")
            self._uploaded_key = key
            self._device_factor_key = key[:12]
            queued = True
        cur = torch.cuda.current_stream(dev)
        if queued:
            ev = torch.cuda.Event()
            ev.record(cur)
            self._upload_event, self._upload_seen, self._upload_stream = ev, {int(cur.cuda_stream)}, int(cur.cuda_stream)
        elif getattr(self, "_upload_event", None) is not None and int(cur.cuda_stream) not in self._upload_seen:
            cur.wait_event(self._upload_event)
            self._upload_seen.add(int(cur.cuda_stream))
        return self._handle

    def _wait_readers(self, dev):
        readers = self.__dict__.get("_reader_events")
        if readers:
            cur = torch.cuda.current_stream(dev)
            for sid, ev in readers.items():
                if sid != int(cur.cuda_stream):
                    cur.wait_event(ev)
            readers.clear()

    def _note_reader(self, dev):
        seen = getattr(self, "_upload_seen", None)
        cur = torch.cuda.current_stream(dev)
        sid = int(cur.cuda_stream)
        if seen is None or sid == getattr(self, "_upload_stream", sid):
            return
        ev = torch.cuda.Event()
        ev.record(cur)
        self.__dict__.setdefault("_reader_events", {})[sid] = ev

    def __del__(self):
        try:
            if getattr(self, "_handle", None) is not None:
                _lib.load().t2n_field_destroy(self._handle)
                self._handle = None
                self._device_rows_ovf_seen = self._device_rows_issued = 0
        except Exception:
            pass

    def timing(self, on=True, kernels=None):
        mode = 1 if on else 0
        if on and kernels is not None:
            mode = sum(1 << (_lib.KERNEL_NAMES.index(k) + 1) for k in kernels)
        _lib.check(_lib.load().t2n_timing_enable(self.sync_params(), mode), "t2n_timing_enable")

    def read_timing(self, reset=True):
        ms = (C.c_double * _lib.T2N_K_COUNT)()
        n = (C.c_int64 * _lib.T2N_K_COUNT)()
        _lib.check(_lib.load().t2n_timing_read(self.sync_params(), ms, n, 1 if reset else 0), "t2n_timing_read")
        return {_lib.KERNEL_NAMES[k]: (ms[k], n[k]) for k in range(_lib.T2N_K_COUNT) if n[k]}

    def normalize_coord(self, xyz_sampled):
        return (xyz_sampled - self.aabb[0]) * self.invaabbSize - 1

    def feature2density(self, density_features):
        if self.fea2denseAct == "softplus":
            return torch.nn.functional.softplus(density_features + self.density_shift)
        return torch.relu(density_features)

    def _density_at(self, xyz, want_sigma):
        lib = _lib.load()
        h = self.sync_params()
        xyz = xyz.detach().reshape(-1, 3).contiguous().float().to(self.basis_mat.weight.device)
        n = xyz.shape[0]
        out = torch.empty(n, device=xyz.device, dtype=torch.float32)
        with torch.cuda.device(xyz.device):
            _lib.check(lib.t2n_density_at(h, _lib.ptr(xyz), n, None if want_sigma else _lib.ptr(out),
                                          _lib.ptr(out) if want_sigma else None, _lib.current_stream_ptr(xyz.device)),
                       "t2n_density_at")
        return out

    def _alpha_at(self, xyz_world):
        lib = _lib.load()
        h = self.sync_params()
        dev = self.basis_mat.weight.device
        xyz = xyz_world.detach().reshape(-1, 3).contiguous().float().to(dev)
        out = torch.empty(xyz.shape[0], device=dev, dtype=torch.float32)
        with torch.cuda.device(dev):
            _lib.check(lib.t2n_alpha_at(h, _lib.ptr(xyz), xyz.shape[0], _lib.ptr(out), _lib.current_stream_ptr(dev)), "t2n_alpha_at")
        return out

    def compute_sigma(self, xyz_norm):
        return self._density_at(xyz_norm, want_sigma=True)

    def shade(self, xyz_norm, viewdirs=None, want_features=True, want_rgb=True):
        lib = _lib.load()
        h = self.sync_params()
        dev = self.basis_mat.weight.device
        xyz = xyz_norm.detach().reshape(-1, 3).contiguous().float().to(dev)
        n = xyz.shape[0]
        vd = None if viewdirs is None else viewdirs.detach().reshape(-1, 3).contiguous().float().to(dev)
        feat = torch.empty(n, self.app_dim, device=dev, dtype=torch.float32) if want_features else None
        rgb = torch.empty(n, 3, device=dev, dtype=torch.float32) if want_rgb else None
        ws = workspace(dev, 256)
        with torch.cuda.device(dev):
            _lib.check(lib.t2n_shade_at(h, _lib.ptr(xyz), _lib.ptr(vd), n, _lib.ptr(feat), _lib.ptr(rgb), _lib.ptr(ws),
                                        ws.numel(), _lib.current_stream_ptr(dev)), "t2n_shade_at")
        return feat, rgb

    @torch.no_grad()
    def filtering_rays(self, all_rays, all_rgbs, all_depth=None, N_samples=256, chunk=10240 * 5, bbox_only=False):
        if not bbox_only and self.alphaMask is None:
            raise T2NError("filtering_rays(bbox_only=False) needs an alphaMask (updateAlphaMask() or a checkpoint's)")
        lib = _lib.load()
        general = self._is_general()
        h = None if general else self.sync_params()
        d = self._general_desc() if general else None
        dev = self.basis_mat.weight.device
        tt = time.time()
        flat = all_rays.reshape(-1, all_rays.shape[-1])
        masks = []
        for idx in torch.split(torch.arange(flat.shape[0]), chunk):
            r = flat[idx].to(dev).contiguous().float()
            m = torch.empty(r.shape[0], dtype=torch.uint8, device=dev)
            with torch.cuda.device(dev):
                if general:
                    _lib.check(lib.t2n_generic_filter_rays(C.byref(d), _lib.ptr(r), r.shape[0], r.shape[1], int(N_samples),
                                                           1 if bbox_only else 0, _lib.ptr(m), _lib.current_stream_ptr(dev)),
                               "t2n_generic_filter_rays")
                elif bbox_only:
                    _lib.check(lib.t2n_filter_rays_bbox(h, _lib.ptr(r), r.shape[0], r.shape[1], _lib.ptr(m),
                                                        _lib.current_stream_ptr(dev)), "t2n_filter_rays_bbox")
                else:
                    _lib.check(lib.t2n_filter_rays_alpha(h, _lib.ptr(r), r.shape[0], r.shape[1], int(N_samples), _lib.ptr(m),
                                                         _lib.current_stream_ptr(dev)), "t2n_filter_rays_alpha")
# ... 475 lines not shown
                    _lib.check(lib.t2n_train_loss_ex(_lib.ptr(rgb), _lib.ptr(depth), _lib.ptr(w), _lib.ptr(z), _lib.ptr(rgb_t), _lib.ptr(dep_t), R, N,
                                                     float(w_depth), float(w_trans), float(delta), kind, float(depth_std), _lib.ptr(d_rgb),
                                                     _lib.ptr(d_depth), _lib.ptr(d_w), _lib.ptr(losses), _lib.ptr(aux), _lib.ptr(lws), lws.numel(),
                                                     _lib.current_stream_ptr(dev)), "t2n_train_loss_ex")
                self.__dict__["last_depth_aux"] = aux
            self._head_flat.zero_()
            views, off = [], 0
            for p in head:
                views.append(self._head_flat[off:off + p.numel()].view_as(p))
                off += p.numel()
            if seed_ev is not None:
                torch.cuda.current_stream(dev).wait_event(seed_ev)
            try:
                grads = self._backward_raw(rays, jitter, N, flags, ws, d_rgb, d_depth, d_w, head_grads=views, device_rows=device_rows)
            except T2NError as e:
                if not device_rows or "DEVICE_ROWS" not in str(e):
                    raise
                device_rows = False
                grads = self._backward_raw(rays, jitter, N, flags, ws, d_rgb, d_depth, d_w, head_grads=views, device_rows=False)
            if device_rows:
                self.device_rows_steps = getattr(self, "device_rows_steps", 0) + 1
                self._device_rows_issued = getattr(self, "_device_rows_issued", 0) + 1
            for p, g in zip(params, grads):
                p.grad = g
            if all_reduce is not None:
                all_reduce()
            _step_with_terms(optimizer, tv, l1, ortho)
            if seed_terms is not None:
                self.seed_factor_grads_with_tv(seed_terms[0], ahead=True, l1=seed_terms[1], ortho=seed_terms[2])
            if speculative:
                evs = self.__dict__.setdefault("_spec_events", [])
                ev = torch.cuda.Event()
                ev.record(torch.cuda.current_stream(dev))
                evs.append(ev)
                if len(evs) > 2:
                    evs.pop(0).synchronize()
        return losses

    def train_step_indexed(self, source, ids, optimizer, N_samples=-1, white_bg=True, w_depth=0.005, w_trans=1e3, delta=0.1,
                           tv=(), all_reduce=None, all_reduce_averages=True, speculative=False, fused=None, graph=None, depth_loss="mse",
                           depth_std=0.1, l1=(), ortho=(), distortion=0.0):
        from .dataset import check_ids
        ids = check_ids(ids, len(source))
        distortion = _distortion_weight(distortion)
        self.__dict__["last_depth_aux"] = None
        self.__dict__["last_distortion"] = None
        l1, ortho = _live_terms(l1), _live_terms(ortho)
        if l1 or ortho:
            _check_reg_route(optimizer, graph, all_reduce)
            if getattr(optimizer, "field", None) is self:
                self._reg_weights(l1, ortho)
        fuse = self._fused_step_for(optimizer, N_samples, white_bg, all_reduce, all_reduce_averages, speculative, fused, graph,
                                    _depth_kind(depth_loss), distortion)
        if fuse is not None:
            fs, N, flags, use_graph = fuse
            return fs.step_indexed(source, ids, N, flags, w_depth, w_trans, delta, tv, use_graph, all_reduce, l1=l1, ortho=ortho)
        rays, rgb_t, dep_t = source.rows(ids)
        return self.train_step(rays, rgb_t, dep_t, optimizer, N_samples=N_samples, white_bg=white_bg, w_depth=w_depth, w_trans=w_trans,
                               delta=delta, tv=tv, all_reduce=all_reduce, all_reduce_averages=all_reduce_averages, speculative=speculative,
                               fused=False if fused is None else fused, graph=graph, depth_loss=depth_loss, depth_std=depth_std, l1=l1, ortho=ortho,
                               distortion=distortion)

    def _fused_step_for(self, optimizer, N_samples, white_bg, all_reduce, all_reduce_averages, speculative, fused, graph, depth_kind=0,
                        distortion=0.0):
        if depth_kind != 0:
            if fused:
                raise T2NError("train_step(fused=True): the one-call step computes the \"mse\" depth term only; depth_loss=gnll / si_log / ssi "
                               "runs on the composed route (fused=None or False)")
            return None
        if distortion > 0:
            if fused or graph:
                raise T2NError(f"train_step({'fused' if fused else 'graph'}=True): the one-call step and its graph form have their loss folded "
                               "into the backward and carry no distortion term; distortion > 0 runs on the composed route (fused=None or "
                               "False, graph=None or False)")
            return None
        can_fuse = self._can_fuse_train_step(optimizer) and (all_reduce is None or all_reduce_averages) and not speculative
        if fused and not can_fuse:
            raise T2NError("train_step(fused=True): needs the tuned field shape with the MLP_Fea_noview head (split-f16 arithmetic), fp32 factor "
                           "storage, no alpha mask, optim.TVAdam(field=tensorf) and an averaging all_reduce")
        if not can_fuse or fused is False:
            return None
        from .trainer import FusedStep
        fs = self.__dict__.get("_fused_step")
        if fs is None or fs.opt is not optimizer:
            fs = self.__dict__["_fused_step"] = FusedStep(self, optimizer)
        N = int(N_samples) if N_samples > 0 else self.nSamples
        flags = FLAG_ADD_BG if (white_bg or bool(torch.rand((1,)) < 0.5)) else 0
        return fs, N, flags, bool(graph) and all_reduce is None

    def _can_fuse_train_step(self, optimizer):
        return (getattr(optimizer, "field", None) is self and self.supports_deferred_factor_grads() and self.shadingMode == "MLP_Fea_noview"
                and not self.mlp_exact_fp32 and self.alphaMask is None and int(self.app_dim) == 27 and int(self.fea_pe) == 6
                and int(self.featureC) == 128 and list(self.density_n_comp) == [16] * 3 and list(self.app_n_comp) == [48] * 3
                and (int(self.nSamples) <= 1024))

    def _poll_device_rows(self):
        if not getattr(self, "device_rows_steps", 0) or self._handle is None:
            return True
        rec = (C.c_uint32 * 10)()
        _lib.check(_lib.load().t2n_field_device_rows_record(self._handle, rec), "t2n_field_device_rows_record")
        if rec[9] < getattr(self, "_device_rows_issued", 0):
            self.device_rows_unanswered = getattr(self, "device_rows_unanswered", 0) + 1
        margin = getattr(self, "_device_rows_margin", 1.25)
        seen = getattr(self, "_device_rows_ovf_seen", 0)
        overflowed = rec[8] > seen
        if overflowed:
            self.device_rows_overflows = getattr(self, "device_rows_overflows", 0) + int(rec[8] - seen)
            self._device_rows_ovf_seen = int(rec[8])
            margin = min(2.0, margin * 1.25)
            self._device_rows_clean = 0
        else:
            self._device_rows_clean = getattr(self, "_device_rows_clean", 0) + 1
            if self._device_rows_clean >= 64:
                margin, self._device_rows_clean = max(1.25, margin / 1.1), 0
        self._device_rows_margin = margin
        need = max(rec[0:8])
        if need:
            self._ctx_rows_hint = (int(need * margin) + 95) // 32 * 32
        return not overflowed

    def stats(self):
        s = self.last_stats.cpu().tolist()
        if s[_lib.STAT_OVERFLOW]:
            raise T2NError("appearance list overflow — workspace sizing bug")
        return {"evaluated": s[_lib.STAT_EVALUATED], "appearance": s[_lib.STAT_APPEARANCE], "f16_redo": s[_lib.STAT_F16_REDO],
                "list_retry": s[_lib.STAT_LIST_RETRY]}

    def feature_staging_counts(self):
        if self._handle is None:
            return (0, 0)
        out = (C.c_uint64 * 2)()
        _lib.check(_lib.load().t2n_field_feature_staging_counts(self._handle, out), "t2n_field_feature_staging_counts")
        return (int(out[0]), int(out[1]))

    def density_cache_counts(self):
        base = self.__dict__.get("_dcache_base", [0, 0, 0])
        out = (C.c_uint64 * 4)()
        if self._handle is not None:
            _lib.check(_lib.load().t2n_field_density_cache_counts(self._handle, out), "t2n_field_density_cache_counts")
        return {"cached": base[0] + int(out[0]), "uncached": base[1] + int(out[1]), "builds": base[2] + int(out[2]), "bytes": int(out[3])}

    def appearance_volume_counts(self):
        out = (C.c_uint64 * 4)()
        if self._handle is not None:
            _lib.check(_lib.load().t2n_field_appearance_volume_counts(self._handle, out), "t2n_field_appearance_volume_counts")
        return {"bytes": int(out[0]), "builds": int(out[1]), "volume": int(out[2]), "direct": int(out[3])}

    def feature_fusion_counts(self):
        out = (C.c_uint64 * 2)()
        if self._handle is not None:
            _lib.check(_lib.load().t2n_field_feature_fusion_counts(self._handle, out), "t2n_field_feature_fusion_counts")
        return {"fused": int(out[0]), "unfused": int(out[1])}

    def density_sum_table(self, shift=(0, 0, 0)):
        h = self.sync_params()
        g = [int(v) for v in self.gridSize]
        dev = self._all_params()[0].device
        out = torch.empty((g[2] + 1, g[1] + 1, g[0] + 1), dtype=torch.float32, device=dev)
        sh = (C.c_int * 3)(*[int(v) for v in shift])
        with torch.cuda.device(dev):
            _lib.check(_lib.load().t2n_field_density_sum_table(h, sh, _lib.ptr(out), _lib.current_stream_ptr(dev)), "t2n_field_density_sum_table")
        return out


class TensorVMSplit(TensorBase):

    def __init__(self, aabb, gridSize, device, **kargs):
        super().__init__(aabb, gridSize, device, **kargs)

    def init_svd_volume(self, res, device):
        self.density_plane, self.density_line = self.init_one_svd(self.density_n_comp, self.gridSize, 0.1, device)
        self.app_plane, self.app_line = self.init_one_svd(self.app_n_comp, self.gridSize, 0.1, device)
        self.basis_mat = nn.Linear(sum(self.app_n_comp), self.app_dim, bias=False).to(device)

    def init_one_svd(self, n_component, gridSize, scale, device):
        planes, lines = [], []
        g = [int(x) for x in gridSize]
        for i in range(3):
            m0, m1 = MAT_MODE[i]
            planes.append(nn.Parameter(scale * torch.randn((1, n_component[i], g[m1], g[m0]))))
            lines.append(nn.Parameter(scale * torch.randn((1, n_component[i], g[VEC_MODE[i]], 1))))
        return nn.ParameterList(planes).to(device), nn.ParameterList(lines).to(device)

    def get_optparam_groups(self, lr_init_spatialxyz=0.02, lr_init_network=0.001):
        groups = [{"params": self.density_line, "lr": lr_init_spatialxyz},
                  {"params": self.density_plane, "lr": lr_init_spatialxyz},
                  {"params": self.app_line, "lr": lr_init_spatialxyz},
                  {"params": self.app_plane, "lr": lr_init_spatialxyz},
                  {"params": self.basis_mat.parameters(), "lr": lr_init_network}]
        if isinstance(self.renderModule, nn.Module):
            groups += [{"params": self.renderModule.parameters(), "lr": lr_init_network}]
        return groups

    def TV_loss_density(self, reg):
        from .losses import tv_planes
        fused = tv_planes(reg, list(self.density_plane), 1e-2)
        if fused is not None:
            return fused
        total = 0
        for p in self.density_plane:
            total = total + reg(p) * 1e-2
        return total

    def TV_loss_app(self, reg):
        from .losses import tv_planes
        fused = tv_planes(reg, list(self.app_plane), 1e-2)
        if fused is not None:
            return fused
        total = 0
        for p in self.app_plane:
            total = total + reg(p) * 1e-2
        return total

    def density_L1(self):
        from .losses import l1_terms
        fused = l1_terms([t for pair in zip(self.density_plane, self.density_line) for t in pair])
        if fused is not None:
            return fused
        total = 0
        for p, l in zip(self.density_plane, self.density_line):
            total = total + torch.mean(torch.abs(p)) + torch.mean(torch.abs(l))
        return total

    def reg_terms(self, l1=0.0, ortho=0.0):
        l1_list = [(self.density_plane, l1), (self.density_line, l1)] if l1 else []
        ortho_list = [(self.density_line, ortho), (self.app_line, ortho)] if ortho else []
        return l1_list, ortho_list

    def vectorDiffs(self, vector_comps):
        total = 0
        for v in vector_comps:
            n_comp, n_size = v.shape[1:-1]
            m = v.view(n_comp, n_size)
            dotp = m @ m.transpose(-1, -2)
            total = total + torch.mean(torch.abs(dotp.view(-1)[1:].view(n_comp - 1, n_comp + 1)[..., :-1]))
        return total

    def vector_comp_diffs(self):
        from .losses import ortho_terms
        fused = ortho_terms(list(self.density_line) + list(self.app_line))
        if fused is not None:
            return fused
        return self.vectorDiffs(self.density_line) + self.vectorDiffs(self.app_line)

    def compute_densityfeature(self, xyz_sampled):
        return self._density_at(xyz_sampled, want_sigma=False)

    def compute_appfeature(self, xyz_sampled):
        return self.shade(xyz_sampled, want_rgb=False)[0]

    @torch.no_grad()
    def up_sampling_VM(self, plane_coef, line_coef, res_target):
        lib = _lib.load()
        res = [int(x) for x in res_target]

        def resize(t, Hout, Wout):
            t = t.detach().contiguous().float()
            _, Cn, Hin, Win = t.shape
            out = torch.empty((1, Cn, Hout, Wout), device=t.device, dtype=torch.float32)
            with torch.cuda.device(t.device):
                _lib.check(lib.t2n_upsample_bilinear(_lib.ptr(t), Cn, Hin, Win, _lib.ptr(out), Hout, Wout,
                                                     _lib.current_stream_ptr(t.device)), "t2n_upsample_bilinear")
            return out

        for i in range(3):
            m0, m1 = MAT_MODE[i]
            plane_coef[i] = nn.Parameter(resize(plane_coef[i].data, res[m1], res[m0]))
            line_coef[i] = nn.Parameter(resize(line_coef[i].data, res[VEC_MODE[i]], 1))
        return plane_coef, line_coef

    @torch.no_grad()
    def upsample_volume_grid(self, res_target):
        self.app_plane, self.app_line = self.up_sampling_VM(self.app_plane, self.app_line, res_target)
        self.density_plane, self.density_line = self.up_sampling_VM(self.density_plane, self.density_line, res_target)
        self._drop_handle()
        self.update_stepSize(res_target)
        print(f"upsamping to {res_target}")

    @torch.no_grad()
    def _voxel_window(self, new_aabb):
        box = torch.as_tensor(new_aabb, dtype=torch.float32).to(self.aabb.device)
        origin, far = self.aabb[0], self.aabb[1]
        lo = torch.round(torch.round((box[0] - origin) / self.units)).long()
        hi = torch.minimum(torch.round((box[1] - origin) / self.units).long() + 1, self.gridSize)
        mask_on_this_grid = self.alphaMask is not None and bool(torch.all(self.alphaMask.gridSize.to(self.gridSize.device) == self.gridSize))
        if not mask_on_this_grid:
            steps = self.gridSize - 1
            f_lo, f_hi = lo / steps, (hi - 1) / steps
            box = torch.stack([(1 - f_lo) * origin + f_lo * far, (1 - f_hi) * origin + f_hi * far])
        return lo, hi, box

    def _adopt_window(self, lo, hi, box):
        self.aabb = box
        self._drop_handle()
        self.update_stepSize(tuple(int(n) for n in (hi - lo)))

    def shrink(self, new_aabb):
        lo, hi, box = self._voxel_window(new_aabb)

        def window(t, *axes):
            idx = [slice(None), slice(None)] + [slice(int(lo[a]), int(hi[a])) for a in axes]
            return nn.Parameter(t.data[tuple(idx)].contiguous())

        for i in range(3):
            m0, m1 = MAT_MODE[i]
            for planes, lines in ((self.density_plane, self.density_line), (self.app_plane, self.app_line)):
# ... 255 lines not shown
```

Baseline: 186.1 billion ray-samples/s.

## Stage appearance-volume corner boxes in LDS for fused feature-row writes

When marching a tile, each wave logs which 4x4x4 density cell box each emitting step pair falls in, using one record per step pair. In the fused rows tail it loads that box of appearance-volume corners into LDS once and interpolates the feature rows for all entries in that box from LDS rather than from global memory, with a prefetch touch of the next box. This targets redundant global gathers of neighbouring corners across rays in a tile, at the cost of extra LDS, per-box synchronisation, and a fallback to the direct path when the log overflows or a step lies outside a small box. Counters and an on/off toggle are exposed.

```diff
diff --git a/include/t2n.h b/include/t2n.h
--- a/include/t2n.h
+++ b/include/t2n.h
@@ -116,6 +116,8 @@
 int t2n_field_set_feature_fusion(t2n_field* f, int on);
 int t2n_field_feature_fusion_counts(const t2n_field* f, uint64_t out[2]);
 int t2n_render_list_shape(int64_t n_rays, int n_samples, int entries_per_ray, uint64_t out[6]);
+int t2n_field_set_row_staging(t2n_field* f, int on);
+int t2n_field_row_staging_counts(const t2n_field* f, uint64_t out[2]);
 int t2n_field_feature_rows(t2n_field* f, const float* app_pos, const uint32_t* counters, uint32_t list_cap, int volume, float* feat,
                            uint32_t feat_rows, t2n_stream stream);
 int t2n_field_set_feature_stage_shape(t2n_field* f, int workgroups, int defer_cap);
diff --git a/text2nerf_amd/_lib.py b/text2nerf_amd/_lib.py
--- a/text2nerf_amd/_lib.py
+++ b/text2nerf_amd/_lib.py
@@ -110,6 +110,8 @@
     "t2n_field_appearance_volume_counts": (C.c_int, [C.c_void_p, C.POINTER(C.c_uint64)]),
     "t2n_field_set_feature_fusion": (C.c_int, [C.c_void_p, C.c_int]),
     "t2n_field_feature_fusion_counts": (C.c_int, [C.c_void_p, C.POINTER(C.c_uint64)]),
+    "t2n_field_set_row_staging": (C.c_int, [C.c_void_p, C.c_int]),
+    "t2n_field_row_staging_counts": (C.c_int, [C.c_void_p, C.POINTER(C.c_uint64)]),
     "t2n_render_list_shape": (C.c_int, [C.c_int64, C.c_int, C.c_int, C.POINTER(C.c_uint64)]),
     "t2n_field_feature_rows": (C.c_int, [C.c_void_p, C.c_void_p, C.c_void_p, C.c_uint32, C.c_int, C.c_void_p, C.c_uint32, C.c_void_p]),
     "t2n_field_density_sum_table": (C.c_int, [C.c_void_p, C.POINTER(C.c_int), C.c_void_p, C.c_void_p]),
diff --git a/text2nerf_amd/csrc/t2n_api.hip b/text2nerf_amd/csrc/t2n_api.hip
--- a/text2nerf_amd/csrc/t2n_api.hip
+++ b/text2nerf_amd/csrc/t2n_api.hip
@@ -927,6 +927,21 @@
     out[0] = f->fusion_counts[0]; out[1] = f->fusion_counts[1];
     return T2N_OK;
 }
+extern "C" int t2n_field_set_row_staging(t2n_field* f, int on) {
+    if (!f) { set_error("t2n_field_set_row_staging: NULL field"); return T2N_ERR_INVALID; }
+    f->row_staging_on = on ? 1 : 0;
+    return T2N_OK;
+}
+extern "C" int t2n_field_row_staging_counts(const t2n_field* f, uint64_t out[2]) {
+    if (!f || !out) { set_error("t2n_field_row_staging_counts: NULL argument"); return T2N_ERR_INVALID; }
+    out[0] = out[1] = 0;
+    if (!f->rows_counters) return T2N_OK;
+    unsigned raw[kLists * kCounterStride];
+    T2N_HIP(hipStreamSynchronize((hipStream_t)f->rows_stream));
+    T2N_HIP(hipMemcpy(raw, f->rows_counters, sizeof(raw), hipMemcpyDeviceToHost));
+    for (int l = 0; l < kLists; ++l) { out[0] += raw[l * kCounterStride + kRowsStagedWord]; out[1] += raw[l * kCounterStride + kRowsDirectWord]; }
+    return T2N_OK;
+}
 extern "C" int t2n_render_list_shape(int64_t n_rays, int n_samples, int entries_per_ray, uint64_t out[6]) {
     if (n_rays <= 0 || n_samples <= 0 || entries_per_ray < 0 || !out) { set_error("t2n_render_list_shape: bad argument"); return T2N_ERR_INVALID; }
     const Carve c = carve_workspace(n_rays, n_samples, true, true, (unsigned)entries_per_ray);
diff --git a/text2nerf_amd/csrc/t2n_app_rows.h b/text2nerf_amd/csrc/t2n_app_rows.h
--- a/text2nerf_amd/csrc/t2n_app_rows.h
+++ b/text2nerf_amd/csrc/t2n_app_rows.h
@@ -6,10 +6,16 @@
 
 struct AvVolume { const float* avol; unsigned row, slice, ny1; };
 
-template <int LPE>
+constexpr unsigned kAvBoxCornerBytes = 112;
+struct AvBox { const char* lds; int ox, oy, oz; };
+struct AvNoBox {};
+
+template <int LPE, typename BOX = AvNoBox>
 __device__ __forceinline__ void av_feature_row(const FactorSet& app, const AvVolume& v, const float4 mine, const bool live, const int q,
-                                               float* __restrict__ row, const bool store) {
+                                               float* __restrict__ row, const bool store, const BOX box = BOX()) {
     constexpr int NQ = 8 / LPE;
+    constexpr bool kBox = !__is_same(BOX, AvNoBox);
+    static_assert(!kBox || LPE == 8, "the staged box is read eight lanes per entry");
     const char* __restrict__ V = reinterpret_cast<const char*>(v.avol);
     const Axes3 A = sample_axes_inbox(app, mine.x, mine.y, mine.z);
     const unsigned ix = (unsigned)min(max(A.a[0].i0, 0), app.W[0] - 1), iy = (unsigned)min(max(A.a[1].i0, 0), app.H[0] - 1);
@@ -19,14 +25,20 @@
     const unsigned o01 = o00 + v.row, o10 = o00 + v.slice, o11 = o10 + v.row;
     const unsigned off[4] = {o00, o01, o10, o11};
     float4 c[4][2][NQ];
+    const char* __restrict__ B = nullptr;
+    if constexpr (kBox) {
+        const unsigned bcell = (unsigned)((((int)iz - box.oz) * 4 + ((int)iy - box.oy)) * 4 + ((int)ix - box.ox)) * kAvBoxCornerBytes;
+        B = box.lds + ((live ? bcell : 0u) + (unsigned)min(q, 6) * 16u);
+    } else {
 #pragma unroll
-    for (int zy = 0; zy < 4; ++zy)
+        for (int zy = 0; zy < 4; ++zy)
 #pragma unroll
-        for (int x = 0; x < 2; ++x)
+            for (int x = 0; x < 2; ++x)
 #pragma unroll
-            for (int i = 0; i < NQ; ++i)
-                c[zy][x][i] = *reinterpret_cast<const float4*>(V + (size_t)off[zy] + ((int)kAvCornerBytes * x + 16 * LPE * i));
-    __builtin_amdgcn_sched_barrier(0);
+                for (int i = 0; i < NQ; ++i)
+                    c[zy][x][i] = *reinterpret_cast<const float4*>(V + (size_t)off[zy] + ((int)kAvCornerBytes * x + 16 * LPE * i));
+    }
+    if constexpr (!kBox) __builtin_amdgcn_sched_barrier(0);
     const float wx0 = live ? A.a[0].w0 : 0.f, wx1 = live ? A.a[0].w1 : 0.f;
     const float wyx[2][2] = {{A.a[1].w0 * wx0, A.a[1].w0 * wx1}, {A.a[1].w1 * wx0, A.a[1].w1 * wx1}};
     const float wz[2] = {A.a[2].w0, A.a[2].w1};
@@ -35,6 +47,14 @@
     for (int zy = 0; zy < 4; ++zy)
 #pragma unroll
         for (int x = 0; x < 2; ++x) {
+            if constexpr (kBox) {
+                if ((zy & 1) == 0 && x == 0) {
+                    if (zy) __builtin_amdgcn_sched_barrier(0);
+#pragma unroll
+                    for (int j = 0; j < 4; ++j)
+                        c[zy + (j >> 1)][j & 1][0] = *reinterpret_cast<const float4*>(B + (int)kAvBoxCornerBytes * (((zy >> 1) * 4 + (j >> 1)) * 4 + (j & 1)));
+                }
+            }
             const float w = wyx[zy & 1][x] * wz[zy >> 1];
 #pragma unroll
             for (int i = 0; i < NQ; ++i) r[i] = (zy == 0 && x == 0) ? f4_mul(c[0][0][i], w) : f4_fma(c[zy][x][i], w, r[i]);
diff --git a/text2nerf_amd/csrc/t2n_internal.h b/text2nerf_amd/csrc/t2n_internal.h
--- a/text2nerf_amd/csrc/t2n_internal.h
+++ b/text2nerf_amd/csrc/t2n_internal.h
@@ -135,6 +135,8 @@
     unsigned long long avol_counts[3] = {0, 0, 0};
     int fusion_on = 1;
     unsigned long long fusion_counts[2] = {0, 0};
+    int row_staging_on = 1;
+    const unsigned* rows_counters = nullptr; void* rows_stream = nullptr;
 };
 
 namespace t2n {
@@ -210,6 +212,7 @@
 constexpr int kKeptMagicWord = 33, kKeptRowsWord = 34;
 constexpr int kOverflowWord = 35;
 constexpr int kHeadPlanWord = 40;
+constexpr int kRowsStagedWord = 50, kRowsDirectWord = 51;
 constexpr int kFailEntriesWord = 36;
 constexpr unsigned kKeptMagic = 0x4b455054u;
 int launch_mlp_ss(t2n_field* f, const float* feat, const unsigned* counters_dev, unsigned list_cap, unsigned tile_hi, float4* app_rgb,
diff --git a/text2nerf_amd/csrc/t2n_march_tiles.hip b/text2nerf_amd/csrc/t2n_march_tiles.hip
--- a/text2nerf_amd/csrc/t2n_march_tiles.hip
+++ b/text2nerf_amd/csrc/t2n_march_tiles.hip
@@ -1,3 +1,4 @@
+#include <type_traits>
 #include "t2n_device.h"
 #include "t2n_app_rows.h"
 
@@ -189,6 +190,67 @@
     av_slot_rows(F.app, vol, app_pos + slot, feat + slot * 32u, count, lane);
 }
 
+constexpr int kRsLogMax = 32;
+constexpr unsigned kRsBoxBytes = 64u * kAvBoxCornerBytes;
+constexpr unsigned kRsHdrBytes = 16u;
+constexpr unsigned kRsRecWords = 6u;
+constexpr unsigned kRsWaveBytes = kRsBoxBytes + kRsHdrBytes + (unsigned)kRsLogMax * kRsRecWords * 4u;
+static_assert(4u * kRsWaveBytes <= 32768u && kRsWaveBytes % 16u == 0u, "five blocks per CU: at most 32 KB of LDS per block; 16-B aligned regions");
+
+struct RsBoxRegs { float4 p0, p1, p2, p3, p4, p5, p6, p7; };
+template <int J>
+__device__ __forceinline__ float4 rs_corner_load(const FieldDev& F, unsigned xq, int oy, int oz, int lane) {
+    const unsigned cy = (unsigned)min(oy + ((J & 1) * 2 + (lane >> 5)), F.app.H[0]), cz = (unsigned)min(oz + (J >> 1), F.app.H[1]);
+    const unsigned off = umad24(umad24(cz, (unsigned)F.app.H[0] + 1u, cy), F.av_row, xq);
+    return *reinterpret_cast<const float4*>(reinterpret_cast<const char*>(F.avol) + off);
+}
+__device__ __forceinline__ RsBoxRegs rs_box_load(const FieldDev& F, int ox, int oy, int oz, int lane) {
+    const unsigned xq = (unsigned)min(ox + ((lane >> 3) & 3), F.app.W[0]) * kAvCornerBytes + (unsigned)min(lane & 7, 6) * 16u;
+    RsBoxRegs b;
+    b.p0 = rs_corner_load<0>(F, xq, oy, oz, lane); b.p1 = rs_corner_load<1>(F, xq, oy, oz, lane);
+    b.p2 = rs_corner_load<2>(F, xq, oy, oz, lane); b.p3 = rs_corner_load<3>(F, xq, oy, oz, lane);
+    b.p4 = rs_corner_load<4>(F, xq, oy, oz, lane); b.p5 = rs_corner_load<5>(F, xq, oy, oz, lane);
+    b.p6 = rs_corner_load<6>(F, xq, oy, oz, lane); b.p7 = rs_corner_load<7>(F, xq, oy, oz, lane);
+    return b;
+}
+__device__ __forceinline__ unsigned rs_box_touch(const FieldDev& F, int ox, int oy, int oz, int lane) {
+    const unsigned cx = (unsigned)min(ox + (lane & 3), F.app.W[0]), cy = (unsigned)min(oy + ((lane >> 2) & 3), F.app.H[0]);
+    const unsigned cz = (unsigned)min(oz + (lane >> 4), F.app.H[1]);
+    const unsigned off = umad24(umad24(cz, (unsigned)F.app.H[0] + 1u, cy), F.av_row, cx * kAvCornerBytes);
+    return *reinterpret_cast<const unsigned*>(reinterpret_cast<const char*>(F.avol) + off);
+}
+__device__ __forceinline__ void rs_touch_done(unsigned v) { asm volatile("" ::"v"(v)); }
+__device__ __forceinline__ void rs_box_store(char* __restrict__ box, int lane, const RsBoxRegs& b) {
+    if ((lane & 7) < 7) {
+        constexpr int S = 8 * (int)kAvBoxCornerBytes;
+        char* __restrict__ d = box + (unsigned)(lane >> 3) * kAvBoxCornerBytes + (unsigned)(lane & 7) * 16u;
+        *reinterpret_cast<float4*>(d) = b.p0;         *reinterpret_cast<float4*>(d + S) = b.p1;
+        *reinterpret_cast<float4*>(d + 2 * S) = b.p2; *reinterpret_cast<float4*>(d + 3 * S) = b.p3;
+        *reinterpret_cast<float4*>(d + 4 * S) = b.p4; *reinterpret_cast<float4*>(d + 5 * S) = b.p5;
+        *reinterpret_cast<float4*>(d + 6 * S) = b.p6; *reinterpret_cast<float4*>(d + 7 * S) = b.p7;
+    }
+}
+__device__ __forceinline__ int rs_permute(int dest, int v) { return __builtin_amdgcn_ds_permute(dest << 2, v); }
+__device__ __forceinline__ void rs_rows(const FieldDev& F, const AvVolume& vol, const AvBox& box, unsigned long long mask, const float4 ent,
+                                        unsigned slot, float* __restrict__ feat, int lane) {
+    const int cnt = __popcll(mask);
+    const int rank = (int)__builtin_amdgcn_mbcnt_hi((unsigned)(mask >> 32), __builtin_amdgcn_mbcnt_lo((unsigned)mask, 0u));
+    const bool bit = (mask >> lane) & 1ull;
+    const int dest = bit ? rank : cnt + (lane - rank);
+    const int px = rs_permute(dest, __float_as_int(ent.x)), py = rs_permute(dest, __float_as_int(ent.y)), pz = rs_permute(dest, __float_as_int(ent.z));
+    const int pw = rs_permute(dest, __float_as_int(ent.w)), ps = rs_permute(dest, (int)slot);
+    const int e = lane >> 3, q = lane & 7;
+#pragma unroll 1
+    for (int s0 = 0; s0 < cnt; s0 += 8) {
+        const int src = s0 + e;
+        const float4 mine = make_float4(__int_as_float(__shfl(px, src)), __int_as_float(__shfl(py, src)), __int_as_float(__shfl(pz, src)),
+                                        __int_as_float(__shfl(pw, src)));
+        const unsigned sl = (unsigned)__shfl(ps, src);
+        const bool live = src < cnt;
+        av_feature_row<8>(F.app, vol, mine, live, q, feat + (size_t)(live ? sl : 0u) * 32u + 4u * (unsigned)q, live, box);
+    }
+}
+
 constexpr int kDenseLd = 20;
 constexpr int kDenseFloats = 64 * kDenseLd;
 struct __attribute__((aligned(4))) F4U { float x, y, z, w; };
@@ -211,7 +273,7 @@
 #define MT_T(var) do {} while (0)
 #endif
 constexpr int mt_waves(bool dense, bool cached) { return cached ? (dense ? T2N_MTCD_WAVES : T2N_MTC_WAVES) : (dense ? T2N_MTD_WAVES : T2N_MT_WAVES); }
-template <bool DENSE, bool ALPHA = false, bool RELU = false, bool CACHED = false, bool ROWS = false>
+template <bool DENSE, bool ALPHA = false, bool RELU = false, bool CACHED = false, bool ROWS = false, bool STAGE = false>
 __global__ __launch_bounds__(256) __attribute__((amdgpu_waves_per_eu(mt_waves(DENSE, CACHED), mt_waves(DENSE, CACHED)))) void k_march_tiles(const TileArgs a) {
     extern __shared__ __attribute__((aligned(16))) float smem[];
     const int lane = threadIdx.x & 63, wid = threadIdx.x >> 6;
@@ -223,16 +285,23 @@
     }
     float* __restrict__ wt = smem + (CACHED ? 0 : 4 * kStageFloats) + (size_t)wid * kDenseFloats;
     const FieldDev& F = a.F;
+    static_assert(!STAGE || ROWS, "staged rows: a tail that writes rows");
+    char* __restrict__ rs_box = reinterpret_cast<char*>(smem) + (unsigned)__builtin_amdgcn_readfirstlane(wid) * kRsWaveBytes;
+    unsigned* __restrict__ rs_hdr = reinterpret_cast<unsigned*>(rs_box + kRsBoxBytes);
+    if constexpr (STAGE) {
+        if (lane == 0) { rs_hdr[0] = 0u; rs_hdr[1] = 0u; }
+    }
     const int tiles_x = (a.img_w + 7) >> 3;
     const long long tile = (long long)blockIdx.x * 4 + wid;
     const int ty = (int)(tile / tiles_x), tx = (int)(tile - (long long)ty * tiles_x);
     const int px = tx * 8 + (lane & 7), py = ty * 8 + (lane >> 3);
     if (ty * 8 >= a.img_h) return;
     const bool have = px < a.img_w && py < a.img_h;
-    const long long r = have ? (long long)py * a.img_w + px : 0;
+    typedef typename std::conditional<STAGE, int, long long>::type ray_t;
+    const ray_t r = have ? (ray_t)((long long)py * a.img_w + px) : 0;
     const int N = a.n_samples;
     Ray ray;
-    if (have) ray = load_ray(F, a.rays + r * a.ray_stride, a.ray_stride);
+    if (have) ray = load_ray(F, a.rays + (long long)r * a.ray_stride, a.ray_stride);
     else { ray.ox = ray.oy = ray.oz = 1e30f; ray.dx = ray.dy = ray.dz = 0.f; ray.tmin = 0.f; ray.last = 0.f; }
     int lo = N, hi = -1;
     if (have) ray_interval<false>(F, ray, N, lo, hi);
@@ -289,6 +358,8 @@
         float part[kSteps];
 #pragma unroll
         for (int q = 0; q < kSteps; ++q) part[q] = 0.f;
+        unsigned emv = 0u;
+        unsigned bo = 0u;
         if (okm) {
 #pragma unroll
             for (int q = 0; q < kSteps; ++q) A[q] = sample_axes_inbox(F.den, xn[q], yn[q], zn[q]);
@@ -316,6 +387,7 @@
             const bool ranged = !(bits & 0x40000000u);
             MT_T(p_axes);
             if (CACHED && ranged && span <= 4) {
+                if constexpr (STAGE) bo = 0x40000000u | (unsigned)amn[0] | (unsigned)amn[1] << 10 | (unsigned)amn[2] << 20;
                 unsigned off[kSteps];
                 CellTaps ct[kSteps];
 #pragma unroll
@@ -367,7 +439,10 @@
                 acc += w;
                 dep = fmaf(w, z[q], dep);
                 if (w > F.thres) {
-                    if (napp < (unsigned)a.cap) a.scratch[(size_t)r * a.cap + napp] = make_float4(xn[q], yn[q], zn[q], w);
+                    if (napp < (unsigned)a.cap) {
+                        a.scratch[(size_t)r * a.cap + napp] = make_float4(xn[q], yn[q], zn[q], w);
+                        if constexpr (STAGE) emv |= 1u << q;
+                    }
                     ++napp;
                     if (napp == (unsigned)a.cap) ovf_from = idx + 1;
                 }
@@ -376,7 +451,7 @@
                 ++nev;
                 w_out[q] = w;
             }
-            if (spill) a.wbuf[r * N + idx] = w_out[q];
+            if (spill) a.wbuf[(long long)r * N + idx] = w_out[q];
             if constexpr (DENSE) {
                 if (idx < N) {
                     const int c16 = idx & 15;
@@ -403,6 +478,21 @@
                 }
             }
         }
+        if constexpr (STAGE) {
+            if (__any(emv != 0u)) {
+                const unsigned long long b0 = __ballot((emv & 1u) != 0u), b1 = __ballot((emv & 2u) != 0u);
+                if (lane == 0) {
+                    const unsigned c = rs_hdr[0];
+                    if (!bo || c >= (unsigned)kRsLogMax) rs_hdr[1] = 1u;
+                    else {
+                        unsigned* __restrict__ rec = rs_hdr + 4 + c * kRsRecWords;
+                        rec[0] = bo; rec[1] = 0u;
+                        rec[2] = (unsigned)b0; rec[3] = (unsigned)(b0 >> 32); rec[4] = (unsigned)b1; rec[5] = (unsigned)(b1 >> 32);
+                        rs_hdr[0] = c + 1u;
+                    }
+                }
+            }
+        }
 #ifdef MT_PROF
         MT_T(p_act); ++p_pairs;
 #endif
@@ -434,6 +524,17 @@
     const bool fits = base + total <= a.list_cap;
     if (!fits && total) void_entries(a.app_pos, a.app_ray, list, a.list_cap, base, base + total, lane);
     const unsigned slot0 = list * a.list_cap + base + (incl - n);
+    unsigned rs_n = 0u;
+    bool staged = false;
+    if constexpr (STAGE) {
+        lds_fence_w();
+        rs_n = (unsigned)__builtin_amdgcn_readfirstlane((int)rs_hdr[0]);
+        const unsigned flag = (unsigned)__builtin_amdgcn_readfirstlane((int)rs_hdr[1]);
+        staged = __builtin_amdgcn_readfirstlane((int)(fits && total)) && !flag;
+#ifdef T2N_MT_NO_TAIL_ROWS
+        staged = false;
+#endif
+    }
     if (have) {
         if (over || !fits) {
             const unsigned k = atomicAdd(a.ovf_count, 1u);
@@ -441,7 +542,7 @@
             a.ray_app[r] = make_int4(ovf_from, (int)napp, nev, Lw > 0 ? (first | (Lw << 11)) : 0);
         } else {
             a.ray_app[r] = make_int4((int)slot0, fits ? (int)n : 0, nev, Lw > 0 ? (first | (Lw << 11)) : 0);
-            if (fits) {
+            if (fits && !staged) {
                 const float4* __restrict__ src = a.scratch + (size_t)r * a.cap;
                 for (unsigned k = 0; k < n; k += 4) {
                     const float4 e0 = src[k], e1 = src[k + 1 < n ? k + 1 : n - 1], e2 = src[k + 2 < n ? k + 2 : n - 1],
@@ -460,7 +561,66 @@
         const unsigned ubase = (unsigned)__builtin_amdgcn_readfirstlane((int)base), utotal = (unsigned)__builtin_amdgcn_readfirstlane((int)total);
         unsigned cnt = utotal;
         if (ubase + utotal > a.list_cap) cnt = ubase < a.list_cap ? a.list_cap - ubase : 0u;
-        slot_rows(F, a.app_pos, a.feat, (size_t)list * a.list_cap + ubase, cnt, lane);
+        if constexpr (STAGE) {
+            if (lane == 0 && cnt) atomicAdd(&a.counters[list * kCounterStride + (staged ? kRowsStagedWord : kRowsDirectWord)], 1u);
+#ifdef T2N_RS_STATS
+            if (lane == 0 && staged) { atomicAdd(&a.counters[list * kCounterStride + 52], rs_n); atomicAdd(&a.counters[list * kCounterStride + 53], utotal); }
+#endif
+            if (staged) {
+                const AvVolume vol{F.avol, F.av_row, F.av_slice, (unsigned)F.app.H[0] + 1u};
+                const unsigned long long mine_m = __ballot(have && !over);
+                auto entry_at = [&](unsigned k) {
+                    int rr = (int)r;
+                    asm volatile("" : "+v"(rr));
+                    return a.scratch[(size_t)rr * a.cap + k];
+                };
+                const unsigned* __restrict__ log = rs_hdr + 4;
+                const unsigned last_k = (unsigned)a.cap - 1u;
+                float4 ne0, ne1;
+                unsigned long long nm0, nm1;
+                unsigned kc = 0u;
+                nm0 = ((unsigned long long)log[3] << 32 | log[2]) & mine_m; nm1 = ((unsigned long long)log[5] << 32 | log[4]) & mine_m;
+                nm0 = (unsigned long long)__builtin_amdgcn_readfirstlane((int)(nm0 >> 32)) << 32 | (unsigned)__builtin_amdgcn_readfirstlane((int)nm0);
+                nm1 = (unsigned long long)__builtin_amdgcn_readfirstlane((int)(nm1 >> 32)) << 32 | (unsigned)__builtin_amdgcn_readfirstlane((int)nm1);
+                unsigned nbo = (unsigned)__builtin_amdgcn_readfirstlane((int)log[0]);
+                ne0 = entry_at(min(kc, last_k));
+                ne1 = entry_at(min(kc + (unsigned)((nm0 >> lane) & 1ull), last_k));
+#pragma unroll 1
+                for (unsigned m = 0; m < rs_n; ++m) {
+                    const bool work = (nm0 | nm1) != 0ull;
+                    const AvBox box{rs_box, (int)(nbo & 1023u), (int)((nbo >> 10) & 1023u), (int)((nbo >> 20) & 1023u)};
+                    if (work) rs_box_store(rs_box, lane, rs_box_load(F, box.ox, box.oy, box.oz, lane));
+                    const float4 e0 = ne0, e1 = ne1;
+                    const unsigned long long m0 = nm0, m1 = nm1;
+                    const bool bit0 = (m0 >> lane) & 1ull, bit1 = (m1 >> lane) & 1ull;
+                    const unsigned k0 = kc, k1 = kc + (bit0 ? 1u : 0u);
+                    kc = k1 + (bit1 ? 1u : 0u);
+                    lds_fence_w();
+                    unsigned touched = 0u;
+                    if (m + 1 < rs_n) {
+                        const unsigned* __restrict__ rec = log + (m + 1) * kRsRecWords;
+                        nm0 = ((unsigned long long)rec[3] << 32 | rec[2]) & mine_m; nm1 = ((unsigned long long)rec[5] << 32 | rec[4]) & mine_m;
+                        nm0 = (unsigned long long)__builtin_amdgcn_readfirstlane((int)(nm0 >> 32)) << 32 | (unsigned)__builtin_amdgcn_readfirstlane((int)nm0);
+                        nm1 = (unsigned long long)__builtin_amdgcn_readfirstlane((int)(nm1 >> 32)) << 32 | (unsigned)__builtin_amdgcn_readfirstlane((int)nm1);
+                        nbo = (unsigned)__builtin_amdgcn_readfirstlane((int)rec[0]);
+                        if (nm0 | nm1) {
+                            touched = rs_box_touch(F, (int)(nbo & 1023u), (int)((nbo >> 10) & 1023u), (int)((nbo >> 20) & 1023u), lane);
+                            ne0 = entry_at(min(kc, last_k));
+                            ne1 = entry_at(min(kc + (unsigned)((nm0 >> lane) & 1ull), last_k));
+                        }
+                    }
+                    if (work) {
+                        if (bit0) { a.app_pos[slot0 + k0] = e0; a.app_ray[slot0 + k0] = (int)r; }
+                        if (bit1) { a.app_pos[slot0 + k1] = e1; a.app_ray[slot0 + k1] = (int)r; }
+#pragma unroll 1
+                        for (int q = 0; q < kSteps; ++q)
+                            rs_rows(F, vol, box, q ? m1 : m0, q ? e1 : e0, slot0 + (q ? k1 : k0), a.feat, lane);
+                    }
+                    rs_touch_done(touched);
+                    lds_fence_w();
+                }
+            } else slot_rows(F, a.app_pos, a.feat, (size_t)list * a.list_cap + ubase, cnt, lane);
+        } else slot_rows(F, a.app_pos, a.feat, (size_t)list * a.list_cap + ubase, cnt, lane);
 #endif
     }
 }
@@ -666,6 +826,11 @@
     if (L.slot_rows && !rows) { set_error("launch_march_tiles: a fused frame needs the cached table, the feature volume, no mask and no weights rows"); return T2N_ERR_STATE; }
     a.feat = rows ? L.feat : nullptr;
     ++f->fusion_counts[rows ? 0 : 1];
+    const FactorSet& fd = f->dev.den; const FactorSet& fa = f->dev.app;
+    const bool stage = rows && f->row_staging_on && fd.W[0] == fa.W[0] && fd.H[0] == fa.H[0] && fd.H[1] == fa.H[1] &&
+                       fa.W[0] < 1024 && fa.H[0] < 1024 && fa.H[1] < 1024 &&
+                       L.n_rays <= 0x7fffffffll;
+    f->rows_counters = rows ? L.counters : nullptr; f->rows_stream = (void*)s;
     a.F.term_eps = (!L.weights && !L.z_vals && !L.sigma_ctx) ? f->term_eps : 0.f;
 #ifdef MT_PROF
     static unsigned long long* prof = nullptr;
@@ -682,10 +847,11 @@
         hipLaunchKernelGGL(k_dense_fill, dim3((unsigned)((L.n_rays + 3) / 4)), dim3(256), 0, s, f->dev, L.rays, (long long)L.n_rays, L.ray_stride,
                            L.n_samples, L.weights, L.z_vals);
     const bool cached = f->dev.dsum != nullptr;
-    const size_t lds = (size_t)4 * ((cached ? 0 : kStageFloats) + (dense ? kDenseFloats : 0)) * sizeof(float);
+    const size_t lds = stage ? (size_t)4 * kRsWaveBytes : (size_t)4 * ((cached ? 0 : kStageFloats) + (dense ? kDenseFloats : 0)) * sizeof(float);
     const bool mask = f->dev.alpha != nullptr, relu = f->dev.act == T2N_ACT_RELU;
     ++f->dcache_counts[cached ? 0 : 1];
-#define T2N_MT_LAUNCH(D, A, R) do { if (rows) hipLaunchKernelGGL((k_march_tiles<D, A, R, true, !D && !A>), grid, dim3(256), lds, s, a); \
+#define T2N_MT_LAUNCH(D, A, R) do { if (stage) hipLaunchKernelGGL((k_march_tiles<D, A, R, true, !D && !A, !D && !A>), grid, dim3(256), lds, s, a); \
+                                    else if (rows) hipLaunchKernelGGL((k_march_tiles<D, A, R, true, !D && !A>), grid, dim3(256), lds, s, a); \
                                     else if (cached) hipLaunchKernelGGL((k_march_tiles<D, A, R, true>), grid, dim3(256), lds, s, a); \
                                     else hipLaunchKernelGGL((k_march_tiles<D, A, R, false>), grid, dim3(256), lds, s, a); } while (0)
     if (dense) { if (mask) { if (relu) T2N_MT_LAUNCH(true, true, true); else T2N_MT_LAUNCH(true, true, false); }
diff --git a/text2nerf_amd/tensorf.py b/text2nerf_amd/tensorf.py
--- a/text2nerf_amd/tensorf.py
+++ b/text2nerf_amd/tensorf.py
@@ -360,6 +360,7 @@
         self.appearance_volume_min_frames = 0
         self.appearance_volume_cap_bytes = 0
         self.feature_fusion = True
+        self.row_staging = True
         self.early_termination = 0.0
         self._handle = None
         self._uploaded_key = None
@@ -763,6 +764,7 @@
             self._dcache_set = (True, 0)
             self._avol_set = (True, 0, 0)
             self._fusion_set = True
+            self._row_staging_set = True
             self._stage_shape_set = (0, 0)
             self._head_rows_set = 32
             self._alpha_key = "unset"
@@ -816,6 +818,10 @@
         if getattr(self, "_fusion_set", True) != fu:
             _lib.check(lib.t2n_field_set_feature_fusion(self._handle, 1 if fu else 0), "t2n_field_set_feature_fusion")
             self._fusion_set = fu
+        rs = bool(getattr(self, "row_staging", True))
+        if getattr(self, "_row_staging_set", True) != rs:
+            _lib.check(lib.t2n_field_set_row_staging(self._handle, 1 if rs else 0), "t2n_field_set_row_staging")
+            self._row_staging_set = rs
         shape = tuple(int(v) for v in self.feature_stage_shape)
         if getattr(self, "_stage_shape_set", (0, 0)) != shape:
             _lib.check(lib.t2n_field_set_feature_stage_shape(self._handle, shape[0], shape[1]), "t2n_field_set_feature_stage_shape")
@@ -1597,6 +1603,12 @@
             _lib.check(_lib.load().t2n_field_feature_fusion_counts(self._handle, out), "t2n_field_feature_fusion_counts")
         return {"fused": int(out[0]), "unfused": int(out[1])}
 
+    def row_staging_counts(self):
+        out = (C.c_uint64 * 2)()
+        if self._handle is not None:
+            _lib.check(_lib.load().t2n_field_row_staging_counts(self._handle, out), "t2n_field_row_staging_counts")
+        return {"staged": int(out[0]), "direct": int(out[1])}
+
     def density_sum_table(self, shift=(0, 0, 0)):
         h = self.sync_params()
         g = [int(v) for v in self.gridSize]
```

Result: faster. 189.9 billion ray-samples/s, median of 6 (+2.0%).
